# alipbcs/ZetaRay

Hardware: NVIDIA H100
Metric: Mpaths/s (1spp ReSTIR PT, 1080p) (higher is better)
Workload: dtype f32

## Files before the change

include/zr_abi.h:

```cpp
#ifndef ZR_ABI_H
#define ZR_ABI_H

#include <stdint.h>
#include <stddef.h>

#ifdef __cplusplus
extern "C" {
#endif

#if defined(_WIN32)
#define ZR_API __declspec(dllexport)
#else
#define ZR_API __attribute__((visibility("default")))
#endif

typedef int32_t zr_status;
enum
{
    ZR_OK = 0,
    ZR_ERR_INVALID_ARG = 1,
    ZR_ERR_CUDA = 2,
    ZR_ERR_NOT_INITIALIZED = 3,
    ZR_ERR_UNSUPPORTED = 4,
    ZR_ERR_OUT_OF_MEMORY = 5
// ... 176 lines not shown
    uint32_t le_b_meta;
    uint32_t lightIdx;
    float w_sum;
    float W;
    uint32_t pad[2];
} zr_rdi_reservoir;

typedef struct zr_image2d
{
    void* d_ptr;
    uint32_t width;
    uint32_t height;
    uint32_t pitch_bytes;
    uint32_t texel_bytes;
} zr_image2d;

typedef void (*zr_halo_exchange_fn)(void* user, const zr_image2d* planes, int n_planes, void* stream);

typedef struct zr_scene zr_scene;

typedef struct zr_scene_desc
{
    const zr_vertex* h_vertices;            uint32_t num_vertices;
    const uint32_t* h_indices;              uint32_t num_indices;
    const zr_mesh_instance* h_instances;    uint32_t num_instances;
    const uint32_t* h_instance_num_tris;
    const zr_material* h_materials;         uint32_t num_materials;
    const zr_emissive_tri* h_emissives;     uint32_t num_emissives;
} zr_scene_desc;

ZR_API zr_status zr_scene_create(const zr_scene_desc* desc, zr_scene** out);
ZR_API void zr_scene_destroy(zr_scene* scene);
ZR_API zr_status zr_scene_bvh_stats(const zr_scene* scene, uint32_t out[4]);

ZR_API zr_status zr_bvh_build_host(const float* h_world_tris, uint32_t num_tris, void* h_nodes, uint32_t node_capacity,
    uint32_t* h_leaf_order, uint32_t out_info[4]);

ZR_API zr_status zr_scene_trace_closest(const zr_scene* scene, const float* d_rays, uint32_t n,
    float* d_hits, void* stream);
ZR_API zr_status zr_scene_trace_any(const zr_scene* scene, const float* d_rays, uint32_t n,
    uint32_t* d_hit_flags, void* stream);


ZR_API zr_status zr_alias_table_build(float* d_weights, uint32_t n, zr_alias_entry* d_table,
    uint32_t* d_scratch, void* stream);
ZR_API zr_status zr_alias_table_sample(const zr_alias_entry* d_table, uint32_t n, uint32_t seed,
    uint32_t num_draws, uint32_t* d_out_idx, float* d_out_pdf, void* stream);
ZR_API zr_status zr_estimate_emissive_power(const zr_scene* scene, float* d_power, void* stream);
ZR_API zr_status zr_prelighting_render(zr_scene* scene, void* stream);

typedef struct zr_presampled_tri
{
    float pos[3];
    uint32_t normal;
    float pdf;
    uint32_t ID;
    uint32_t idx;
    uint32_t bary;
    uint16_t le[3];
    uint16_t twoSided;
} zr_presampled_tri;
#define ZR_PRESAMPLING_MIN_EMISSIVES 13107u
#define ZR_PRESAMPLING_NUM_SETS 128u
#define ZR_PRESAMPLING_SET_SIZE 512u
ZR_API zr_status zr_scene_set_presampling(zr_scene* scene, uint32_t num_sets, uint32_t set_size);
ZR_API zr_status zr_presample_emissives(zr_scene* scene, uint32_t frame_num, void* stream);
// ... 221 lines not shown
```

zetaray_b200/csrc/rdi.cu:

```cuda
#include "zr_pixel.cuh"
#include "zr_planes.h"
#include "zr_schedule.h"

#include "zr_rdi.cuh"

namespace zr
{
namespace
{
#ifndef ZR_RDI_THREADS
#define ZR_RDI_THREADS 512
#endif
    __global__ void ZR_LB(ZR_RDI_THREADS) k_di_temporal(SceneDev sc, FrameView f, DIParams prm, zr_rdi_reservoir* __restrict__ resCurr,
        const zr_rdi_reservoir* __restrict__ resPrev, uint2* __restrict__ target, float4* __restrict__ finalImg, uint32_t dispX, uint32_t dispY,
        const uint32_t* __restrict__ order)
    {
        const zr_frame_constants& fc = f.fc;
        uint2 sg = make_uint2(0, 0);
        const uint32_t groupFlat = order[blockIdx.x] * (ZR_RDI_THREADS / 64) + (threadIdx.x >> 6);
        const uint32_t tInGroup = threadIdx.x & 63;
        uint2 px = make_uint2(0xffffffffu, 0xffffffffu);
        if (groupFlat < dispX * dispY)
            px = SwizzleThreadGroup(groupFlat, 0, tInGroup & 7, tInGroup >> 3, 8, 8, dispX, 16, 4, 16 * dispY, sg);
        const long long t0 = clock64();
        bool act = !(px.x >= f.W || px.y >= f.H || px.y < prm.rowBegin || px.y >= prm.rowEnd);
        const uint32_t x = px.x, y = px.y;
        const size_t idx = act ? (size_t)y * f.W + x : 0;
        if (act)
        {
            const GFlags flags = FlagsAt(f.core, f.W, x, y);
            if (flags.invalid)
            {
                finalImg[idx] = f4(0, 0, 0, 0);
                act = false;
            }
            else if (flags.emissive && !prm.spatial)
            {
                WriteEmissive(fc, f, finalImg, idx);
                act = false;
            }
        }
        Pixel p;
        p.surface = BSDF::ShadingData::InitEmpty();
        p.pos = f3(0); p.normal = f3(0); p.roughness = 0;
        RNG rng_thread; rng_thread.State = 0;
        int numBsdfSamples = 0;
        if (act)
        {
            p = LoadPixel(f, sc, f.core, f.coat, x, y, false, x, y);
            rng_thread = RNG::Init(x, y, fc.FrameNum);
            numBsdfSamples = (!p.surface.GlossSpecular() && p.roughness < 0.3f) ? 2 : 1;
        }
        RNG rng_group = RNG::Init(groupFlat % dispX, groupFlat / dispX, fc.FrameNum);
        const uint32_t sampleSetIdx = rng_group.UniformUintBounded_Faster(sc.numSampleSets);
        Reservoir r = RIS_InitialCandidates_Sync(act, sc, p.pos, p.normal, p.roughness, p.surface, sampleSetIdx, numBsdfSamples, rng_thread);
        if (prm.temporal)
        {
            float2 motionVec = f2(0, 0);
            TemporalCandidate tc; tc.valid = false; tc.px = tc.py = 0; tc.pos = tc.normal = f3(0);
            tc.surface = BSDF::ShadingData::InitEmpty();
            ZR_PHASE();
            if (act)
            {
                motionVec = unpack_snorm16x2(__ldg(&f.me[idx].x));
                const float2 currUV = f2((float)x + 0.5f, (float)y + 0.5f) / f2((float)f.W, (float)f.H);
                const float2 prevUV = currUV - motionVec;
                tc = FindTemporalCandidate(f, sc, p.pos, p.normal, p.roughness, p.surface, prevUV);
            }
            TemporalResample1_Sync(act && tc.valid, sc, p.pos, p.normal, p.surface, tc, resPrev, f.W, r, rng_thread);
            if (act && prm.spatial)
            {
                const bool disoccluded = !tc.valid && (dot(motionVec, motionVec) > 0);
                r.target = disoccluded ? -r.target : r.target;
                WriteTarget(target, idx, r.target);
                r.target = Math::Sanitize(r.target);
            }
        }
        AccountCost(prm.costMap, f.W, f.H, px.x, px.y, t0);
        if (!act)
            return;
        if (prm.temporal || prm.reset)
        {
            zr_rdi_reservoir rec;
            r.Write(rec, prm.M_max);
            StoreRdi(&resCurr[idx], rec);
        }
        if (!prm.spatial || !prm.temporal)
            WriteFinal(fc, finalImg, idx, r.target * r.W);
    }

    __global__ void ZR_LB(ZR_RDI_THREADS) k_di_spatial(SceneDev sc, FrameView f, DIParams prm, const zr_rdi_reservoir* __restrict__ resCurr,
        const uint2* __restrict__ target, float4* __restrict__ finalImg, uint32_t dispX, uint32_t dispY,
        const uint32_t* __restrict__ order)
    {
        const zr_frame_constants& fc = f.fc;
        uint2 sg = make_uint2(0, 0);
        const uint32_t groupFlat = order[blockIdx.x] * (ZR_RDI_THREADS / 64) + (threadIdx.x >> 6);
        const uint32_t tInGroup = threadIdx.x & 63;
        uint2 px = make_uint2(0xffffffffu, 0xffffffffu);
        if (groupFlat < dispX * dispY)
            px = SwizzleThreadGroup(groupFlat, 0, tInGroup & 7, tInGroup >> 3, 8, 8, dispX, 16, 4, 16 * dispY, sg);
        const long long t0 = clock64();
        bool active = px.x < f.W && px.y < f.H && px.y >= prm.rowBegin && px.y < prm.rowEnd;
        const int x = (int)px.x, y = (int)px.y;
        const size_t idx = active ? (size_t)y * f.W + x : 0;
        if (active)
        {
            const GFlags flags = FlagsAt(f.core, f.W, x, y);
            if (flags.invalid) active = false;
            else if (flags.emissive)
            {
                WriteEmissive(fc, f, finalImg, idx);
                active = false;
            }
        }
        Pixel p;
        p.surface = BSDF::ShadingData::InitEmpty();
        p.pos = f3(0); p.normal = f3(0); p.roughness = 0; p.z = 0;
        Reservoir r = Reservoir::Init();
        bool disoccluded = false;
        if (active)
        {
            p = LoadPixel(f, sc, f.core, f.coat, x, y, false, x, y);
            zr_rdi_reservoir rec;
            LoadRdi(&resCurr[idx], rec);
            r = Reservoir::Load(rec);
            if (r.lightIdx != UINT32_MAX_)
            {
                const zr_emissive_tri& tri = sc.emissives[r.lightIdx];
                r.lightID = tri.ID;
                const float3 vtx0 = Light::Vtx0(tri);
                const float3 vtx1 = Light::DecodeEmissiveTriV1(tri);
                const float3 vtx2 = Light::DecodeEmissiveTriV2(tri);
                r.lightPos = (1.0f - r.bary.x - r.bary.y) * vtx0 + r.bary.x * vtx1 + r.bary.y * vtx2;
                r.lightNormal = cross(vtx1 - vtx0, vtx2 - vtx0);
                r.lightNormal = dot(r.lightNormal, r.lightNormal) == 0 ? r.lightNormal : normalize(r.lightNormal);
                r.doubleSided = Light::IsDoubleSided(tri);
                r.target = LoadTarget(target, idx);
                disoccluded = r.target.x < 0 || r.target.y < 0 || r.target.z < 0;
                r.target = abs3(r.target);
            }
        }
        const uint32_t waveDisoccluded = __popc(__ballot_sync(0xffffffffu, active && disoccluded));
        RNG rng_group = RNG::Init(groupFlat % dispX, groupFlat / dispX, fc.FrameNum);
        rng_group.UniformUintBounded_Faster(sc.numSampleSets);
        const bool extra = !prm.stochasticSpatial || (rng_group.Uniform() < 0.6f);
        if (prm.extraDisocclusion)
            disoccluded = disoccluded && (waveDisoccluded > 3);
        int numSamples = extra ? 2 : 1;
        numSamples = !disoccluded ? numSamples : 4;
        RNG rng = RNG::Init((uint32_t)x, (uint32_t)y, fc.FrameNum);
        const float u0 = rng.Uniform();
        const int offset = (int)rng.UniformUintBounded_Faster(8);
        const float theta = u0 * TWO_PI;
        float sinTheta, cosTheta;
        zr_sincosf(theta, &sinTheta, &cosTheta);
        PairwiseMIS pairwiseMIS = PairwiseMIS::Init((uint32_t)numSamples, r);
        float3 samplePos[4]; int spx[4], spy[4]; uint32_t k = 0;
        ZR_PHASE();
        for (int i = 0; i < 4; i++)
        {
            if (!(active && i < numSamples)) continue;
            const float2 sampleUV = f2(c_disk32[((offset + i) & 31) * 2], c_disk32[((offset + i) & 31) * 2 + 1]);
            float2 rotated;
            rotated.x = dot(sampleUV, f2(cosTheta, -sinTheta));
            rotated.y = dot(sampleUV, f2(sinTheta, cosTheta));
            rotated = rotated * 16.0f;
            const float fx = fmaxf(rintf((float)x + rotated.x), 0.0f), fy = fmaxf(rintf((float)y + rotated.y), 0.0f);
            if (fx >= (float)f.W || fy >= (float)f.H) continue;
            const int qx = (int)fx, qy = (int)fy;
            float rough_i;
            const GFlags flags_i = FlagsAt(f.core, f.W, qx, qy, &rough_i);
            if (flags_i.invalid || flags_i.emissive) continue;
            const Pixel pi = LoadPixel(f, sc, f.core, f.coat, qx, qy, false, qx, qy);
            bool valid = PlaneHeuristicDI(pi.pos, p.normal, p.pos, p.z);
            valid = valid && (fabsf(rough_i - p.roughness) < 0.15f);
            if (!valid) continue;
            samplePos[k] = pi.pos; spx[k] = qx; spy[k] = qy;
            k++;
        }
        pairwiseMIS.k = k;
        for (uint32_t i = 0; i < 4; i++)
        {
            const bool go = active && (i < k);
            if (!__syncthreads_or(go))
                break;
            Pixel pi;
            pi.normal = f3(0);
            BSDF::ShadingData surface_i = BSDF::ShadingData::InitEmpty();
            Reservoir r_spatial = Reservoir::Init();
            float3 pos_i = f3(0);
            if (go)
            {
                pi = LoadPixel(f, sc, f.core, f.coat, spx[i], spy[i], false, spx[i], spy[i]);
                const uint4 c = ld128(&f.core[(size_t)spy[i] * f.W + spx[i]]);
                const float3 bc = f3((float)(c.z & 0xff) / 255.0f, (float)((c.z >> 8) & 0xff) / 255.0f, (float)((c.z >> 16) & 0xff) / 255.0f);
                const float bw = pi.flags.subsurface ? (float)(c.z >> 24) / 255.0f : 0.0f;
                pos_i = samplePos[i];
                const float3 wo_i = normalize(pi.origin - pos_i);
                surface_i = BSDF::ShadingData::Init(pi.normal, wo_i, pi.flags.metallic, pi.roughness, bc, BSDF::ETA_AIR,
                    pi.eta_next, pi.flags.transmissive, 0.0f, to_half(bw), pi.surface.coat_weight, pi.surface.coat_color,
                    pi.coatRoughness, pi.coatIor, sc.rho);
                zr_rdi_reservoir recN;
                LoadRdi(&resCurr[(size_t)spy[i] * f.W + spx[i]], recN);
                r_spatial = Reservoir::Load(recN);
            }
            pairwiseMIS.Stream_Sync(go, sc, r, p.pos, p.normal, p.surface, r_spatial, pos_i, pi.normal, surface_i, rng);
        }
        AccountCost(prm.costMap, f.W, f.H, px.x, px.y, t0);
        if (!active)
            return;
        pairwiseMIS.End(r, rng);
        const Reservoir rs = pairwiseMIS.r_s;
        WriteFinal(fc, finalImg, idx, rs.target * rs.W);
    }
}
}

struct zr_direct_pass
{
    uint32_t width = 0, height = 0;
    struct Sized
    {
        zr::Planes planes{ "zr_direct_pass" };
        zr_rdi_reservoir* d_res[2] = { nullptr, nullptr };
        uint2* d_target = nullptr;
        float4* d_final = nullptr;
    } sz;
    int currTemporalIdx = 0;
    bool isTemporalReservoirValid = false;
    bool resetTemporalTextures = true;
    bool patternLoaded = false;
    zr_direct_params params = Defaults();
// ... 30 lines not shown
    }
    zr_status LoadPattern()
    {
        if (patternLoaded) return ZR_OK;
        float pat[64];
        zr_status st = zr::read_asset("zr_direct_pass", "disk32.bin", pat, sizeof(pat));
        if (st != ZR_OK) return st;
        ZR_CUDA(cudaMemcpyToSymbol(zr::c_disk32, pat, 256));
        patternLoaded = true;
        return ZR_OK;
    }
    zr_status Render(const zr_frame_inputs* in, cudaStream_t stream)
    {
        using namespace zr;
        FrameView f;
        zr_status st = LightingFrame("zr_direct_pass", in, width, height, f);
        if (st != ZR_OK) return st;
        st = LoadPattern();
        if (st != ZR_OK) return st;
        const bool doTemporal = isTemporalReservoirValid && params.temporal_resample;
        const bool doSpatial = doTemporal && params.spatial_resample;
        if (doTemporal && (!in->prev.d_core || !in->prev.d_coat))
        {
            set_error("zr_direct_pass_render: temporal reuse needs the previous G-buffer");
            return ZR_ERR_INVALID_ARG;
        }
        DIParams prm{ doTemporal, doSpatial, params.stochastic_spatial, params.extra_disocclusion_sampling, params.M_max,
            params.alpha_min, resetTemporalTextures, strip.rowBegin, strip.ClampedRowEnd(height), strip.d_costMap };
        const uint32_t dispX = (width + 7) / 8, dispY = (height + 7) / 8;
        const int cur = currTemporalIdx;
        st = strip.Schedule(width, height, 8, 8, ZR_RDI_THREADS / 64);
        if (st != ZR_OK) return st;
        const BlockSchedule& sched = strip.sched;
        ZR_PROF("k_di_temporal", stream);
        k_di_temporal<<<sched.count, ZR_RDI_THREADS, 0, stream>>>(in->scene->dev, f, prm, sz.d_res[cur], sz.d_res[1 - cur], sz.d_target, sz.d_final, dispX, dispY, sched.d_order);
        ZR_LAUNCH_CHECK();
        strip.Exchange(sz.d_res[cur], width, height, 32u, stream);
        if (doSpatial)
        {
            ZR_PROF("k_di_spatial", stream);
            k_di_spatial<<<sched.count, ZR_RDI_THREADS, 0, stream>>>(in->scene->dev, f, prm, sz.d_res[cur], sz.d_target, sz.d_final, dispX, dispY, sched.d_order);
            ZR_LAUNCH_CHECK();
        }
        isTemporalReservoirValid = true;
        currTemporalIdx = 1 - cur;
        resetTemporalTextures = false;
        return ZR_OK;
    }
};

extern "C"
{
    zr_status zr_direct_pass_create(uint32_t width, uint32_t height, zr_direct_pass** out) { return zr::CreatePass("zr_direct_pass", width, height, out); }
    zr_status zr_direct_pass_resize(zr_direct_pass* p, uint32_t width, uint32_t height) { return zr::ResizePass("zr_direct_pass", p, width, height); }
    zr_status zr_direct_pass_reset_temporal(zr_direct_pass* p) { return zr::ResetPass(p); }
    zr_status zr_direct_pass_default_params(zr_direct_params* out) { return zr::DefaultParams<zr_direct_pass>(out); }
    zr_status zr_direct_pass_set_params(zr_direct_pass* p, const zr_direct_params* params)
    {
        if (!p || !params) return ZR_ERR_INVALID_ARG;
        if (params->M_max == 0 || params->M_max > 31) { zr::set_error("zr_direct_pass_set_params: M_max must be in 1..31 (5-bit field)"); return ZR_ERR_INVALID_ARG; }
        p->params = *params;
        return ZR_OK;
    }
    zr_status zr_direct_pass_render(zr_direct_pass* p, const zr_frame_inputs* in, void* stream)
    {
        if (!p) return ZR_ERR_INVALID_ARG;
        return p->Render(in, (cudaStream_t)stream);
    }
    zr_status zr_direct_pass_set_rows(zr_direct_pass* p, uint32_t y0, uint32_t y1) { return p ? p->strip.SetRows(y0, y1, p->height) : ZR_ERR_INVALID_ARG; }
    zr_status zr_direct_pass_set_halo_exchange(zr_direct_pass* p, zr_halo_exchange_fn fn, void* user) { return p ? p->strip.SetHaloExchange(fn, user) : ZR_ERR_INVALID_ARG; }
    zr_status zr_direct_pass_set_schedule_costs(zr_direct_pass* p, const double* h_tile_cost, uint32_t tiles_x, uint32_t tiles_y)
    {
        return p ? p->strip.SetScheduleCosts(h_tile_cost, tiles_x, tiles_y, p->width, p->height) : ZR_ERR_INVALID_ARG;
    }
// ... 28 lines not shown
```

zetaray_b200/csrc/rpt.cu:

```cuda
#include "zr_rpt_io.cuh"
#include "zr_rpt_spatial.h"
#include "zr_schedule.h"

namespace zr
{
namespace
{
    using namespace RPT;

    __device__ __align__(8) float c_disk512[1024];

#ifndef ZR_PT_THREADS
#define ZR_PT_THREADS 768
#endif
    struct PtParked
    {
        Reservoir r;
        Reconnection rc;
        uint32_t pad;
    };
    static_assert(sizeof(PtParked) % 4 == 0 && (sizeof(PtParked) / 4) % 2 == 1, "PtParked must be an odd number of words");
    constexpr size_t PT_SMEM_BYTES = (size_t)ZR_PT_THREADS * sizeof(PtParked);

    __global__ void ZR_LB(ZR_PT_THREADS) k_pathtrace(SceneDev sc, FrameView f, RptParams prm, zr_rpt_reservoir* __restrict__ res,
        float4* __restrict__ target, float4* __restrict__ finalImg, uint32_t dispX, uint32_t dispY, const uint32_t* __restrict__ order)
    {
        extern __shared__ PtParked s_ptParked[];
        const zr_frame_constants& fc = f.fc;
        const long long t0 = clock64();
        uint2 sg = make_uint2(0, 0);
        const uint32_t groupFlat = order[blockIdx.x] * (ZR_PT_THREADS / 128) + (threadIdx.x >> 7);
        const uint32_t tInGroup = threadIdx.x & 127;
        uint2 px = make_uint2(0xffffffffu, 0xffffffffu);
        if (groupFlat < dispX * dispY)
            px = SwizzleThreadGroup(groupFlat, 0, tInGroup & 15, tInGroup >> 4, 16, 8, dispX, 16, 4, 16 * dispY, sg);
        bool inBounds = px.x < f.W && px.y < f.H && px.y >= prm.rowBegin && px.y < prm.rowEnd;
        const size_t idx = (size_t)px.y * f.W + px.x;
        bool alive = false;
        if (inBounds)
        {
            const GFlags flags = FlagsAt(f.core, f.W, px.x, px.y);
            if (flags.invalid || flags.emissive)
            {
                if (!fc.Accumulate || !fc.CameraStatic)
                    finalImg[idx] = f4(0, 0, 0, 0);
                inBounds = false;
            }
        }
        float3 pos = f3(0), normal = f3(0), li = f3(0), throughput = f3(0), throughput_k = f3(1), tr = f3(1);
        BSDF::ShadingData surface;
        BSDF::BSDFSample bsdfSample = BSDF::BSDFSample::Init();
        HitEmissive nextHit;
        nextHit.hit = false;
        Reconnection& rc = s_ptParked[threadIdx.x].rc;
        Reservoir& r = s_ptParked[threadIdx.x].r;
        rc = Reconnection::Init();
        r = Reservoir::Init();
        PrevHit prevHit;
        prevHit.alpha_lobe = 0; prevHit.wi = f3(0); prevHit.pdf = 0; prevHit.lobe = BSDF::DIFFUSE_R;
        float eta_curr = BSDF::ETA_AIR, eta_next = BSDF::DEFAULT_ETA_MAT;
        bool inTranslucentMedium = false;
        int bounce = 0, maxNumBounces = 0;
        RNG rngReplay, rngThread, rngGroup;
        rngReplay.State = rngThread.State = rngGroup.State = 0;
        uint32_t sampleSetIdx = 0;
        uint32_t seedReplay0 = 0;

        if (inBounds)
        {
            const Pixel p = LoadPixel(f, sc, f.core, f.coat, px.x, px.y, false, px.x, px.y);
            rngGroup = RNG::Init4(sg.x, sg.y, fc.FrameNum, 1);
            const uint3 state = RNG::PCG3d(make_uint3(px.x, px.y, fc.FrameNum));
            rngReplay = RNG::InitSeed(state.x);
            rngThread = RNG::InitSeed(state.y);
            seedReplay0 = state.x;
            maxNumBounces = (int)(p.surface.specTr ? prm.maxGlossyTrBounces : prm.maxNonTrBounces);
            bsdfSample = BSDF::SampleBSDF(p.normal, p.surface, rngReplay);
            if (dot(bsdfSample.bsdfOverPdf, bsdfSample.bsdfOverPdf) != 0)
            {
                sampleSetIdx = rngGroup.UniformUintBounded_Faster(sc.numSampleSets);
                pos = p.pos; normal = p.normal; surface = p.surface;
                throughput = bsdfSample.bsdfOverPdf;
                prevHit.alpha_lobe = BSDF::LobeAlpha(p.surface, bsdfSample.lobe);
                prevHit.lobe = bsdfSample.lobe; prevHit.wi = bsdfSample.wi; prevHit.pdf = bsdfSample.pdf;
                eta_curr = dot(p.normal, bsdfSample.wi) < 0 ? p.eta_next : BSDF::ETA_AIR;
                inTranslucentMedium = eta_curr != BSDF::ETA_AIR;
                alive = true;
            }
        }
        ZR_PHASE();
        if (alive)
            nextHit = FindClosestEmissive(sc, pos, normal, bsdfSample.wi, surface.Transmissive());

        while (__syncthreads_or(alive))
        {
            bool atRR = false;
            Hit hitInfo;
            float prevBsdfSamplePdf = 0; BSDF::LOBE prevBsdfSampleLobe = BSDF::DIFFUSE_R;
            const int pathVertex = bounce + 2;
            if (alive && !nextHit.hit)
                alive = false;
            if (alive)
            {
                hitInfo = HitAttributes(sc, nextHit.geoIdx, nextHit.primIdx, nextHit.bary, nextHit.t);
                const float3 newPos = mad(hitInfo.t, bsdfSample.wi, pos);
                if (!GetMaterialData(sc, -bsdfSample.wi, eta_curr, hitInfo, surface, eta_next))
                    alive = false;
                else
                {
                    pos = newPos;
                    normal = hitInfo.normal;
                    prevBsdfSamplePdf = bsdfSample.pdf;
                    prevBsdfSampleLobe = bsdfSample.lobe;
                    tr = f3(1);
                    if (inTranslucentMedium && (surface.trDepth > 0))
                    {
                        const float3 c = surface.baseColor_Fr0_TrCol;
                        const float3 extCoeff = f3(-zr_logf(c.x), -zr_logf(c.y), -zr_logf(c.z)) / surface.trDepth;
                        tr = f3(zr_expf(-hitInfo.t * extCoeff.x), zr_expf(-hitInfo.t * extCoeff.y), zr_expf(-hitInfo.t * extCoeff.z));
                        throughput *= tr;
                    }
                }
            }
            ZR_PHASE();
            BSDF::BSDFSample nextBsdfSample = bsdfSample;
            const int nextBounce = pathVertex - 1;
            if (alive && nextBounce <= maxNumBounces)
                nextBsdfSample = BSDF::SampleBSDF(hitInfo.normal, surface, rngReplay);
            ZR_PHASE();
            RaySetup rs; rs.go = false;
            RayHit rh; rh.hit = false;
            if (alive)
            {
                rs = SetupClosestEmissive(pos, hitInfo.normal, nextBsdfSample.wi, surface.Transmissive());
                if (rs.go)
                    rh = TraceClosest(sc, rs.o, nextBsdfSample.wi, rs.tmin, FLT_MAX_);
            }
            ZR_PHASE();
            NeeLightState nee;
            nee.facing = false; nee.ld = f3(0);
            bool lightSample = false;
            uint32_t seed_nee = 0;
            if (alive)
            {
                nextHit = FinishClosestEmissive(sc, rs, rh, nextBsdfSample.wi);
                const DirectLightingEstimate ls_b = NEE_Bsdf_Finish(sc, pos, surface, nextBounce, maxNumBounces, nextBsdfSample, nextHit);
                if (nextHit.HitWasEmissive())
                {
                    const float3 fOverPdf = throughput * ls_b.ld;
                    li += fOverPdf;
                    rc.L = Reconnection::half3(ls_b.ld * throughput_k);
                    MaybeSetCase2OrCase3(pathVertex, pos, hitInfo.normal, hitInfo.t, hitInfo.ID, hitInfo.meshIdx, surface,
                        prevHit, ls_b, 0, rc, prm.alpha_min);
                    r.Update(Math::Luminance(fOverPdf), fOverPdf, rc, rngThread);
                }
                lightSample = !IsSpecularSurface(surface);
                if (lightSample)
                {
                    seed_nee = rngThread.State;
                    BSDF::ShadingData surfNee = surface;
                    nee = NEE_Emissive_Begin(sc, pos, hitInfo.normal, surfNee, sampleSetIdx, rngThread);
                }
            }
            ZR_PHASE();
            if (lightSample && nee.facing && dot(nee.ld, nee.ld) > 0)
            {
                const RaySetup seg = SetupSegment(pos, nee.ret.wi, nee.t, hitInfo.normal, nee.ret.ID, surface.Transmissive());
                const bool visible = seg.go ? !TraceAnyExcept(sc, seg.o, nee.ret.wi, seg.tmin, seg.tmax, nee.ret.ID) : false;
                nee.ld *= visible ? 1.0f : 0.0f;
            }
            ZR_PHASE();
            if (lightSample)
            {
                float bsdfPdf = 0;
                if (nee.facing && dot(nee.ld, nee.ld) > 0)
                {
                    BSDF::ShadingData surfNee = surface;
                    surfNee.SetWi(nee.ret.wi, hitInfo.normal);
                    bsdfPdf = BSDF::BSDFSamplerPdf(hitInfo.normal, surfNee, nee.ret.wi, rngThread);
                    bsdfPdf *= nee.dwdA;
                }
                const DirectLightingEstimate ls = NEE_Emissive_Finish(nee, bsdfPdf);
                const float3 fOverPdf = throughput * ls.ld;
                li += fOverPdf;
                if (rc.IsCase2() || rc.IsCase3())
                    rc.Clear();
                rc.L = Reconnection::half3(ls.ld * throughput_k);
                MaybeSetCase2OrCase3(pathVertex, pos, hitInfo.normal, hitInfo.t, hitInfo.ID, hitInfo.meshIdx, surface,
                    prevHit, ls, seed_nee, rc, prm.alpha_min);
                r.Update(Math::Luminance(fOverPdf), fOverPdf, rc, rngThread);
            }
            if (alive)
            {
                bsdfSample = nextBsdfSample;
                if (bounce >= (maxNumBounces - 1))
                    alive = false;
                else
                {
                    if (rc.IsCase2() || rc.IsCase3())
                        rc.Clear();
                    bounce++;
                    atRR = true;
                }
            }
            const uint32_t rrMask = __ballot_sync(0xffffffffu, atRR);
            if (rrMask == 0)
                continue;
            const int rrBounce = __shfl_sync(0xffffffffu, bounce, __ffs(rrMask) - 1);
            const bool doRR = prm.russianRoulette && (rrBounce >= 3);
            float waveThroughput = 0.0f;
// ... 251 lines not shown

struct zr_indirect_pass
{
    uint32_t width = 0, height = 0;
    struct Sized
    {
        zr::Planes planes{ "zr_indirect_pass" };
        zr_rpt_reservoir* d_res[2] = { nullptr, nullptr };
        float4* d_target = nullptr;
        float4* d_final = nullptr;
        uint16_t* d_neighbor = nullptr;
        uint16_t* d_threadMap = nullptr;
        zr::SpatialQueued queued;
    } sz;
    zr::ShiftStreams shiftStreams;
    int currTemporalIdx = 0;
    bool isTemporalReservoirValid = false;
    bool resetTemporalTextures = true;
    bool patternLoaded = false;
    zr::LightingStrip strip{ "zr_indirect_pass" };
    zr_indirect_params params = Defaults();

    static zr_indirect_params Defaults()
    {
        zr_indirect_params p{};
        p.max_non_tr_bounces = 3; p.max_glossy_tr_bounces = 4; p.russian_roulette = 1; p.temporal_resample = 1;
        p.num_spatial_passes = 1; p.M_max_temporal = 10; p.M_max_spatial = 8; p.boiling_suppression = 1;
        p.sort_temporal = 1; p.sort_spatial = 1; p.alpha_min = 0.175f * 0.175f;
        return p;
    }

    zr_status Setup()
    {
        ZR_CUDA(cudaFuncSetAttribute(zr::k_pathtrace, cudaFuncAttributeMaxDynamicSharedMemorySize, (int)zr::PT_SMEM_BYTES));
        int ptBlocks = 0;
        ZR_CUDA(cudaOccupancyMaxActiveBlocksPerMultiprocessor(&ptBlocks, zr::k_pathtrace, ZR_PT_THREADS, zr::PT_SMEM_BYTES));
        if (ptBlocks < 1)
        {
            zr::set_error("zr_indirect_pass: k_pathtrace (%d threads, %zu B shared) cannot be resident", ZR_PT_THREADS, zr::PT_SMEM_BYTES);
            return ZR_ERR_UNSUPPORTED;
        }
        const size_t ptSmem = (size_t)ptBlocks * (zr::PT_SMEM_BYTES + 1024);
        ZR_CUDA(cudaFuncSetAttribute(zr::k_pathtrace, cudaFuncAttributePreferredSharedMemoryCarveout,
            (int)((ptSmem * 100 + 228 * 1024 - 1) / (228 * 1024))));
        return shiftStreams.Init();
    }

    zr_status OnWindowResized(uint32_t w, uint32_t h)
    {
        const size_t n = (size_t)w * h;
        Sized next;
        for (int i = 0; i < 2; i++) ZR_TRY(next.planes.Alloc(next.d_res[i], n));
        ZR_TRY(next.planes.Alloc(next.d_threadMap, n));
        ZR_TRY(next.planes.Alloc(next.d_target, n));
        ZR_TRY(next.planes.Alloc(next.d_final, n));
        ZR_TRY(next.planes.Alloc(next.d_neighbor, n));
        ZR_TRY(next.queued.Build(w, h, next.d_res[0], next.d_res[1]));
        ZR_TRY(next.planes.Clear());
        sz = std::move(next);
        width = w; height = h;
        strip.ForgetSize();
        ResetFlags();
        return ZR_OK;
    }

    void ResetFlags() { currTemporalIdx = 0; isTemporalReservoirValid = false; resetTemporalTextures = true; }
    zr_status ResetTemporal()
    {
        ZR_TRY(sz.planes.Clear());
        ResetFlags();
        return ZR_OK;
    }

    zr_status LoadPattern()
    {
        if (patternLoaded) return ZR_OK;
        float pat[1024];
// ... 3 lines not shown
        patternLoaded = true;
        return ZR_OK;
    }

    zr_status Render(const zr_frame_inputs* in, cudaStream_t stream)
    {
        using namespace zr;
        FrameView f;
        zr_status st = LightingFrame("zr_indirect_pass", in, width, height, f);
        if (st != ZR_OK) return st;
        st = LoadPattern();
        if (st != ZR_OK) return st;

        const bool doTemporal = params.temporal_resample && isTemporalReservoirValid;
        const bool doSpatial = (params.num_spatial_passes > 0) && doTemporal;
        if (doTemporal && (!in->prev.d_core || !in->prev.d_coat))
        {
            set_error("zr_indirect_pass_render: temporal reuse needs the previous G-buffer");
            return ZR_ERR_INVALID_ARG;
        }
        RptParams prm;
        prm.maxNonTrBounces = params.max_non_tr_bounces; prm.maxGlossyTrBounces = params.max_glossy_tr_bounces;
        prm.russianRoulette = params.russian_roulette; prm.M_max_temporal = params.M_max_temporal; prm.M_max_spatial = params.M_max_spatial;
        prm.boilingSuppression = params.boiling_suppression; prm.sortSpatial = params.sort_spatial; prm.alpha_min = params.alpha_min;
        prm.temporalResample = doTemporal; prm.resetTemporal = resetTemporalTextures; prm.spatialFlag = doSpatial;
        prm.rowBegin = strip.rowBegin; prm.rowEnd = strip.ClampedRowEnd(height);
        prm.costMap = strip.d_costMap;
        st = strip.Schedule(width, height, 16, 8, ZR_PT_THREADS / 128);
        if (st != ZR_OK) return st;
        const uint32_t rows = prm.rowEnd - prm.rowBegin;

        int cur = currTemporalIdx;
        const uint32_t dispX = (width + 15) / 16, dispY = (height + 7) / 8;
        ZR_PROF("k_pathtrace", stream);
        k_pathtrace<<<strip.sched.count, ZR_PT_THREADS, PT_SMEM_BYTES, stream>>>(in->scene->dev, f, prm, sz.d_res[cur], sz.d_target, sz.d_final, dispX, dispY,
            strip.sched.d_order);
        ZR_LAUNCH_CHECK();
        if (doTemporal)
        {
            st = sz.queued.RunTemporal(shiftStreams, in->scene->dev, f, prm, sz.d_res[cur], sz.d_res[1 - cur], sz.d_target, sz.d_final, stream);
            if (st != ZR_OK) return st;
        }
        strip.Exchange(sz.d_res[cur], width, height, 64u, stream);
        if (doSpatial)
        {
            for (uint32_t pass = 0; pass < params.num_spatial_passes; pass++)
            {
                ZR_PROF("k_spatial_search", stream);
                k_spatial_search<<<dim3((width + 31) / 32, (rows + 7) / 8), 256, 0, stream>>>(f, prm, sz.d_neighbor);
                ZR_LAUNCH_CHECK();
                zr_rpt_reservoir* rin = sz.d_res[cur];
                zr_rpt_reservoir* rout = sz.d_res[1 - cur];
                cur = 1 - cur;
                if (params.sort_spatial)
                {
                    const uint32_t sx = (width + 31) / 32, sy = (height + 31) / 32;
                    ZR_PROF("k_sort", stream);
                    const uint32_t ty0 = prm.rowBegin / 32, ty1 = (prm.rowEnd + 31) / 32;
                    k_sort<<<dim3(sx, ty1 - ty0), 256, 0, stream>>>(f, 3, 1u, rin, nullptr, sz.d_neighbor, sz.d_threadMap, sx, sy, ty0);
                    ZR_LAUNCH_CHECK();
                }
                st = sz.queued.Run(shiftStreams, in->scene->dev, f, prm, rin, rout, sz.d_target, sz.d_final, sz.d_neighbor, sz.d_threadMap, stream);
                if (st != ZR_OK) return st;
                strip.Exchange(rout, width, height, 64u, stream);
            }
        }
        isTemporalReservoirValid = true;
        currTemporalIdx = 1 - cur;
        resetTemporalTextures = false;
        return ZR_OK;
    }
};

extern "C"
{
    zr_status zr_indirect_pass_create(uint32_t width, uint32_t height, zr_indirect_pass** out) { return zr::CreatePass("zr_indirect_pass", width, height, out); }
    zr_status zr_indirect_pass_resize(zr_indirect_pass* p, uint32_t width, uint32_t height) { return zr::ResizePass("zr_indirect_pass", p, width, height); }
    zr_status zr_indirect_pass_reset_temporal(zr_indirect_pass* p) { return zr::ResetPass(p); }
    zr_status zr_indirect_pass_default_params(zr_indirect_params* out) { return zr::DefaultParams<zr_indirect_pass>(out); }
    zr_status zr_indirect_pass_set_params(zr_indirect_pass* p, const zr_indirect_params* params)
    {
        if (!p || !params) return ZR_ERR_INVALID_ARG;
        if (params->max_non_tr_bounces < 1 || params->max_non_tr_bounces > 8 || params->max_glossy_tr_bounces < 1 ||
            params->max_glossy_tr_bounces > 8 || params->M_max_temporal > 15 || params->M_max_spatial > 15 || params->num_spatial_passes > 2)
        {
            zr::set_error("zr_indirect_pass_set_params: value out of range (bounces 1..8, M_max <= 15, spatial passes <= 2)");
            return ZR_ERR_INVALID_ARG;
        }
        p->params = *params;
        return ZR_OK;
    }
    zr_status zr_indirect_pass_render(zr_indirect_pass* p, const zr_frame_inputs* in, void* stream)
    {
        if (!p) return ZR_ERR_INVALID_ARG;
        return p->Render(in, (cudaStream_t)stream);
// ... 38 lines not shown
```

zetaray_b200/csrc/rpt_spatial.cu:

```cuda
#include "zr_rpt_spatial.h"
#include "zr_rpt_shift.cuh"
#include "zr_tma.cuh"

namespace zr
{
namespace
{
    using namespace RPT;

    __global__ void __launch_bounds__(256) k_spatial_classify(FrameView f, RptParams prm, const zr_rpt_reservoir* __restrict__ resIn,
        const uint16_t* __restrict__ neighbor, uint32_t* __restrict__ queue, uint32_t* __restrict__ counters, uint32_t capacity)
    {
        __shared__ uint32_t s_count[SpatialQueued::NUM_CLASSES], s_base[SpatialQueued::NUM_CLASSES];
        const uint32_t x = blockIdx.x * 32 + (threadIdx.x & 31);
        const uint32_t y = prm.rowBegin + blockIdx.y * 8 + (threadIdx.x >> 5);
        if (threadIdx.x < SpatialQueued::NUM_CLASSES) s_count[threadIdx.x] = 0;
        __syncthreads();
        uint32_t cls[2] = { NO_ITEM, NO_ITEM };
        if (x < f.W && y < f.H && y < prm.rowEnd)
        {
            const GFlags flags = FlagsAt(f.core, f.W, (int)x, (int)y);
            int nx = 0, ny = 0;
            if (!(flags.invalid || flags.emissive) && NeighborOf(f, neighbor, (int)x, (int)y, nx, ny))
            {
// ... 290 lines not shown
    capacity = 2 * n;
    ZR_TRY(planes.Alloc(d_queue, NUM_CLASSES * capacity, false));
    ZR_TRY(planes.Alloc(d_counters, 16, false));
    ZR_TRY(planes.Alloc(d_shift, n));
    ZR_TRY(planes.Alloc(d_flags, n));
    ZR_TRY(planes.Alloc(d_maps, 2, false));
    const zr_rpt_reservoir* res[2] = { res0, res1 };
    CUtensorMap maps[2];
    swizzled = (w % 2) == 0;
    for (int i = 0; i < 2; i++)
    {
        mapBase[i] = res[i];
        bool ok;
        if (swizzled)
        {
            const uint64_t dims[3] = { 16, w / 2, h };
            const uint64_t strides[2] = { 128, (uint64_t)w * 64 };
            const uint32_t box[3] = { 16, 16, 32 };
            ok = tma::EncodeWords(&maps[i], res[i], 3, dims, strides, box, true);
        }
        else
            ok = tma::EncodePlane2D(&maps[i], res[i], w, h, 64, (uint64_t)w * 64, 32, 32);
        if (!ok)
        {
            set_error("zr_indirect_pass: cuTensorMapEncodeTiled failed for the %ux%u reservoir plane", w, h);
            return ZR_ERR_CUDA;
        }
    }
    ZR_CUDA(cudaMemcpy(d_maps, maps, sizeof(maps), cudaMemcpyHostToDevice));
    return planes.Clear();
}

zr_status SpatialQueued::Run(const ShiftStreams& ss, const SceneDev& sc, const FrameView& f, const RptParams& prm, const zr_rpt_reservoir* resIn,
    zr_rpt_reservoir* resOut, const float4* target, float4* finalImg, const uint16_t* neighbor, const uint16_t* threadMap, cudaStream_t stream)
{
    const int plane = resIn == mapBase[0] ? 0 : (resIn == mapBase[1] ? 1 : -1);
    if (plane < 0) { set_error("zr_indirect_pass: spatial input is not one of the pass's reservoir planes"); return ZR_ERR_INVALID_ARG; }
    const uint32_t rows = prm.rowEnd - prm.rowBegin;
    ZR_CUDA(cudaMemsetAsync(d_counters, 0, 16 * sizeof(uint32_t), stream));
    {
        ZR_PROF("k_spatial_classify", stream);
        k_spatial_classify<<<dim3((width + 31) / 32, (rows + 7) / 8), 256, 0, stream>>>(f, prm, resIn, neighbor, d_queue, d_counters, (uint32_t)capacity);
        ZR_LAUNCH_CHECK();
    }
    {
        ZR_PROF("k_shift", stream);
        const zr_status ls = LaunchShifts<false>(*this, ss, sc, f, prm, resIn, nullptr, neighbor, stream);
        zr::prof_after();
        if (ls != ZR_OK) return ls;
        cudaError_t e = cudaGetLastError();
        if (e != cudaSuccess) return zr::cuda_fail(e, "k_shift launch");
    }
    {
        const uint32_t tilesX = (width + 31) / 32;
        const uint32_t tileRow0 = prm.rowBegin / 32, tileRow1 = (prm.rowEnd + 31) / 32;
        const uint32_t numTiles = tilesX * (tileRow1 - tileRow0);
        const uint32_t grid = numTiles < (uint32_t)ss.numSMs ? numTiles : (uint32_t)ss.numSMs;
        ZR_PROF("k_spatial_merge", stream);
        k_spatial_merge<<<grid, 1024, sizeof(MergeSmem), stream>>>(d_maps + plane, f, prm, resIn, resOut, target, finalImg, neighbor, threadMap,
            d_shift, tilesX, tileRow0, numTiles, swizzled ? 1u : 0u);
        ZR_LAUNCH_CHECK();
    }
    return ZR_OK;
}
}
```

zetaray_b200/csrc/rpt_temporal.cu:

```cuda
#include "zr_rpt_spatial.h"
#include "zr_rpt_shift.cuh"

namespace zr
{
namespace
{
    using namespace RPT;
    enum : uint8_t { TF_OK = 1, TF_REPLAY_OK = 2 };

    __global__ void __launch_bounds__(256) k_temporal_classify(SceneDev sc, FrameView f, RptParams prm, const zr_rpt_reservoir* __restrict__ resCurr,
        const zr_rpt_reservoir* __restrict__ resPrev, uint8_t* __restrict__ tflags, uint32_t* __restrict__ queue, uint32_t* __restrict__ counters,
        uint32_t capacity)
    {
        __shared__ uint32_t s_count[SpatialQueued::NUM_CLASSES], s_base[SpatialQueued::NUM_CLASSES];
        const int x = (int)(blockIdx.x * 32 + (threadIdx.x & 31));
        const int y = (int)(prm.rowBegin + blockIdx.y * 8 + (threadIdx.x >> 5));
        if (threadIdx.x < SpatialQueued::NUM_CLASSES) s_count[threadIdx.x] = 0;
        __syncthreads();
        uint32_t cls[2] = { NO_ITEM, NO_ITEM };
        uint32_t flagBits = 0;
        if (x < (int)f.W && y < (int)f.H && y < (int)prm.rowEnd)
        {
            const size_t idx = (size_t)y * f.W + x;
            const GFlags flags = DecodeFlags(ld128(&f.core[idx]).w & 0xff);
// ... 115 lines not shown
            const float m_prev = denom > 0 ? numerator / denom : 0;
            const float w_prev = m_prev * r_prev.W * targetLum_curr;
            if (r_curr.Update(w_prev, shTarget, r_prev.rc, rng))
            {
                r_curr.rc.partialJacobian = shJ;
                changed = true;
            }
        }
        const float targetLum = Math::Luminance(r_curr.target);
        r_curr.W = targetLum > 0 ? r_curr.w_sum / targetLum : 0;
        r_curr.M = M_new;
        if (changed)
        {
            zr_rpt_reservoir out;
            r_curr.Write(out, M_max);
            StoreRecord(&resCurr[idx], out);
            if (prm.spatialFlag)
            {
                r_curr.target = Math::Sanitize(r_curr.target);
                target[idx] = f4(r_curr.target.x, r_curr.target.y, r_curr.target.z, 0.0f);
            }
        }
        else
        {
            r_curr.WriteReservoirData(rec, M_max);
            st128(&resCurr[idx], make_uint4(rec.meta, asuint(rec.w_sum), asuint(rec.W), rec.L_b));
        }
        if (!prm.spatialFlag)
            WriteOutputColor(fc, finalImg, idx, r_curr.target * r_curr.W);
    }
}

zr_status SpatialQueued::RunTemporal(const ShiftStreams& ss, const SceneDev& sc, const FrameView& f, const RptParams& prm, zr_rpt_reservoir* resCurr,
    const zr_rpt_reservoir* resPrev, float4* target, float4* finalImg, cudaStream_t stream)
{
    const uint32_t rows = prm.rowEnd - prm.rowBegin;
    const dim3 grid((width + 31) / 32, (rows + 7) / 8);
    ZR_CUDA(cudaMemsetAsync(d_counters, 0, 16 * sizeof(uint32_t), stream));
    {
        ZR_PROF("k_temporal_classify", stream);
        k_temporal_classify<<<grid, 256, 0, stream>>>(sc, f, prm, resCurr, resPrev, d_flags, d_queue, d_counters, (uint32_t)capacity);
        ZR_LAUNCH_CHECK();
    }
    {
        ZR_PROF("k_shift_temporal", stream);
        const zr_status ls = LaunchShifts<true>(*this, ss, sc, f, prm, resCurr, resPrev, nullptr, stream);
        zr::prof_after();
        if (ls != ZR_OK) return ls;
        cudaError_t e = cudaGetLastError();
        if (e != cudaSuccess) return zr::cuda_fail(e, "k_shift (temporal) launch");
    }
    {
        ZR_PROF("k_temporal_merge", stream);
        k_temporal_merge<<<grid, 256, 0, stream>>>(sc, f, prm, resCurr, resPrev, target, finalImg, d_flags, d_shift);
        ZR_LAUNCH_CHECK();
    }
    return ZR_OK;
}
}
```

zetaray_b200/csrc/scene.cu:

```cuda
#include "zr_scene.cuh"
#include <vector>
#include <algorithm>
#include <cmath>
#include <cstring>

namespace zr
{
namespace
{
    __global__ void k_world_tris(SceneDev sc, const uint32_t* __restrict__ triMesh, const uint32_t* __restrict__ meshFirstTri,
        uint32_t numTris, float* __restrict__ out )
    {
        const uint32_t g = blockIdx.x * blockDim.x + threadIdx.x;
        if (g >= numTris) return;
        const uint32_t m = triMesh[g];
        const uint32_t p = g - meshFirstTri[m];
        const zr_mesh_instance md = LoadInstance(sc, m);
        const float4 q = normalize(Math::DecodeNormalized4(md.Rotation));
        const float3 s = h3(md.Scale);
        const float3 t = f3(md.Translation[0], md.Translation[1], md.Translation[2]);
        const uint32_t tri = p * 3 + md.BaseIdxOffset;
        float3 pw[3];
        for (int k = 0; k < 3; k++)
        {
// ... 59 lines not shown
            if (mi.MatIdx >= desc->num_materials)
            {
                set_error("zr_scene_create: instance %u uses material %u of %u", m, (unsigned)mi.MatIdx, desc->num_materials);
                return ZR_ERR_INVALID_ARG;
            }
            for (uint64_t i = 0; i < 3 * nt; i++)
                if ((uint64_t)mi.BaseVtxOffset + desc->h_indices[mi.BaseIdxOffset + i] >= desc->num_vertices)
                {
                    set_error("zr_scene_create: instance %u, index %llu points past the vertex buffer", m, (unsigned long long)i);
                    return ZR_ERR_INVALID_ARG;
                }
            if (mi.BaseEmissiveTriOffset != 0xffffffffu && (uint64_t)mi.BaseEmissiveTriOffset + nt > desc->num_emissives)
            {
                set_error("zr_scene_create: instance %u's emissive triangles [%u, %llu) lie past the %u emissive triangles", m,
                    mi.BaseEmissiveTriOffset, (unsigned long long)(mi.BaseEmissiveTriOffset + nt), desc->num_emissives);
                return ZR_ERR_INVALID_ARG;
            }
            totalTris += nt;
        }
        if (totalTris == 0) { set_error("zr_scene_create: scene has no triangles"); return ZR_ERR_INVALID_ARG; }
        if (totalTris > 0x7fffffffull) { set_error("zr_scene_create: more than 2^31 triangles"); return ZR_ERR_INVALID_ARG; }
        if (desc->num_emissives && !desc->h_emissives) { set_error("zr_scene_create: null emissive buffer"); return ZR_ERR_INVALID_ARG; }
    }
    zr_scene* sc = new zr_scene();
    zr_status st;
#define UP(field, ptr, n) if ((st = upload(sc, ptr, n, &sc->dev.field)) != ZR_OK) { zr_scene_destroy(sc); return st; }
    UP(vertices, desc->h_vertices, desc->num_vertices);
    UP(indices, desc->h_indices, desc->num_indices);
    UP(instances, desc->h_instances, desc->num_instances);
    UP(materials, desc->h_materials, desc->num_materials);
    UP(emissives, desc->h_emissives, desc->num_emissives);
    sc->dev.numInstances = desc->num_instances;
    sc->dev.numEmissives = desc->num_emissives;

    std::vector<uint32_t> triMesh, meshFirst(desc->num_instances);
    uint32_t total = 0;
    for (uint32_t m = 0; m < desc->num_instances; m++)
    {
        meshFirst[m] = total;
        if (desc->h_instances[m].BaseIdxOffset + 3 * desc->h_instance_num_tris[m] > desc->num_indices)
        {
            set_error("zr_scene_create: instance %u indexes past the index buffer", m);
            zr_scene_destroy(sc);
            return ZR_ERR_INVALID_ARG;
        }
        for (uint32_t p = 0; p < desc->h_instance_num_tris[m]; p++) triMesh.push_back(m);
        total += desc->h_instance_num_tris[m];
    }
    if (total == 0) { set_error("zr_scene_create: scene has no triangles"); zr_scene_destroy(sc); return ZR_ERR_INVALID_ARG; }
    sc->dev.numTris = total;
    UP(triMesh, triMesh.data(), triMesh.size());
    UP(meshFirstTri, meshFirst.data(), meshFirst.size());

    {
        std::vector<uint16_t> rho(64 * 32 * 16);
        if ((st = read_asset("zr_scene_create", "rho_lut.bin", rho.data(), rho.size() * sizeof(uint16_t))) != ZR_OK) { zr_scene_destroy(sc); return st; }
        UP(rho, rho.data(), rho.size());
    }

    float* d_wt = nullptr;
    cudaError_t e = cudaMalloc(&d_wt, (size_t)total * 9 * sizeof(float));
    if (e != cudaSuccess) { zr_scene_destroy(sc); return cuda_fail(e, "world triangles (alloc)"); }
    k_world_tris<<<(total + 127) / 128, 128>>>(sc->dev, sc->dev.triMesh, sc->dev.meshFirstTri, total, d_wt);
    count_launch();
    e = cudaGetLastError();
    std::vector<float> wt((size_t)total * 9);
// ... 51 lines not shown
    zr_status zr_scene_create(const zr_scene_desc* desc, zr_scene** out) { return zr::scene_create(desc, out); }
    void zr_scene_destroy(zr_scene* sc)
    {
        if (!sc) return;
        for (int i = 0; i < sc->numAllocs; i++) cudaFree(sc->allocs[i]);
        if (sc->d_alias) cudaFree(sc->d_alias);
        if (sc->d_power) cudaFree(sc->d_power);
        if (sc->d_aliasScratch) cudaFree(sc->d_aliasScratch);
        if (sc->d_sampleSets) cudaFree(sc->d_sampleSets);
        if (sc->d_lvg) cudaFree(sc->d_lvg);
        delete sc;
    }
    zr_status zr_bvh_build_host(const float* h_world_tris, uint32_t num_tris, void* h_nodes, uint32_t node_capacity,
        uint32_t* h_leaf_order, uint32_t out_info[4])
    {
        if (!h_world_tris || !out_info || num_tris == 0) { zr::set_error("zr_bvh_build_host: null argument"); return ZR_ERR_INVALID_ARG; }
        zr::BvhBuild w;
        zr::build_bvh8(h_world_tris, num_tris, w);
        out_info[0] = (uint32_t)w.nodes.size(); out_info[1] = num_tris; out_info[2] = w.maxDepth; out_info[3] = w.maxStack;
        if (h_nodes)
        {
            if (node_capacity < w.nodes.size()) { zr::set_error("zr_bvh_build_host: %zu nodes, capacity %u", w.nodes.size(), node_capacity); return ZR_ERR_INVALID_ARG; }
            memcpy(h_nodes, w.nodes.data(), w.nodes.size() * sizeof(zr::BVH8Node));
        }
        if (h_leaf_order) memcpy(h_leaf_order, w.leafOrder.data(), (size_t)num_tris * sizeof(uint32_t));
        return ZR_OK;
    }
    zr_status zr_scene_bvh_stats(const zr_scene* sc, uint32_t out[4])
    {
        if (!sc || !out) return ZR_ERR_INVALID_ARG;
        out[0] = sc->info.numNodes; out[1] = sc->info.numTris; out[2] = sc->info.maxDepth; out[3] = sc->info.bytes;
        return ZR_OK;
    }
    zr_status zr_scene_trace_closest(const zr_scene* sc, const float* d_rays, uint32_t n, float* d_hits, void* stream)
    {
        if (!sc || !d_rays || !d_hits) { zr::set_error("zr_scene_trace_closest: null argument"); return ZR_ERR_INVALID_ARG; }
        if (n == 0) return ZR_OK;
        ZR_PROF("k_trace_closest", (cudaStream_t)stream);
        zr::k_trace_closest<<<(n + 127) / 128, 128, 0, (cudaStream_t)stream>>>(sc->dev, d_rays, n, d_hits);
        ZR_LAUNCH_CHECK();
        return ZR_OK;
    }
    zr_status zr_scene_trace_any(const zr_scene* sc, const float* d_rays, uint32_t n, uint32_t* d_flags, void* stream)
    {
        if (!sc || !d_rays || !d_flags) { zr::set_error("zr_scene_trace_any: null argument"); return ZR_ERR_INVALID_ARG; }
        if (n == 0) return ZR_OK;
        ZR_PROF("k_trace_any", (cudaStream_t)stream);
        zr::k_trace_any<<<(n + 127) / 128, 128, 0, (cudaStream_t)stream>>>(sc->dev, d_rays, n, d_flags);
        ZR_LAUNCH_CHECK();
        return ZR_OK;
    }
    zr_status zr_scene_get_alias_table(const zr_scene* sc, const zr_alias_entry** d_table, uint32_t* n)
    {
        if (!sc || !d_table || !n) return ZR_ERR_INVALID_ARG;
        *d_table = sc->d_alias; *n = sc->dev.numEmissives;
        return ZR_OK;
    }
}
```

zetaray_b200/csrc/zr_bsdf.cuh:

```cuda
#pragma once
#include "zr_common.cuh"

namespace zr
{
namespace RT
{
    ZR_D float BalanceHeuristic(float p_1, float p_2, float f, float n_1 = 1, float n_2 = 1)
    {
        float denom = n_1 * p_1 + n_2 * p_2;
        if (denom == 0) return 0;
        return (n_1 * f) / denom;
    }
    ZR_D float BalanceHeuristic3(float p_1, float p_2, float p_3, float f, float n_1 = 1, float n_2 = 1, float n_3 = 1)
    {
        float denom = n_1 * p_1 + n_2 * p_2 + n_3 * p_3;
        if (denom == 0) return 0;
        return (n_1 * f) / denom;
    }
    ZR_D float3 PowerHeuristic(float p_1, float p_2, float3 f, float n_1 = 1, float n_2 = 1)
    {
        float a = n_1 * p_1;
        float b = n_2 * p_2;
        float denom = a * a + b * b;
        if (denom == 0) return f3(0);
// ... 149 lines not shown
        f *= dwh_dwi;
        f *= ndotwi;
        return f * (1 - fr);
    }
    ZR_D float3 SampleGGXVNDF(float3 wo, float alpha_x, float alpha_y, float2 u)
    {
        float3 Vh = normalize(f3(alpha_x * wo.x, alpha_y * wo.y, wo.z));
        float phi = TWO_PI * u.x;
        float z = mad((1.0f - u.y), (1.0f + Vh.z), -Vh.z);
        float sinTheta = sqrtf(saturate(1.0f - z * z));
        float s, c;
        zr_sincosf(phi, &s, &c);
        float x = sinTheta * c;
        float y = sinTheta * s;
        float3 cc = f3(x, y, z);
        float3 Nh = cc + Vh;
        return normalize(f3(alpha_x * Nh.x, alpha_y * Nh.y, fmaxf(0.0f, Nh.z)));
    }
    ZR_D float3 SampleGGXMicrofacet(float3 wo, float alpha, float3 shadingNormal, float2 u)
    {
        Math::CoordinateSystem onb = Math::CoordinateSystem::Build(shadingNormal);
        float3 woLocal = f3(dot(onb.b1, wo), dot(onb.b2, wo), dot(shadingNormal, wo));
        float3 whLocal = SampleGGXVNDF(woLocal, alpha, alpha, u);
        return mad(whLocal.x, onb.b1, mad(whLocal.y, onb.b2, whLocal.z * shadingNormal));
    }
    ZR_D float GGXMicrofacetPdf(float alpha, float ndotwh, float ndotwo)
    {
        float alphaSq = alpha * alpha;
        float NDF = GGX(ndotwh, alphaSq);
        float G1 = SmithG1(alphaSq, ndotwo);
        return (NDF * G1) / ndotwo;
    }

    struct ShadingData
    {
        float alpha;
        float3 wo;
        float ndotwi, ndotwo, ndotwh, whdotwi, whdotwo, wodotwi, g_wo;
        float3 baseColor_Fr0_TrCol;
        float eta;
        bool specTr, metallic, backfacing_wo, invalid, reflection;
        float trDepth;
        float subsurface;
        float coat_weight;
        float3 coat_color;
        float coat_alpha;
        float coat_eta;
        const uint16_t* rho;

        static ZR_D ShadingData InitEmpty()
        {
            ShadingData ret;
            memset(&ret, 0, sizeof(ret));
            ret.eta = DEFAULT_ETA_MAT / ETA_AIR;
            ret.coat_eta = DEFAULT_ETA_COAT;
            return ret;
        }
        static ZR_D ShadingData Init(float3 shadingNormal, float3 wo, bool metallic, float roughness, float3 baseColor,
            float eta_curr = ETA_AIR, float eta_next = DEFAULT_ETA_MAT, bool specTr = false,
            float transmissionDepth = 0, float subsurface = 0, float coat_weight = 0, float3 coat_color = f3(0.0f),
            float coat_roughness = 0, float eta_coat = DEFAULT_ETA_COAT, const uint16_t* rhoTable = nullptr)
        {
            float2 roughness4 = f2(roughness, coat_roughness);
            if (coat_weight > 0 && coat_roughness > 0)
            {
                roughness4 = roughness4 * roughness4;
                roughness4 = roughness4 * roughness4;
                float roughness_coated = fminf(roughness4.x + 2 * roughness4.y, 1);
                roughness_coated = rsqrt_(rsqrt_(roughness_coated));
                roughness = Math::Lerp(roughness, roughness_coated, coat_weight);
            }
            ShadingData si;
            memset(&si, 0, sizeof(si));
            si.wo = wo;
            float ndotwo = dot(shadingNormal, wo);
            si.backfacing_wo = ndotwo <= 0;
            si.ndotwo = fmaxf(ndotwo, 1e-5f);
            si.metallic = metallic;
            si.alpha = roughness * roughness;
            si.baseColor_Fr0_TrCol = baseColor;
            si.specTr = specTr;
            si.trDepth = to_half(transmissionDepth);
            si.subsurface = to_half(subsurface);
            float eta_base = eta_curr == ETA_AIR ? eta_next : eta_curr;
            float eta_no_coat = eta_next / eta_curr;
            float eta_coated = eta_base >= eta_coat ? eta_base / eta_coat : eta_coat / eta_base;
            si.eta = Math::Lerp(eta_no_coat, eta_coated, coat_weight);
            si.g_wo = !metallic && !specTr ? E_FON_approx(fmaxf(ndotwo, 1e-4f), roughness) : 0;
            si.coat_weight = coat_weight;
            si.coat_color = coat_color;
            si.coat_alpha = coat_roughness * coat_roughness;
            si.coat_eta = eta_curr == ETA_AIR ? eta_coat / ETA_AIR : ETA_AIR / eta_coat;
            si.rho = rhoTable;
            return si;
        }

        ZR_D bool ThinWalled() const { return subsurface > 0; }
        ZR_D bool Transmissive() const { return specTr || ThinWalled(); }
        ZR_D bool Coated() const { return coat_weight != 0; }
        ZR_D bool GlossSpecular() const { return alpha <= MAX_ALPHA_SPECULAR; }
        ZR_D bool CoatSpecular() const { return coat_alpha <= MAX_ALPHA_SPECULAR; }
        ZR_D float3 TransmissionTint() const { return trDepth > 0 ? f3(1) : baseColor_Fr0_TrCol; }

        ZR_D void SetWi_Refl(float3 wi, float3 shadingNormal, float3 wh)
        {
            reflection = true;
            float ndotwi_n = dot(shadingNormal, wi);
            ndotwh = saturate(dot(shadingNormal, wh));
            whdotwo = saturate(dot(wh, wo));
            whdotwi = whdotwo;
            bool isInvalid = backfacing_wo || ndotwh == 0 || whdotwo == 0;
            invalid = isInvalid || ndotwi_n <= 0;
            ndotwi = fmaxf(ndotwi_n, 1e-5f);
            wodotwi = dot(wo, wi);
        }
        ZR_D void SetWi_Refl(float3 wi, float3 shadingNormal)
        {
            float3 wh = normalize(wi + wo);
            SetWi_Refl(wi, shadingNormal, wh);
        }
        ZR_D void SetWi_Tr(float3 wi, float3 shadingNormal, float3 wh)
        {
            reflection = false;
            float ndotwi_n = dot(shadingNormal, wi);
            ndotwh = saturate(dot(shadingNormal, wh));
            whdotwo = saturate(dot(wh, wo));
            whdotwi = fabsf(dot(wh, wi));
            bool isInvalid = backfacing_wo || (specTr && (ndotwh == 0 || whdotwo == 0));
            invalid = isInvalid || ndotwi_n >= 0 || !Transmissive() || metallic;
            ndotwi = fmaxf(fabsf(ndotwi_n), 1e-5f);
            wodotwi = dot(wo, wi);
        }
// ... 27 lines not shown
            tir = false;
            if (metallic)
                return FresnelSchlick(fr0, cosTheta_i);
            float eta_relative = 1.0f / eta;
            float sinTheta_iSq = saturate(mad(-cosTheta_i, cosTheta_i, 1.0f));
            float cosTheta_tSq = mad(-eta_relative * eta_relative, sinTheta_iSq, 1.0f);
            tir = cosTheta_tSq <= 0;
            if (tir)
                return f3(1);
            float cosTheta_t = sqrtf(cosTheta_tSq);
            return f3(Fresnel_Dielectric(cosTheta_i, eta_relative, cosTheta_t));
        }
        ZR_D float3 Fresnel() const
        {
            float3 fr0 = metallic ? baseColor_Fr0_TrCol : f3(DielectricF0(eta));
            bool unused;
            return Fresnel(fr0, unused);
        }
        ZR_D float Fresnel_Coat(float& cosTheta_t) const
        {
            cosTheta_t = 0;
            float cosTheta_i = whdotwo;
            float eta_relative = 1.0f / coat_eta;
            float sinTheta_iSq = saturate(mad(-cosTheta_i, cosTheta_i, 1.0f));
            float cosTheta_tSq = mad(-eta_relative * eta_relative, sinTheta_iSq, 1.0f);
            if (cosTheta_tSq <= 0)
                return 1;
            cosTheta_t = sqrtf(cosTheta_tSq);
            float Fr0 = DielectricF0(coat_eta);
            float cosTheta = coat_eta > 1 ? cosTheta_i : cosTheta_t;
            return FresnelSchlick_Dielectric(Fr0, cosTheta);
        }
    };

    ZR_D bool IsLobeValid(const ShadingData& surface, LOBE lt)
    {
        if (lt == ALL) return true;
        if (surface.metallic && (lt != GLOSSY_R) && (lt != COAT)) return false;
        if (!surface.specTr && (lt == GLOSSY_T)) return false;
        if (surface.specTr && (lt == DIFFUSE_R)) return false;
        if (!surface.ThinWalled() && (lt == DIFFUSE_T)) return false;
        if (!surface.Coated() && (lt == COAT)) return false;
        return true;
    }
    ZR_D float LobeAlpha(const ShadingData& surface, LOBE lt)
    {
        if (lt == GLOSSY_R || lt == GLOSSY_T) return surface.alpha;
        if (lt == COAT) return surface.coat_alpha;
        return 1.0f;
    }

    ZR_D float3 EvalDiffuse(bool EON, const ShadingData& surface)
    {
        float s = surface.subsurface == 0 ? 1 : surface.subsurface * 0.5f;
        float diffuseRoughness = sqrtf(surface.alpha);
        float3 diffuse = OrenNayar(EON, surface.baseColor_Fr0_TrCol, diffuseRoughness, surface.ndotwo, surface.ndotwi,
            surface.wodotwi, surface.g_wo);
        return s * diffuse;
    }
    ZR_D float3 SampleDiffuse(float3 normal, float2 u, float& pdf)
    {
        float3 wiLocal = Sampling::SampleCosineWeightedHemisphere(u, pdf);
        Math::CoordinateSystem onb = Math::CoordinateSystem::Build(normal);
        return mad(wiLocal.x, onb.b1, mad(wiLocal.y, onb.b2, wiLocal.z * normal));
    }
    ZR_D float DiffusePdf(const ShadingData& surface) { return surface.ndotwi * ONE_OVER_PI; }
    ZR_D float3 EvalGloss(const ShadingData& surface, float3 fr)
    {
        return GGXMicrofacetBRDF(surface.alpha, surface.ndotwh, surface.ndotwo, surface.ndotwi, fr, surface.GlossSpecular());
    }
    ZR_D float3 SampleGloss(const ShadingData& surface, float3 shadingNormal, float2 u)
    {
        if (surface.GlossSpecular())
            return reflect(-surface.wo, shadingNormal);
        float3 wh = SampleGGXMicrofacet(surface.wo, surface.alpha, shadingNormal, u);
        return reflect(-surface.wo, wh);
    }
    ZR_D float GlossPdf(const ShadingData& surface)
    {
        if (surface.GlossSpecular())
            return surface.ndotwh >= MIN_N_DOT_H_SPECULAR ? 1.0f : 0.0f;
        float pdf = GGXMicrofacetPdf(surface.alpha, surface.ndotwh, surface.ndotwo);
        return pdf / 4.0f;
    }
    ZR_D float EvalTranslucentTr(const ShadingData& surface, float fr)
    {
        return GGXMicrofacetBTDF(surface.alpha, surface.ndotwh, surface.ndotwo, surface.ndotwi, surface.whdotwo,
            surface.whdotwi, surface.eta, fr, surface.GlossSpecular());
    }
    ZR_D float EvalCoat(const ShadingData& surface, float Fr)
    {
        return surface.coat_weight * GGXMicrofacetBRDF(surface.coat_alpha, surface.ndotwh, surface.ndotwo, surface.ndotwi,
            f3(Fr), surface.CoatSpecular()).x;
    }
    ZR_D float3 SampleCoat(const ShadingData& surface, float3 shadingNormal, float2 u)
    {
        float3 wh = surface.CoatSpecular() ? shadingNormal :
            SampleGGXMicrofacet(surface.wo, surface.coat_alpha, shadingNormal, u);
        return reflect(-surface.wo, wh);
    }
    ZR_D float CoatPdf(const ShadingData& surface)
    {
        if (surface.CoatSpecular())
            return surface.ndotwh >= MIN_N_DOT_H_SPECULAR ? 1.0f : 0.0f;
        float pdf = GGXMicrofacetPdf(surface.coat_alpha, surface.ndotwh, surface.ndotwo);
        return pdf / 4.0f;
    }
    ZR_D float3 TranslucentTrOverPdf(const ShadingData& surface, float fr)
    {
        if (surface.GlossSpecular())
            return (1 - fr) * surface.TransmissionTint();
        float alphaSq = surface.alpha * surface.alpha;
        return SmithHeightCorrelatedG2OverG1(alphaSq, surface.ndotwi, surface.ndotwo) * (1 - fr) * surface.TransmissionTint();
    }
    ZR_D float3 coat_tr_pow(float3 coat_color, float c)
    {
        return f3(zr_expf(c * zr_logf(coat_color.x)), zr_expf(c * zr_logf(coat_color.y)), zr_expf(c * zr_logf(coat_color.z)));
    }
    ZR_D float3 BaseWeight(const ShadingData& surface)
    {
        float3 base_weight = f3(1);
        if (surface.Coated())
        {
            float cosTheta_t;
            float Fr_coat = surface.Fresnel_Coat(cosTheta_t);
            bool tir_c = cosTheta_t <= 0;
            if (tir_c)
                return f3(0);
            float reflectance_c = surface.CoatSpecular() ? Fr_coat :
                GGXReflectance_Dielectric(surface.rho, surface.coat_alpha, surface.ndotwo, surface.coat_eta);
            float c = 0.5f / cosTheta_t + 0.5f / surface.whdotwo;
            float3 coat_tr = coat_tr_pow(surface.coat_color, c);
            base_weight = Math::Lerp(f3(1.0f), (1 - reflectance_c) * coat_tr, surface.coat_weight);
        }
        return base_weight;
    }
    ZR_D float3 TransmittanceToDielectricBaseTr(const ShadingData& surface)
    {
        float3 base_weight = BaseWeight(surface);
        float reflectance_g = surface.GlossSpecular() ? 0 :
            GGXReflectance_Dielectric(surface.rho, surface.alpha, surface.ndotwo, surface.eta);
        return (1 - reflectance_g) * base_weight;
    }
    ZR_D float3 DielectricBaseSpecularTr(const ShadingData& surface, float Fr_g)
    {
        if (surface.invalid || !surface.specTr)
            return f3(0);
        float3 transmittance = TransmittanceToDielectricBaseTr(surface);
        float glossyTr = EvalTranslucentTr(surface, Fr_g);
        return glossyTr * surface.TransmissionTint() * transmittance;
    }
    ZR_D float3 DielectricBaseDiffuseTr(const ShadingData& surface, float Fr_g)
    {
        if (surface.invalid)
            return f3(0);
        float3 base_weight = BaseWeight(surface);
        float reflectance_g = surface.GlossSpecular() ? Fr_g :
            GGXReflectance_Dielectric(surface.rho, surface.alpha, surface.ndotwo, surface.eta);
        return (1 - reflectance_g) * EvalDiffuse(false, surface) * base_weight;
    }

    struct BSDFEval { float3 f; float3 Fr_g; bool tir; };

    ZR_D BSDFEval Unified(const ShadingData& surface)
    {
        BSDFEval ret;
        ret.f = f3(0); ret.Fr_g = f3(0); ret.tir = false;
        if (surface.invalid)
            return ret;
        float3 base_weight = f3(1);
        if (surface.Coated())
        {
            float cosThetaT_o;
            float Fr_coat = surface.Fresnel_Coat(cosThetaT_o);
            bool tir_c = cosThetaT_o <= 0;
            if (!surface.reflection && tir_c)
                return ret;
            if (surface.reflection)
            {
                ret.f = f3(EvalCoat(surface, Fr_coat));
                if (tir_c)
                    return ret;
            }
            float reflectance_c = surface.CoatSpecular() ? Fr_coat :
                GGXReflectance_Dielectric(surface.rho, surface.coat_alpha, surface.ndotwo, surface.coat_eta);
            float c = 1.0f / cosThetaT_o;
            float3 coat_tr = coat_tr_pow(surface.coat_color, c);
            base_weight = Math::Lerp(f3(1.0f), (1 - reflectance_c) * coat_tr, surface.coat_weight);
        }
        float3 fr0 = surface.metallic ? surface.baseColor_Fr0_TrCol : f3(DielectricF0(surface.eta));
        ret.Fr_g = surface.Fresnel(fr0, ret.tir);
        float3 glossyRefl = EvalGloss(surface, ret.Fr_g);
        if (surface.metallic || ret.tir)
        {
            ret.f += base_weight * glossyRefl;
            return ret;
        }
        float reflectance_g = surface.GlossSpecular() ? ret.Fr_g.x :
            GGXReflectance_Dielectric(surface.rho, surface.alpha, surface.ndotwo, surface.eta);
        if (!surface.specTr)
        {
            float3 diffuse = EvalDiffuse(true, surface);
            ret.f += base_weight * ((1 - reflectance_g) * diffuse + glossyRefl * (surface.reflection ? 1.0f : 0.0f));
            return ret;
        }
        if (surface.reflection)
        {
            ret.f += glossyRefl * base_weight;
            return ret;
        }
        reflectance_g = surface.GlossSpecular() ? 0 : reflectance_g;
        float glossyTr = EvalTranslucentTr(surface, ret.Fr_g.x);
        ret.f = ((1 - reflectance_g) * glossyTr * surface.TransmissionTint()) * base_weight;
        return ret;
    }

    struct BSDFSample
    {
        float3 wi; LOBE lobe; float pdf; float3 bsdfOverPdf; float3 f;
        static ZR_D BSDFSample Init() { BSDFSample r; r.wi = f3(0); r.lobe = DIFFUSE_R; r.pdf = 0; r.bsdfOverPdf = f3(0); r.f = f3(0); return r; }
    };
    struct BSDFSamplerEval { float pdf; float3 bsdfOverPdf; float3 f; };

    ZR_D BSDFSample SampleBSDF_NoDiffuse(float3 normal, ShadingData surface, float2 u_c, float2 u_g,
        float u_wrs_0, float u_wrs_1)
    {
        BSDFSample ret = BSDFSample::Init();
        float pdf_base = 1;
        if (surface.Coated())
        {
            float reflectance_c = GGXReflectance_Dielectric(surface.rho, surface.coat_alpha, surface.ndotwo, surface.coat_eta);
            float pdf_coat = reflectance_c * surface.coat_weight;
            pdf_base = 1 - pdf_coat;
            if (u_wrs_0 < pdf_coat)
            {
                float3 wi_c = SampleCoat(surface, normal, u_c);
                surface.SetWi_Refl(wi_c, normal);
                BSDFEval eval = Unified(surface);
                ret.wi = wi_c;
                ret.lobe = COAT;
                ret.f = eval.f;
                ret.pdf = CoatPdf(surface) * pdf_coat;
                ret.bsdfOverPdf = ret.f / ret.pdf;
                return ret;
            }
        }
        float3 wh = surface.GlossSpecular() ? normal : SampleGGXMicrofacet(surface.wo, surface.alpha, normal, u_g);
        float3 wi_r = reflect(-surface.wo, wh);
        surface.SetWi_Refl(wi_r, normal, wh);
        float wh_pdf = GGXMicrofacetPdf(surface.alpha, surface.ndotwh, surface.ndotwo);
        ret.wi = wi_r;
        ret.lobe = GLOSSY_R;
        ret.pdf = surface.GlossSpecular() ? 1 : wh_pdf / 4.0f;
        ret.pdf *= pdf_base;
        BSDFEval eval = Unified(surface);
        ret.f = eval.f;
        ret.bsdfOverPdf = ret.f / ret.pdf;
        if (surface.metallic || !surface.specTr || eval.tir)
            return ret;
        float3 wi_t = refract(-surface.wo, wh, 1 / surface.eta);
        float p_r = eval.Fr_g.x * Math::Luminance(f3(1.0f));
        p_r = p_r / (p_r + (1 - eval.Fr_g.x) * Math::Luminance(f3(1.0f)));
        if (u_wrs_1 < p_r)
        {
            ret.bsdfOverPdf /= p_r;
            ret.pdf *= p_r;
        }
        else
        {
            surface.SetWi_Tr(wi_t, normal, wh);
            ret.pdf = (1 - p_r) * pdf_base;
            if (!surface.GlossSpecular())
            {
                ret.pdf *= wh_pdf * surface.whdotwo;
                float dwh_dwi = JacobianHalfVecToIncident_Tr(surface.eta, surface.whdotwo, surface.whdotwi);
                ret.pdf *= dwh_dwi;
            }
            ret.f = DielectricBaseSpecularTr(surface, eval.Fr_g.x);
            ret.bsdfOverPdf = ret.pdf > 0 ? ret.f / ret.pdf : f3(0);
            ret.wi = wi_t;
            ret.lobe = GLOSSY_T;
        }
        return ret;
    }

    ZR_D BSDFSample SampleBSDF_NoDiffuse(float3 normal, const ShadingData& surface, RNG& rng)
    {
        float2 u_c = rng.Uniform2D();
        float2 u_g = rng.Uniform2D();
        float u_wrs_0 = rng.Uniform();
        float u_wrs_1 = rng.Uniform();
        return SampleBSDF_NoDiffuse(normal, surface, u_c, u_g, u_wrs_0, u_wrs_1);
    }

    ZR_D BSDFSample SampleBSDF_NoSpecTr(float3 normal, ShadingData surface, float2 u_coat, float2 u_g, float2 u_d,
        float u_wrs_g, float u_wrs_dr, float u_wrs_dt)
    {
        BSDFSample ret = BSDFSample::Init();
        float w_sum = 0;
        float3 target = f3(0);
        if (surface.Coated())
        {
            float3 wi_c = SampleCoat(surface, normal, u_coat);
            surface.SetWi_Refl(wi_c, normal);
            BSDFEval eval = Unified(surface);
            target = eval.f;
            ret.wi = wi_c;
            ret.lobe = COAT;
            ret.f = target;
            float pdf_c = CoatPdf(surface);
            float pdf_g = GlossPdf(surface);
            float pdf_d = !surface.metallic ? DiffusePdf(surface) : 0;
            float targetLum_c = Math::Luminance(target);
            w_sum = RT::BalanceHeuristic3(pdf_c, pdf_g, pdf_d, targetLum_c);
        }
        {
            float3 wi_g = SampleGloss(surface, normal, u_g);
            surface.SetWi_Refl(wi_g, normal);
            BSDFEval eval = Unified(surface);
            float3 target_g = eval.f;
            float pdf_g = GlossPdf(surface);
            float pdf_d = !surface.metallic && !eval.tir ? DiffusePdf(surface) : 0;
            float pdf_c = surface.Coated() ? CoatPdf(surface) : 0;
            float w_g = RT::BalanceHeuristic3(pdf_g, pdf_d, pdf_c, Math::Luminance(target_g));
            w_sum += w_g;
            if ((w_sum > 0) && (u_wrs_g < (w_g / w_sum)))
            {
                target = target_g;
// ... 15 lines not shown
                float pdf_g = GlossPdf(surface);
                float pdf_c = surface.Coated() ? CoatPdf(surface) : 0;
                float w_dr = RT::BalanceHeuristic3(pdf_d, pdf_g, pdf_c, Math::Luminance(target_dr));
                w_sum += w_dr;
                if ((w_sum > 0) && (u_wrs_dr < (w_dr / w_sum)))
                {
                    target = target_dr;
                    ret.wi = wi_d;
                    ret.lobe = DIFFUSE_R;
                    ret.f = target_dr;
                }
            }
            if (surface.ThinWalled())
            {
                float3 wi_dt = -wi_d;
                float3 target_dt = DielectricBaseDiffuseTr(surface, Fr_g);
                float w_dt = Math::Luminance(target_dt) / pdf_d;
                w_sum += w_dt;
                if ((w_sum > 0) && (u_wrs_dt < (w_dt / w_sum)))
                {
                    target = target_dt;
                    ret.wi = wi_dt;
                    ret.lobe = DIFFUSE_T;
                    ret.f = target_dt;
                }
            }
        }
        float targetLum = Math::Luminance(target);
        ret.bsdfOverPdf = targetLum > 0 ? target * w_sum / targetLum : f3(0);
        ret.pdf = w_sum > 0 ? targetLum / w_sum : 0;
        return ret;
    }

    ZR_D BSDFSample SampleBSDF(float3 normal, const ShadingData& surface, RNG& rng)
    {
        float2 u_c = rng.Uniform2D();
        float2 u_g = rng.Uniform2D();
        float2 u_d = rng.Uniform2D();
        float u_wrs_0 = rng.Uniform();
        float u_wrs_1 = rng.Uniform();
        float u_wrs_2 = rng.Uniform();
        if (!surface.specTr)
            return SampleBSDF_NoSpecTr(normal, surface, u_c, u_g, u_d, u_wrs_0, u_wrs_1, u_wrs_2);
        return SampleBSDF_NoDiffuse(normal, surface, u_c, u_g, u_wrs_0, u_wrs_1);
    }

    ZR_D BSDFSamplerEval EvalBSDFSampler_NoSpecTr(float3 normal, ShadingData surface, float3 wi, LOBE lobe,
        float2 u_c, float2 u_g, float2 u_d)
    {
        BSDFSamplerEval ret;
        float w_sum = 0;
        float3 target = f3(0);
        if (surface.Coated())
        {
            const bool isZ_c = lobe == COAT;
            const float3 wi_c = isZ_c ? wi : SampleCoat(surface, normal, u_c);
            surface.SetWi_Refl(wi_c, normal);
            target = Unified(surface).f;
            const float targetLum_c = Math::Luminance(target);
            const float pdf_c = CoatPdf(surface);
            const float pdf_g = GlossPdf(surface);
            const float pdf_d = !surface.metallic ? DiffusePdf(surface) : 0;
            w_sum = RT::BalanceHeuristic3(pdf_c, pdf_g, pdf_d, targetLum_c);
        }
        {
            const bool isZ_g = lobe == GLOSSY_R;
            const float3 wi_g = isZ_g ? wi : SampleGloss(surface, normal, u_g);
            surface.SetWi_Refl(wi_g, normal);
            const float3 target_g = Unified(surface).f;
            const float targetLum_g = Math::Luminance(target_g);
            const float pdf_g = GlossPdf(surface);
            const float pdf_d = !surface.metallic ? DiffusePdf(surface) : 0;
            const float pdf_c = surface.Coated() ? CoatPdf(surface) : 0;
            w_sum += RT::BalanceHeuristic3(pdf_g, pdf_d, pdf_c, targetLum_g);
            target = isZ_g ? target_g : target;
        }
        if (!surface.metallic)
        {
            float pdfUnused;
            float3 w_d = SampleDiffuse(normal, u_d, pdfUnused);
            float Fr_g;
            {
                const bool isZ_dr = lobe == DIFFUSE_R;
                const float3 wi_d = isZ_dr ? wi : w_d;
                surface.SetWi_Refl(wi_d, normal);
                BSDFEval eval = Unified(surface);
                const float3 target_dr = eval.f;
                Fr_g = eval.Fr_g.x;
                const float targetLum_dr = Math::Luminance(target_dr);
                const float pdf_d = DiffusePdf(surface);
                const float pdf_g = GlossPdf(surface);
                const float pdf_c = surface.Coated() ? CoatPdf(surface) : 0;
                w_sum += RT::BalanceHeuristic3(pdf_d, pdf_g, pdf_c, targetLum_dr);
                target = isZ_dr ? target_dr : target;
            }
            if (surface.ThinWalled())
            {
                const bool isZ_dt = lobe == DIFFUSE_T;
                const float3 target_dt = DielectricBaseDiffuseTr(surface, Fr_g);
                const float targetLum_dt = Math::Luminance(target_dt);
                const float pdf_d = DiffusePdf(surface);
                w_sum += targetLum_dt / pdf_d;
                target = isZ_dt ? target_dt : target;
            }
        }
        float targetLum = Math::Luminance(target);
        ret.bsdfOverPdf = targetLum > 0 ? target * w_sum / targetLum : f3(0);
        ret.pdf = w_sum > 0 ? targetLum / w_sum : 0;
        ret.f = target;
        return ret;
    }

    ZR_D BSDFSamplerEval EvalBSDFSampler_NoDiffuse(float3 normal, ShadingData surface, float3 wi, LOBE lobe)
    {
        float3 wh = surface.SetWi(wi, normal);
        BSDFEval eval = Unified(surface);
        float pdf_base = 1;
        BSDFSamplerEval ret;
        ret.f = eval.f;
        if (surface.Coated())
        {
            float reflectance_c = GGXReflectance_Dielectric(surface.rho, surface.coat_alpha, surface.ndotwo, surface.coat_eta);
            float pdf_coat = reflectance_c * surface.coat_weight;
            pdf_base = 1 - pdf_coat;
            if (lobe == COAT)
            {
                ret.pdf = CoatPdf(surface) * pdf_coat;
                ret.bsdfOverPdf = ret.f / ret.pdf;
                return ret;
            }
        }
        const float wh_pdf = GGXMicrofacetPdf(surface.alpha, surface.ndotwh, surface.ndotwo);
        ret.pdf = !surface.GlossSpecular() ? wh_pdf / 4.0f : (surface.ndotwh >= MIN_N_DOT_H_SPECULAR ? 1.0f : 0.0f);
        ret.pdf *= pdf_base;
        ret.bsdfOverPdf = ret.f / ret.pdf;
        if (surface.metallic || !surface.specTr || eval.tir)
            return ret;
        float targetScaleLum = Math::Luminance(f3(1.0f));
        float targetScaleOtherLum = Math::Luminance(f3(1.0f));
        float p_r = eval.Fr_g.x * (lobe == GLOSSY_R ? targetScaleLum : targetScaleOtherLum);
        p_r = p_r / (p_r + (1 - eval.Fr_g.x) * (lobe == GLOSSY_R ? targetScaleOtherLum : targetScaleLum));
        if (lobe == GLOSSY_R)
        {
            ret.bsdfOverPdf /= p_r;
            ret.pdf *= p_r;
            return ret;
        }
        ret.bsdfOverPdf = ((!surface.invalid ? 1.0f : 0.0f) * (!surface.reflection ? 1.0f : 0.0f)) *
            TranslucentTrOverPdf(surface, eval.Fr_g.x);
        ret.bsdfOverPdf *= TransmittanceToDielectricBaseTr(surface);
        ret.bsdfOverPdf *= f3(1.0f);
        ret.bsdfOverPdf /= pdf_base;
        ret.bsdfOverPdf /= (1 - p_r);
        ret.pdf = 1 - p_r;
        ret.pdf *= surface.GlossSpecular() ? (surface.ndotwh >= MIN_N_DOT_H_SPECULAR ? 1.0f : 0.0f) : wh_pdf * surface.whdotwo;
        ret.pdf *= pdf_base;
        if (!surface.GlossSpecular())
        {
            float dwh_dwi = JacobianHalfVecToIncident_Tr(surface.eta, surface.whdotwo, surface.whdotwi);
            ret.pdf *= dwh_dwi;
        }
        return ret;
    }

    ZR_D BSDFSamplerEval EvalBSDFSampler(float3 normal, const ShadingData& surface, float3 wi, LOBE lobe, RNG& rng)
    {
        float2 u_c = rng.Uniform2D();
        float2 u_g = rng.Uniform2D();
        float2 u_d = rng.Uniform2D();
        rng.Uniform(); rng.Uniform(); rng.Uniform();
        if (!surface.specTr)
            return EvalBSDFSampler_NoSpecTr(normal, surface, wi, lobe, u_c, u_g, u_d);
        return EvalBSDFSampler_NoDiffuse(normal, surface, wi, lobe);
    }

    ZR_D float BSDFSamplerPdf_NoDiffuse(float3 normal, ShadingData surface, float3 wi)
    {
        float3 wh = surface.SetWi(wi, normal);
        float pdf_base = 1;
        float pdf_c = 0;
        if (surface.Coated())
        {
            float reflectance_c = GGXReflectance_Dielectric(surface.rho, surface.coat_alpha, surface.ndotwo, surface.coat_eta);
            float pdf_coat = reflectance_c * surface.coat_weight;
            pdf_base = 1 - pdf_coat;
            if (surface.reflection)
                pdf_c = CoatPdf(surface) * pdf_coat;
        }
        const float wh_pdf = GGXMicrofacetPdf(surface.alpha, surface.ndotwh, surface.ndotwo);
        if (surface.metallic || !surface.specTr)
        {
            float pdf_gr = surface.GlossSpecular() ? (surface.ndotwh >= MIN_N_DOT_H_SPECULAR ? 1.0f : 0.0f) : wh_pdf / 4.0f;
            pdf_gr *= pdf_base;
            return surface.reflection ? pdf_c + pdf_gr : 0;
        }
        float pdf_g = surface.GlossSpecular() ? (surface.ndotwh >= MIN_N_DOT_H_SPECULAR ? 1.0f : 0.0f) : 1;
        pdf_g *= pdf_base;
        float targetScaleLum = Math::Luminance(f3(1.0f));
        float targetScaleOtherLum = Math::Luminance(f3(1.0f));
        float Fr_g = surface.Fresnel().x;
        float pdf_r = Fr_g * (surface.reflection ? targetScaleLum : targetScaleOtherLum);
        pdf_r = pdf_r / (pdf_r + (1 - Fr_g) * (surface.reflection ? targetScaleOtherLum : targetScaleLum));
        if (surface.reflection)
        {
            pdf_g *= surface.GlossSpecular() ? 1 : (wh_pdf / 4.0f);
            pdf_g *= pdf_r;
            return pdf_g + pdf_c;
        }
        pdf_g *= 1 - pdf_r;
        if (!surface.GlossSpecular())
        {
            pdf_g *= wh_pdf * surface.whdotwo;
            float dwh_dwi = JacobianHalfVecToIncident_Tr(surface.eta, surface.whdotwo, surface.whdotwi);
            pdf_g *= dwh_dwi;
        }
        return pdf_g;
    }

    ZR_D float BSDFSamplerPdf(float3 normal, ShadingData surface, float3 wi_z, RNG& rng)
    {
        if (surface.specTr)
            return BSDFSamplerPdf_NoDiffuse(normal, surface, wi_z);
        surface.SetWi(wi_z, normal);
        if (!surface.reflection && !surface.ThinWalled())
            return 0;
        BSDFEval eval_z = Unified(surface);
        float targetLum = Math::Luminance(eval_z.f);
        if (targetLum == 0)
            return 0;
        float w_sum_c, w_sum_g, w_sum_dr, w_sum_dt;
        {
            float pdf_g = GlossPdf(surface);
            float pdf_d = !surface.metallic ? DiffusePdf(surface) : 0;
            float pdf_c = surface.Coated() ? CoatPdf(surface) : 0;
            float w = surface.reflection ? RT::BalanceHeuristic3(pdf_g, pdf_d, pdf_c, targetLum) :
                (targetLum / pdf_d) * (!surface.metallic ? 1.0f : 0.0f);
            w_sum_g = w; w_sum_dr = w; w_sum_dt = w; w_sum_c = w;
        }
        if (w_sum_g == 0)
            return 0;
        float pdf_d;
        float3 wi_d = SampleDiffuse(normal, rng.Uniform2D(), pdf_d);
        float Fr_g = 0;
        if (!surface.metallic)
        {
            surface.SetWi_Refl(wi_d, normal);
            BSDFEval eval = Unified(surface);
            Fr_g = eval.Fr_g.x;
            float targetLum_dr = Math::Luminance(eval.f);
            float pdf_g = GlossPdf(surface);
            float pdf_c = surface.Coated() ? CoatPdf(surface) : 0;
            float w = RT::BalanceHeuristic3(pdf_d, pdf_g, pdf_c, targetLum_dr);
// ... 39 lines not shown
```

zetaray_b200/csrc/zr_pixel.cuh:

```cuda
#pragma once
#include "zr_rt.cuh"

namespace zr
{
struct GFlags { bool metallic, transmissive, emissive, invalid, trDepthGt0, subsurface, coated; };

ZR_D GFlags DecodeFlags(uint32_t v)
{
    GFlags r;
    r.transmissive = (v & 0x1) != 0;
    r.emissive = (v & (1 << 1)) != 0;
    r.invalid = (v & (1 << 2)) != 0;
    r.trDepthGt0 = (v & (1 << 3)) != 0;
    r.subsurface = (v & (1 << 4)) != 0;
    r.coated = (v & (1 << 5)) != 0;
    r.metallic = (v & (1 << 7)) != 0;
    return r;
}

ZR_D float DecodeIOR(float e) { return mad(e, 2.5f - 1.0f, 1.0f); }

struct FrameView
{
    zr_frame_constants fc;
// ... 5 lines not shown
inline zr_status LightingFrame(const char* pass, const zr_frame_inputs* in, uint32_t width, uint32_t height, FrameView& f)
{
    if (!in || !in->scene || !in->curr.d_core || !in->curr.d_motion_emissive || !in->curr.d_coat)
    {
        set_error("%s_render: missing scene or G-buffer", pass);
        return ZR_ERR_INVALID_ARG;
    }
    const zr_status st = check_frame_size(pass, in->frame, width, height);
    if (st != ZR_OK) return st;
    if (in->scene->dev.numEmissives == 0 || !in->scene->aliasBuilt)
    {
        set_error("%s_render: needs emissive triangles and zr_prelighting_render first (the sun/sky variants are not part of this build)", pass);
        return ZR_ERR_UNSUPPORTED;
    }
    if (in->scene->dev.sampleSetSize && !in->scene->samplesValid)
    {
        set_error("%s_render: presampling is enabled but zr_presample_emissives has not run", pass);
        return ZR_ERR_NOT_INITIALIZED;
    }
    f.fc = in->frame;
    f.core = (const uint4*)in->curr.d_core; f.depth = (const float*)in->curr.d_depth;
    f.me = (const uint2*)in->curr.d_motion_emissive; f.coat = (const uint2*)in->curr.d_coat;
    f.pcore = (const uint4*)in->prev.d_core; f.pcoat = (const uint2*)in->prev.d_coat;
    f.W = width; f.H = height;
    return ZR_OK;
}

ZR_D void AccountCost(unsigned long long* costMap, uint32_t W, uint32_t H, uint32_t x, uint32_t y, long long t0)
{
    if (costMap && threadIdx.x == 0 && x < W && y < H)
        atomicAdd(&costMap[(size_t)(y >> 5) * ((W + 31) >> 5) + (x >> 5)], (unsigned long long)(clock64() - t0));
}

struct Pixel
{
    GFlags flags; float roughness; float z; float3 pos, normal, origin; float2 lensSample;
    BSDF::ShadingData surface; float eta_next;
    float coatRoughness, coatIor;
};

ZR_D float3 row3(const float m[3][4], int r) { return f3(m[r][0], m[r][1], m[r][2]); }

ZR_D GFlags FlagsAt(const uint4* __restrict__ core, uint32_t W, int x, int y, float* roughness = nullptr)
{
    const uint32_t w = __ldg(&core[(size_t)y * W + x].w);
    if (roughness) *roughness = (float)((w >> 8) & 0xff) / 255.0f;
    return DecodeFlags(w & 0xff);
}

ZR_D Pixel LoadPixel(const FrameView& f, const SceneDev& sc, const uint4* __restrict__ core, const uint2* __restrict__ coat,
    int px, int py, bool prev, int coatX, int coatY)
{
    const zr_frame_constants& fc = f.fc;
    Pixel p;
    const uint4 c = ld128(&core[(size_t)py * f.W + px]);
    p.flags = DecodeFlags(c.w & 0xff);
    p.roughness = (float)((c.w >> 8) & 0xff) / 255.0f;
    p.z = asfloat(c.x);
    p.lensSample = f2(0, 0);
    p.origin = prev ? f3(fc.PrevViewInv[0][3], fc.PrevViewInv[1][3], fc.PrevViewInv[2][3]) : f3(fc.CameraPos[0], fc.CameraPos[1], fc.CameraPos[2]);
    if (fc.DoF)
    {
        const uint3 h = RNG::PCG3d(make_uint3((uint32_t)px, (uint32_t)py, (uint32_t)px));
        RNG rngDoF = RNG::Init(h.z, h.y, prev ? fc.FrameNum - 1 : fc.FrameNum);
        p.lensSample = Sampling::UniformSampleDiskConcentric(rngDoF.Uniform2D());
        p.lensSample = p.lensSample * fc.LensRadius;
    }
    const float2 renderDim = f2((float)f.W, (float)f.H);
    const float2 jitter = prev ? f2(fc.PrevCameraJitter[0], fc.PrevCameraJitter[1]) : f2(fc.CurrCameraJitter[0], fc.CurrCameraJitter[1]);
    const float3 bx = prev ? row3(fc.PrevView, 0) : row3(fc.CurrView, 0);
    const float3 by = prev ? row3(fc.PrevView, 1) : row3(fc.CurrView, 1);
    const float3 bz = prev ? row3(fc.PrevView, 2) : row3(fc.CurrView, 2);
    p.pos = Math::WorldPosFromScreenSpace2(f2((float)px, (float)py), renderDim, p.z, fc.TanHalfFOV, fc.AspectRatio, jitter,
        bx, by, bz, fc.DoF != 0, p.lensSample, fc.FocusDepth, p.origin);
    p.normal = Math::DecodeUnitVector(Math::DecodeUNorm2(c.y));
    const float3 baseColor = f3((float)(c.z & 0xff) / 255.0f, (float)((c.z >> 8) & 0xff) / 255.0f, (float)((c.z >> 16) & 0xff) / 255.0f);
    const float baseW = p.flags.subsurface ? (float)(c.z >> 24) / 255.0f : 0.0f;
    p.eta_next = BSDF::DEFAULT_ETA_MAT;
    if (p.flags.transmissive)
        p.eta_next = DecodeIOR((float)((c.w >> 16) & 0xff) / 255.0f);
    float coat_weight = 0; float3 coat_color = f3(0.0f); float coat_roughness = 0; float coat_ior = BSDF::DEFAULT_ETA_COAT;
    if (p.flags.coated)
    {
        const uint2 cc = __ldg(&coat[(size_t)coatY * f.W + coatX]);
        const uint32_t px_ = cc.x & 0xffff, py_ = cc.x >> 16, pz_ = cc.y & 0xffff;
        coat_weight = Math::UNorm8ToFloat((py_ >> 8) & 0xff);
        coat_roughness = Math::UNorm8ToFloat(pz_ & 0xff);
        coat_color = Math::UnpackRGB8(px_ | ((py_ & 0xff) << 16));
        coat_ior = DecodeIOR(Math::UNorm8ToFloat(pz_ >> 8));
    }
    p.coatRoughness = coat_roughness; p.coatIor = coat_ior;
    const float3 wo = normalize(p.origin - p.pos);
    p.surface = BSDF::ShadingData::Init(p.normal, wo, p.flags.metallic, p.roughness, baseColor, BSDF::ETA_AIR, p.eta_next,
        p.flags.transmissive, p.flags.trDepthGt0 ? 1.0f : 0.0f, to_half(baseW), coat_weight, coat_color, coat_roughness,
        coat_ior, sc.rho);
    return p;
}

ZR_D void WriteOutputColor(const zr_frame_constants& fc, float4* __restrict__ finalImg, size_t idx, float3 li)
{
    li = isnan3(li) ? f3(0) : li;
    if (fc.Accumulate && fc.CameraStatic && fc.NumFramesCameraStatic > 1)
    {
        const float4 prev = finalImg[idx];
        finalImg[idx] = f4(prev.x + li.x, prev.y + li.y, prev.z + li.z, prev.w);
    }
    else
        finalImg[idx] = f4(li.x, li.y, li.z, 0.0f);
}
}
```

zetaray_b200/csrc/zr_rdi.cuh:

```cuda
#pragma once
#include "zr_pixel.cuh"

namespace zr
{
namespace
{
    struct DIParams
    {
        uint32_t temporal, spatial, stochasticSpatial, extraDisocclusion, M_max; float alpha_min; uint32_t reset;
        uint32_t rowBegin, rowEnd;
        unsigned long long* costMap;
    };

    __constant__ float c_disk32[64];

struct Reservoir
{
    float w_sum, W; float3 le; uint32_t lightIdx; float2 bary; uint32_t M;
    float3 target; uint32_t lightID; float3 lightPos, lightNormal; bool doubleSided;

    static ZR_D Reservoir Init()
    {
        Reservoir r;
        r.le = f3(0); r.M = 0; r.w_sum = 0; r.W = 0; r.lightIdx = UINT32_MAX_; r.bary = f2(0, 0);
// ... 80 lines not shown
struct EmissiveData
{
    float3 wi; float t; uint32_t ID; float3 lightPos, lightNormal; bool doubleSided;
    static ZR_D EmissiveData Init(const SceneDev& sc, uint32_t lightIdx, float2 bary)
    {
        EmissiveData ret;
        const zr_emissive_tri& tri = sc.emissives[lightIdx];
        ret.ID = tri.ID;
        const float3 vtx0 = Light::Vtx0(tri);
        const float3 vtx1 = Light::DecodeEmissiveTriV1(tri);
        const float3 vtx2 = Light::DecodeEmissiveTriV2(tri);
        ret.lightPos = (1.0f - bary.x - bary.y) * vtx0 + bary.x * vtx1 + bary.y * vtx2;
        ret.lightNormal = cross(vtx1 - vtx0, vtx2 - vtx0);
        ret.lightNormal = dot(ret.lightNormal, ret.lightNormal) == 0 ? ret.lightNormal : normalize(ret.lightNormal);
        ret.doubleSided = Light::IsDoubleSided(tri);
        ret.wi = f3(0); ret.t = 0;
        return ret;
    }
    ZR_D void SetSurfacePos(float3 pos)
    {
        wi = lightPos - pos;
        t = dot(wi, wi) == 0 ? 0 : length(wi);
        wi = t == 0 ? f3(0) : wi / t;
        lightNormal = doubleSided && dot(-wi, lightNormal) < 0 ? -lightNormal : lightNormal;
    }
    ZR_D float dWdA() const
    {
        float cosThetaPrime = saturate(dot(lightNormal, -wi));
        return t == 0 ? 0 : cosThetaPrime / (t * t);
    }
};

#define ZR_PHASE() __syncthreads()
ZR_D Reservoir RIS_InitialCandidates_Sync(bool act, const SceneDev& sc, float3 pos, float3 normal, float roughness, BSDF::ShadingData surface,
    uint32_t sampleSetIdx, int numBsdfSamples, RNG& rng)
{
    Reservoir r = Reservoir::Init();
    const bool specular = surface.GlossSpecular() && (surface.metallic || surface.specTr) && (!surface.Coated() || surface.CoatSpecular());
    const int numLightSamples = !specular ? 3 : 0;
    for (int s_b = 0; s_b < 2; s_b++)
    {
        const bool go = act && (s_b < numBsdfSamples);
        BSDF::BSDFSample bsdfSample = BSDF::BSDFSample::Init();
        ZR_PHASE();
        if (go)
            bsdfSample = BSDF::SampleBSDF_NoDiffuse(normal, surface, rng);
        ZR_PHASE();
        BSDFHitInfo hitInfo;
        hitInfo.hit = false;
        if (go)
            hitInfo = FindClosestHitDI(sc, pos, normal, bsdfSample.wi, surface.Transmissive());
        ZR_PHASE();
        if (go)
        {
            float3 wi = bsdfSample.wi;
            float pdf_w = bsdfSample.pdf;
            float w_b = 0;
            float3 le = f3(0), lightNormal = f3(0), target = f3(0);
            uint32_t emissiveID = UINT32_MAX_;
            bool doubleSided = false;
            if (hitInfo.hit)
            {
                const zr_emissive_tri& emissive = sc.emissives[hitInfo.emissiveTriIdx];
                le = Light::Le_EmissiveTriangle(emissive);
                const float3 vtx0 = Light::Vtx0(emissive);
                const float3 vtx1 = Light::DecodeEmissiveTriV1(emissive);
                const float3 vtx2 = Light::DecodeEmissiveTriV2(emissive);
// ... 46 lines not shown
            wi = isZero ? wi : wi / t;
            dwdA = isZero ? 0 : saturate(dot(lightSample.normal, -wi)) / (t * t);
            surface.SetWi(wi, normal);
            facing = dot(lightSample.normal, -wi) > 0;
            if (facing)
                target = le * BSDF::Unified(surface).f * dwdA;
        }
        ZR_PHASE();
        if (go && facing && (dot(target, target) > 0))
            target *= Visibility_Segment(sc, pos, wi, t, normal, lightID, surface.Transmissive()) ? 1.0f : 0.0f;
        ZR_PHASE();
        if (go)
        {
            const float denom = (float)numLightSamples * pdf_light + (float)numBsdfSamples * BSDF::BSDFSamplerPdf_NoDiffuse(normal, surface, wi) * dwdA;
            const float m_l = denom > 0 ? 1.0f / denom : 0;
            const float w_l = m_l * Math::Luminance(target);
            if (r.Update(w_l, le, emissiveIdx, lightSample.bary, rng))
            {
                r.target = target; r.lightID = lightID; r.lightNormal = lightSample.normal; r.lightPos = lightSample.pos; r.doubleSided = doubleSided;
            }
        }
    }
    float targetLum = Math::Luminance(r.target);
    r.W = targetLum > 0.0f ? r.w_sum / targetLum : 0.0f;
    return r;
}

ZR_D bool PlaneHeuristicDI(float3 samplePos, float3 currNormal, float3 currPos, float linearDepth, float tolerance = 1e-1f)
{
    float planeDist = dot(currNormal, samplePos - currPos);
    return fabsf(planeDist) <= tolerance * linearDepth;
}

struct TemporalCandidate { BSDF::ShadingData surface; float3 pos, normal; int px, py; bool valid; };

ZR_D TemporalCandidate FindTemporalCandidate(const FrameView& f, const SceneDev& sc, float3 pos, float3 normal, float roughness, const BSDF::ShadingData& surface, float2 prevUV)
{
    TemporalCandidate c; c.valid = false; c.px = c.py = 0; c.pos = c.normal = f3(0);
    if (prevUV.x < 0.0f || prevUV.y < 0.0f || prevUV.x > 1.0f || prevUV.y > 1.0f) return c;
    const float2 renderDim = f2((float)f.W, (float)f.H);
    float2 pp = prevUV * renderDim;
    int ppx = (int)pp.x, ppy = (int)pp.y;
    float prevRoughness;
    GFlags prevFlags = FlagsAt(f.pcore, f.W, ppx, ppy, &prevRoughness);
    if (prevFlags.invalid || prevFlags.emissive || (fabsf(prevRoughness - roughness) > 0.15f) ||
        (prevFlags.metallic != surface.metallic) || (prevFlags.transmissive != surface.specTr))
        return c;
    Pixel p = LoadPixel(f, sc, f.pcore, f.pcoat, ppx, ppy, true, ppx, ppy);
    if (!PlaneHeuristicDI(p.pos, normal, pos, p.z))
        return c;
    c.surface = p.surface; c.px = ppx; c.py = ppy; c.pos = p.pos; c.normal = p.normal; c.valid = true;
    return c;
}

ZR_D void TemporalResample1_Sync(bool act, const SceneDev& sc, float3 pos, float3 normal, const BSDF::ShadingData& surface, TemporalCandidate candidate,
    const zr_rdi_reservoir* prevRes, uint32_t W, Reservoir& r_curr, RNG& rng)
{
    Reservoir r_prev = Reservoir::Init();
    if (act)
        r_prev = Reservoir::Load(prevRes[(size_t)candidate.py * W + candidate.px]);
    const uint32_t newM = r_curr.M + r_prev.M;
    const bool doCtT = act && (r_curr.w_sum != 0);
    float3 wi_offset = f3(0);
    float t_offset = 0, targetLum_offset = 0;
    float3 target_offset = f3(0);
    if (doCtT)
    {
        wi_offset = r_curr.lightPos - candidate.pos;
        const bool isZero = dot(wi_offset, wi_offset) == 0;
        t_offset = isZero ? 0 : length(wi_offset);
        wi_offset = isZero ? wi_offset : wi_offset / t_offset;
        candidate.surface.SetWi(wi_offset, candidate.normal);
        float3 lightNormal = r_curr.lightNormal;
        if (r_curr.doubleSided && dot(-wi_offset, lightNormal) < 0)
            lightNormal = -lightNormal;
        float cosThetaPrime = saturate(dot(lightNormal, -wi_offset));
        const float dwdA = isZero ? 0 : cosThetaPrime / (t_offset * t_offset);
        target_offset = r_curr.le * dwdA;
    }
    ZR_PHASE();
    if (doCtT)
    {
        target_offset *= BSDF::Unified(candidate.surface).f;
        targetLum_offset = Math::Luminance(target_offset);
    }
    ZR_PHASE();
    if (doCtT)
    {
        if (targetLum_offset > 0)
            targetLum_offset *= Visibility_Segment(sc, candidate.pos, wi_offset, t_offset, candidate.normal, r_curr.lightID,
                candidate.surface.Transmissive()) ? 1.0f : 0.0f;
        const float numerator = (float)r_curr.M * Math::Luminance(r_curr.target);
        const float denom = numerator + (float)r_prev.M * targetLum_offset * 1.0f;
        const float m_curr = denom > 0 ? numerator / denom : 0;
        r_curr.w_sum *= m_curr;
    }
    const bool doTtC = act && (r_prev.lightIdx != UINT32_MAX_);
    EmissiveData prevEmissive;
    BSDF::ShadingData surfaceWi = surface;
    float3 target_curr = f3(0);
    if (doTtC)
    {
        prevEmissive = EmissiveData::Init(sc, r_prev.lightIdx, r_prev.bary);
        prevEmissive.SetSurfacePos(pos);
        const float dwdA = prevEmissive.dWdA();
        surfaceWi.SetWi(prevEmissive.wi, normal);
        target_curr = r_prev.le * dwdA;
    }
    ZR_PHASE();
    if (doTtC)
        target_curr *= BSDF::Unified(surfaceWi).f;
    ZR_PHASE();
    if (doTtC)
    {
        if (dot(target_curr, target_curr) > 0)
            target_curr *= Visibility_Segment(sc, pos, prevEmissive.wi, prevEmissive.t, normal, prevEmissive.ID, surfaceWi.Transmissive()) ? 1.0f : 0.0f;
        const float targetLum_curr = Math::Luminance(target_curr);
        if (targetLum_curr > 0)
        {
            const float targetLum_prev = r_prev.W > 0 ? r_prev.w_sum / r_prev.W : 0;
            const float numerator = (float)r_prev.M * targetLum_prev;
            const float denom = numerator / 1.0f + (float)r_curr.M * targetLum_curr;
            const float m_prev = denom > 0 ? numerator / denom : 0;
            const float w_prev = m_prev * targetLum_curr * r_prev.W;
            if (r_curr.Update(w_prev, r_prev.le, r_prev.lightIdx, r_prev.bary, rng))
                r_curr.target = target_curr;
        }
    }
    if (act)
    {
        float targetLum = Math::Luminance(r_curr.target);
        r_curr.W = targetLum > 0.0f ? r_curr.w_sum / targetLum : 0.0f;
        r_curr.M = newM;
    }
}

struct PairwiseMIS
{
    Reservoir r_s; float m_c; float M_s; uint32_t k;
    static ZR_D PairwiseMIS Init(uint32_t numStrategies, const Reservoir& r_c)
    {
        PairwiseMIS ret;
        ret.r_s = Reservoir::Init(); ret.m_c = 1.0f; ret.M_s = to_half((float)r_c.M); ret.k = numStrategies;
        return ret;
    }
    ZR_D float Compute_m_i(const Reservoir& r_c, const Reservoir& r_i, float targetLum, float jacobian) const
    {
        const float p_i_y_i = r_i.W > 0 ? r_i.w_sum / r_i.W : 0;
        const float p_c_y_i = targetLum;
        float numerator = (float)r_i.M * p_i_y_i;
        float denom = (numerator / jacobian) + ((float)r_c.M / (float)k) * p_c_y_i;
        return denom > 0 ? numerator / denom : 0;
    }
    ZR_D void Update_m_c(const Reservoir& r_c, const Reservoir& r_i, float targetLum, float jacobian)
    {
        const float p_i_y_c = targetLum;
        const float p_c_y_c = Math::Luminance(r_c.target);
        const float numerator = (float)r_i.M * p_i_y_c * jacobian;
        const float denom = numerator + ((float)r_c.M / (float)k) * p_c_y_c;
        m_c += 1 - (numerator / denom);
    }
    ZR_D void Stream_Sync(bool act, const SceneDev& sc, const Reservoir& r_c, float3 pos_c, float3 normal_c, BSDF::ShadingData surface_c, const Reservoir& r_i,
        float3 pos_i, float3 normal_i, BSDF::ShadingData surface_i, RNG& rng)
    {
        float3 target_c_y_i = f3(0), target_i_y_c = f3(0.0f);
        float m_i = 0;
        const bool has_i = act && (r_i.lightIdx != UINT32_MAX_);
        const float jacobian_i_to_c = 1;
        EmissiveData emissive_i;
        if (has_i)
        {
            emissive_i = EmissiveData::Init(sc, r_i.lightIdx, r_i.bary);
            emissive_i.SetSurfacePos(pos_c);
            float dwdA = emissive_i.dWdA();
            surface_c.SetWi(emissive_i.wi, normal_c);
            target_c_y_i = r_i.le * dwdA;
        }
        ZR_PHASE();
        if (has_i && (dot(target_c_y_i, target_c_y_i) > 0))
            target_c_y_i *= Visibility_Segment(sc, pos_c, emissive_i.wi, emissive_i.t, normal_c, emissive_i.ID, surface_c.Transmissive()) ? 1.0f : 0.0f;
        ZR_PHASE();
        if (has_i)
        {
            target_c_y_i *= BSDF::Unified(surface_c).f;
            const float targetLum = Math::Luminance(target_c_y_i);
            m_i = Compute_m_i(r_c, r_i, targetLum, jacobian_i_to_c);
        }
        float jacobian_c_to_i = 0;
        const bool has_c = act && (r_c.lightIdx != UINT32_MAX_);
        float3 wi_i = f3(0);
        float t_i = 0;
        if (has_c)
        {
            jacobian_c_to_i = 1;
            wi_i = r_c.lightPos - pos_i;
            const bool isZero = dot(wi_i, wi_i) == 0;
// ... 79 lines not shown
```

zetaray_b200/csrc/zr_rpt.cuh:

```cuda
#pragma once
#include "zr_rt.cuh"

namespace zr
{
namespace RPT
{
    using BSDF::LOBE;
    using BSDF::ShadingData;
    using Light::TYPE;

    struct Reconnection
    {
        static constexpr uint32_t EMPTY = 0xf;
        float3 x_k;
        uint32_t ID;
        uint32_t meshIdx;
        float partialJacobian;
        float3 w_k_lightNormal_w_sky;
        float lightPdf;
        uint32_t seed_replay;
        uint32_t seed_nee;
        float dwdA;
        float3 L;
        uint32_t k;
// ... 199 lines not shown
                s.lightPdf = rc.lightPdf;
            }
        }
        ZR_D void WriteReservoirData(zr_rpt_reservoir& s, uint32_t M_max) const
        {
            uint32_t k = rc.Empty() ? rc.k : (rc.k > 2 ? rc.k : 2) - 2;
            uint32_t m = M < M_max ? M : M_max;
            s.meta = (s.meta & 0xffffff00u) | ((k | (m << 4)) & 0xff);
            s.w_sum = w_sum; s.W = W;
        }
    };

    ZR_D bool CanReconnect(float alpha_lobe_k_min_1, float alpha_lobe_k, LOBE lobe_k_min_1, LOBE lobe_k, float alpha_min)
    {
        if ((alpha_lobe_k_min_1 < alpha_min) || (alpha_lobe_k < alpha_min)) return false;
        if ((lobe_k_min_1 == BSDF::GLOSSY_T) && (lobe_k == BSDF::GLOSSY_T)) return false;
        return true;
    }

    struct DirectLightingEstimate
    {
        float3 ld, le, wi, pos, normal;
        float pdf_solidAngle, dwdA;
        TYPE lt; LOBE lobe; uint32_t ID; float pdf_light; bool twoSided;
        static ZR_D DirectLightingEstimate Init()
        {
            DirectLightingEstimate r;
            r.ld = f3(0); r.le = f3(0); r.wi = f3(0); r.pdf_solidAngle = 0; r.dwdA = 1; r.lt = Light::NONE;
            r.ID = UINT32_MAX_; r.pos = f3(0); r.pdf_light = 0; r.twoSided = true; r.normal = f3(0); r.lobe = BSDF::DIFFUSE_R;
            return r;
        }
    };

    ZR_D bool IsSpecularSurface(const ShadingData& surface)
    {
        return surface.GlossSpecular() && (surface.metallic || surface.specTr) && (!surface.Coated() || surface.CoatSpecular());
    }

#define ZR_PHASE() __syncthreads()

    struct RaySetup { float3 o; float tmin, tmax; bool go; };

    ZR_D RaySetup SetupClosestEmissive(float3 pos, float3 normal, float3 wi, bool transmissive)
    {
        RaySetup rs; rs.o = f3(0); rs.tmin = 0; rs.tmax = FLT_MAX_; rs.go = true;
        const bool wiBackface = dot(normal, wi) <= 0;
        if (wiBackface)
        {
            if (transmissive) normal = -normal;
            else { rs.go = false; return rs; }
        }
        rs.o = RTU::OffsetRayRTG(pos, normal);
        rs.tmin = wiBackface ? T_MIN_TR_RAY : T_MIN_REFL_RAY;
        return rs;
    }
    ZR_D HitEmissive FinishClosestEmissive(const SceneDev& sc, const RaySetup& rs, const RayHit& h, float3 wi)
    {
        HitEmissive ret;
        ret.hit = false;
        ret.emissiveTriIdx = UINT32_MAX_;
        ret.t = 0; ret.geoIdx = 0; ret.primIdx = 0; ret.bary = f2(0, 0); ret.lightPos = f3(0);
        if (rs.go && h.hit)
        {
            ret.hit = true;
            ret.bary = h.bary;
            ret.t = h.t;
            ret.geoIdx = __ldg(&sc.triMesh[h.tri]);
// ... 26 lines not shown
        Hit ret;
        ret.hit = false;
        ret.ID = UINT32_MAX_;
        ret.t = 0; ret.uv = f2(0, 0); ret.normal = f3(0); ret.meshIdx = 0; ret.matIdx = 0;
        return ret;
    }
    ZR_D Hit FinishClosest(const SceneDev& sc, const RaySetup& rs, const RayHit& h)
    {
        if (!(rs.go && h.hit))
            return MissHit();
        const uint32_t mesh = __ldg(&sc.triMesh[h.tri]);
        return HitAttributes(sc, mesh, h.tri - __ldg(&sc.meshFirstTri[mesh]), h.bary, h.t);
    }
    ZR_D RaySetup SetupSegment(float3 origin, float3 wi, float rayT, float3 normal, uint32_t triID, bool transmissive)
    {
        RaySetup rs; rs.o = f3(0); rs.tmin = 0; rs.tmax = 0; rs.go = false;
        if (triID == UINT32_MAX_) return rs;
        if (rayT < 1e-6f) return rs;
        const float ndotwi = dot(normal, wi);
        if (ndotwi == 0) return rs;
        const bool wiBackface = ndotwi < 0;
        if (wiBackface)
        {
            if (transmissive) normal = -normal;
            else return rs;
        }
        rs.o = RTU::OffsetRayRTG(origin, normal);
        rs.tmin = 3e-6f;
        rs.tmax = Math::PrevFloat32(rayT * 0.999f - Math::NextFloat32(rs.tmin));
        rs.go = true;
        return rs;
    }

    ZR_D DirectLightingEstimate NEE_Bsdf_Finish(const SceneDev& sc, float3 pos, const ShadingData& surface, int nextBounce,
        int maxNumBounces, BSDF::BSDFSample& bsdfSample, const HitEmissive& hitInfo)
    {
        DirectLightingEstimate ret = DirectLightingEstimate::Init();
        const bool specular = IsSpecularSurface(surface);
        const int numLightSamples = specular ? 0 : 1;
        const float wiPdf = bsdfSample.pdf;
        const float3 wi = bsdfSample.wi;
        const float3 f = bsdfSample.f;
        if (hitInfo.HitWasEmissive())
        {
            const zr_emissive_tri& emissive = sc.emissives[hitInfo.emissiveTriIdx];
            const float3 le = Light::Le_EmissiveTriangle(emissive);
            const float3 vtx0 = Light::Vtx0(emissive);
            const float3 vtx1 = Light::DecodeEmissiveTriV1(emissive);
            const float3 vtx2 = Light::DecodeEmissiveTriV2(emissive);
            float3 lightNormal = cross(vtx1 - vtx0, vtx2 - vtx0);
            float twoArea = length(lightNormal);
            lightNormal = dot(lightNormal, lightNormal) == 0 ? f3(0.0f) : lightNormal / twoArea;
            lightNormal = Light::IsDoubleSided(emissive) && (dot(-wi, lightNormal) < 0) ? -lightNormal : lightNormal;
            float lightPdf = 0;
            if (!specular)
            {
                const float lightSourcePdf = numLightSamples > 0 ? sc.aliasTable[hitInfo.emissiveTriIdx].CachedP_Orig : 0;
                lightPdf = twoArea > 0 ? lightSourcePdf * (2.0f / twoArea) : 0;
            }
            float dwdA = saturate(dot(lightNormal, -wi)) / (hitInfo.t * hitInfo.t);
            float wiPdf_area = wiPdf * dwdA;
            float3 ld = le * f * dwdA;
            ret.ld = specular ? (wiPdf_area > 0 ? ld / wiPdf_area : f3(0)) : RT::PowerHeuristic(wiPdf_area, lightPdf, ld);
            ret.le = le; ret.wi = wi; ret.pdf_solidAngle = wiPdf; ret.dwdA = dwdA; ret.ID = emissive.ID;
            ret.pos = mad(hitInfo.t, wi, pos);
            ret.normal = lightNormal; ret.pdf_light = lightPdf; ret.lobe = bsdfSample.lobe; ret.lt = Light::EMISSIVE;
            ret.twoSided = Light::IsDoubleSided(emissive);
        }
        if (nextBounce >= maxNumBounces)
            bsdfSample.bsdfOverPdf = f3(0);
        return ret;
    }

    struct NeeLightState { DirectLightingEstimate ret; float3 ld; float t, lightPdf, dwdA; bool facing; };

    ZR_D NeeLightState NEE_Emissive_Begin(const SceneDev& sc, float3 pos, float3 normal, ShadingData& surface, uint32_t sampleSetIdx, RNG& rng)
    {
        NeeLightState st;
        st.ret = DirectLightingEstimate::Init();
        st.ret.lt = Light::EMISSIVE;
        st.ret.lobe = BSDF::ALL;
        const Light::LightSample lightSample = Light::SampleLight(sc, pos, sampleSetIdx, rng, true);
        const float3 le = lightSample.le;
        st.lightPdf = lightSample.pdf;
        st.t = length(lightSample.pos - pos);
        const float3 wi = (lightSample.pos - pos) / st.t;
        st.facing = (dot(lightSample.normal, -wi) > 0) && (st.t > 0);
        st.ld = f3(0); st.dwdA = 0;
        if (st.facing)
        {
            st.dwdA = saturate(dot(lightSample.normal, -wi)) / (st.t * st.t);
            surface.SetWi(wi, normal);
            st.ld = le * BSDF::Unified(surface).f * st.dwdA;
            st.ret.le = le; st.ret.wi = wi; st.ret.ID = lightSample.ID;
            st.ret.pos = lightSample.pos; st.ret.normal = lightSample.normal; st.ret.twoSided = lightSample.twoSided;
        }
        return st;
    }
    ZR_D DirectLightingEstimate NEE_Emissive_Finish(const NeeLightState& st, float bsdfPdf)
    {
        DirectLightingEstimate ret = st.ret;
        if (st.facing)
        {
            ret.ld = RT::PowerHeuristic(st.lightPdf, bsdfPdf, st.ld);
            ret.pdf_solidAngle = st.lightPdf / st.dwdA; ret.dwdA = st.dwdA; ret.pdf_light = st.lightPdf;
        }
        return ret;
    }

    struct OffsetPath { float3 target; float partialJacobian; bool surfKMin1Tramsmissive; };

    struct OffsetPathContext
    {
        float3 throughput, pos, normal;
        ShadingData surface;
        float eta_curr, eta_next;
        RNG rngReplay;

        static ZR_D OffsetPathContext Init()
        {
            OffsetPathContext c;
            c.throughput = f3(0); c.pos = f3(0); c.normal = f3(0);
            c.surface = ShadingData::InitEmpty();
            c.eta_curr = BSDF::ETA_AIR; c.eta_next = BSDF::DEFAULT_ETA_MAT; c.rngReplay.State = 0;
            return c;
        }
        ZR_D OffsetPathContext Quantize() const
        {
            OffsetPathContext ctx = Init();
            ctx.throughput = f3(to_half(throughput.x), to_half(throughput.y), to_half(throughput.z));
            if (dot(ctx.throughput, ctx.throughput) == 0)
                return ctx;
            ctx.pos = pos;
            ctx.normal = Math::DecodeOct32(Math::EncodeOct32u(normal));
            ctx.eta_curr = mad(Math::UNorm8ToFloat(Math::FloatToUNorm8((eta_curr - 1.0f) / 1.5f)), 1.5f, 1.0f);
            ctx.eta_next = mad(Math::UNorm8ToFloat(Math::FloatToUNorm8((eta_next - 1.0f) / 1.5f)), 1.5f, 1.0f);
            float3 wo = Math::DecodeOct32(Math::EncodeOct32u(surface.wo));
            float roughness = Math::UNorm8ToFloat(Math::FloatToUNorm8(!surface.GlossSpecular() ? sqrtf(surface.alpha) : 0));
            float3 baseColor = Math::UnpackRGB8(Math::Float3ToRGB8(surface.baseColor_Fr0_TrCol));
            bool metallic = surface.metallic;
            bool specTr = surface.specTr;
            float trDepth = surface.trDepth > 0 ? 1.0f : 0.0f;
            bool coated = surface.Coated();
            float subsurface = Math::UNorm8ToFloat(Math::FloatToUNorm8(surface.subsurface));
            float eta_next_ = ctx.eta_curr == BSDF::ETA_AIR ? ctx.eta_next : BSDF::ETA_AIR;
            float coat_weight = 0; float3 coat_color = f3(0.0f); float coat_roughness = 0; float coat_ior = BSDF::DEFAULT_ETA_COAT;
            if (coated)
            {
                coat_weight = Math::UNorm8ToFloat(Math::FloatToUNorm8(surface.coat_weight));
                coat_color = Math::UnpackRGB8(Math::Float3ToRGB8(surface.coat_color));
                coat_roughness = Math::UNorm8ToFloat(Math::FloatToUNorm8(!surface.CoatSpecular() ? sqrtf(surface.coat_alpha) : 0));
                float coat_eta = surface.coat_eta >= 1.0f ? surface.coat_eta : 1.0f / surface.coat_eta;
                coat_ior = mad(Math::UNorm8ToFloat(Math::FloatToUNorm8((coat_eta - 1.0f) / 1.5f)), 1.5f, 1.0f);
            }
            ctx.surface = ShadingData::Init(ctx.normal, wo, metallic, roughness, baseColor, ctx.eta_curr, eta_next_, specTr,
                trDepth, to_half(subsurface), coat_weight, coat_color, coat_roughness, coat_ior, surface.rho);
            return ctx;
        }
    };

    ZR_D OffsetPathContext Replay_kGt2_Sync(bool act, const SceneDev& sc, float3 pos, float3 normal, float ior, const ShadingData& surface,
        const Reconnection& rc, float alpha_min)
    {
        OffsetPathContext ctx = OffsetPathContext::Init();
        BSDF::BSDFSample bsdfSample = BSDF::BSDFSample::Init();
        const int numBounces = (int)rc.k - 2;
        int bounce = 0;
        bool go = act, inTranslucentMedium = false;
        float alpha_lobe_prev = 0;
        LOBE lobe_prev = BSDF::DIFFUSE_R;
        if (go)
        {
            ctx.pos = pos; ctx.normal = normal; ctx.surface = surface;
            ctx.rngReplay = RNG::InitSeed(rc.seed_replay);
            ctx.eta_curr = BSDF::ETA_AIR; ctx.eta_next = ior;
            ctx.throughput = f3(1);
            bsdfSample = BSDF::SampleBSDF(ctx.normal, ctx.surface, ctx.rngReplay);
            if (dot(bsdfSample.bsdfOverPdf, bsdfSample.bsdfOverPdf) == 0) { ctx.throughput = f3(0); go = false; }
            else
            {
                ctx.throughput = bsdfSample.bsdfOverPdf;
                ctx.eta_curr = dot(ctx.normal, bsdfSample.wi) < 0 ? ctx.eta_next : BSDF::ETA_AIR;
                inTranslucentMedium = ctx.eta_curr != BSDF::ETA_AIR;
                alpha_lobe_prev = BSDF::LobeAlpha(ctx.surface, bsdfSample.lobe);
                lobe_prev = bsdfSample.lobe;
            }
        }
        while (__syncthreads_or(go))
        {
            RaySetup rs; rs.go = false;
            RayHit h; h.hit = false;
            if (go)
            {
                rs = SetupClosest(ctx.pos, ctx.normal, bsdfSample.wi, ctx.surface.Transmissive());
                if (rs.go)
                    h = TraceClosest(sc, rs.o, bsdfSample.wi, rs.tmin, FLT_MAX_);
            }
            ZR_PHASE();
            if (go)
            {
                Hit hitInfo = FinishClosest(sc, rs, h);
                if (!hitInfo.hit) { ctx.throughput = f3(0); go = false; }
                else if (!GetMaterialData(sc, -bsdfSample.wi, ctx.eta_curr, hitInfo, ctx.surface, ctx.eta_next)) { ctx.throughput = f3(0); go = false; }
                else
                {
                    ctx.pos = mad(hitInfo.t, bsdfSample.wi, ctx.pos);
                    ctx.normal = hitInfo.normal;
                    bounce++;
                    if (inTranslucentMedium && (ctx.surface.trDepth > 0))
                    {
                        float3 c = ctx.surface.baseColor_Fr0_TrCol;
                        float3 extCoeff = f3(-zr_logf(c.x), -zr_logf(c.y), -zr_logf(c.z)) / ctx.surface.trDepth;
                        ctx.throughput *= f3(zr_expf(-hitInfo.t * extCoeff.x), zr_expf(-hitInfo.t * extCoeff.y), zr_expf(-hitInfo.t * extCoeff.z));
                    }
                    if (bounce >= numBounces)
                        go = false;
                }
            }
            ZR_PHASE();
            if (go)
            {
                bsdfSample = BSDF::SampleBSDF(ctx.normal, ctx.surface, ctx.rngReplay);
                if (dot(bsdfSample.bsdfOverPdf, bsdfSample.bsdfOverPdf) == 0) { ctx.throughput = f3(0); go = false; }
                else
                {
                    const float alpha_lobe = BSDF::LobeAlpha(ctx.surface, bsdfSample.lobe);
                    if (CanReconnect(alpha_lobe_prev, alpha_lobe, lobe_prev, bsdfSample.lobe, alpha_min)) { ctx.throughput = f3(0); go = false; }
                    else
                    {
                        const bool transmitted = dot(ctx.normal, bsdfSample.wi) < 0;
                        ctx.eta_curr = transmitted ? (ctx.eta_curr == BSDF::ETA_AIR ? ctx.eta_next : BSDF::ETA_AIR) : ctx.eta_curr;
                        ctx.throughput *= bsdfSample.bsdfOverPdf;
                        inTranslucentMedium = ctx.eta_curr != BSDF::ETA_AIR;
                        alpha_lobe_prev = alpha_lobe;
                        lobe_prev = bsdfSample.lobe;
                    }
                }
            }
        }
        return ctx;
    }

    template<int CASE = 0>
    ZR_D OffsetPath Shift2_Sync(bool act, const SceneDev& sc, float3 pos, float3 normal, float ior, const ShadingData& surface,
        const Reconnection& rc, const OffsetPathContext* replayed, float alpha_min)
    {
        OffsetPath ret; ret.target = f3(0); ret.partialJacobian = 0; ret.surfKMin1Tramsmissive = false;
        OffsetPathContext ctx = OffsetPathContext::Init();
        const bool case1 = CASE == 0 ? rc.IsCase1() : CASE == 1, case2 = CASE == 0 ? rc.IsCase2() : CASE == 2,
            case3 = CASE == 0 ? rc.IsCase3() : CASE == 3;
        bool go = act;
        if (go)
        {
            ctx.pos = pos; ctx.normal = normal; ctx.surface = surface;
            ctx.rngReplay = RNG::InitSeed(rc.seed_replay);
            ctx.eta_curr = BSDF::ETA_AIR; ctx.eta_next = ior;
            ctx.throughput = f3(1);
            const int numBounces = (int)rc.k - 2;
            if (numBounces != 0)
            {
                ctx = *replayed;
                if (dot(ctx.throughput, ctx.throughput) == 0)
                    go = false;
                else
                {
                    ctx.rngReplay.State = 0;
                    for (int bounce = 0; bounce < numBounces; bounce++)
                    {
                        ctx.rngReplay.Uniform4D();
                        ctx.rngReplay.Uniform4D();
                        ctx.rngReplay.Uniform();
                    }
                }
            }
            if (go)
                ret.surfKMin1Tramsmissive = ctx.surface.specTr;
        }
        bool step = go && !case3;
        float3 w_k_min_1 = f3(0);
        if (step)
        {
// ... 15 lines not shown
            else if (BSDF::LobeAlpha(ctx.surface, rc.lobe_k_min_1) < alpha_min)
                go = false;
        }
        ZR_PHASE();
        BSDF::BSDFSamplerEval eval; eval.pdf = 0; eval.bsdfOverPdf = f3(0); eval.f = f3(0);
        if (step)
        {
            eval = BSDF::EvalBSDFSampler(ctx.normal, ctx.surface, w_k_min_1, rc.lobe_k_min_1, ctx.rngReplay);
            if (dot(eval.bsdfOverPdf, eval.bsdfOverPdf) == 0) { step = false; go = false; }
        }
        ZR_PHASE();
        RaySetup rs; rs.go = false;
        RayHit h; h.hit = false;
        if (step)
        {
            rs = SetupClosest(ctx.pos, ctx.normal, w_k_min_1, ctx.surface.Transmissive());
            if (rs.go)
                h = TraceClosest(sc, rs.o, w_k_min_1, rs.tmin, FLT_MAX_);
        }
        ZR_PHASE();
        if (step)
        {
            Hit hitInfo = FinishClosest(sc, rs, h);
            if (!hitInfo.hit || (hitInfo.ID != rc.ID)) { step = false; go = false; }
            else
            {
                const float3 y_k = mad(hitInfo.t, w_k_min_1, ctx.pos);
                const bool transmitted = dot(ctx.normal, w_k_min_1) < 0;
                ctx.eta_curr = transmitted ? (ctx.eta_curr == BSDF::ETA_AIR ? ctx.eta_next : BSDF::ETA_AIR) : ctx.eta_curr;
                const bool inTranslucentMedium = ctx.eta_curr != BSDF::ETA_AIR;
                if (!GetMaterialData(sc, -w_k_min_1, ctx.eta_curr, hitInfo, ctx.surface, ctx.eta_next)) { step = false; go = false; }
                else
                {
                    if (inTranslucentMedium && (ctx.surface.trDepth > 0))
                    {
                        float3 c = ctx.surface.baseColor_Fr0_TrCol;
                        float3 extCoeff = f3(-zr_logf(c.x), -zr_logf(c.y), -zr_logf(c.z)) / ctx.surface.trDepth;
                        ctx.throughput *= f3(zr_expf(-hitInfo.t * extCoeff.x), zr_expf(-hitInfo.t * extCoeff.y), zr_expf(-hitInfo.t * extCoeff.z));
                    }
                    float partialJacobian = eval.pdf;
                    partialJacobian *= fabsf(dot(-w_k_min_1, hitInfo.normal));
                    partialJacobian /= (hitInfo.t * hitInfo.t);
                    ctx.pos = y_k;
                    ctx.normal = hitInfo.normal;
                    ctx.throughput *= eval.bsdfOverPdf;
                    ret.partialJacobian = partialJacobian;
                    if (partialJacobian == 0) go = false;
                }
            }
        }
        const bool nee = go && !case1;
        ShadingData surfWi = ctx.surface;
        float3 wiE = rc.w_k_lightNormal_w_sky;
        float3 nrmE = ctx.normal;
        LOBE lobeE = rc.lobe_k;
        float dwdA = rc.dwdA, tE = 0, lightPdfE = rc.lightPdf;
        float3 ld = f3(0);
        RNG rngNEE = RNG::InitSeed(rc.seed_nee);
        bool needBsdf = nee;
        if (nee && case3)
        {
            wiE = rc.x_k - ctx.pos;
            tE = length(wiE);
            wiE /= tE;
            const float3 lightNormal = rc.w_k_lightNormal_w_sky;
            const bool twoSided = rc.lightPdf > 0;
            lightPdfE = fabsf(rc.lightPdf);
            nrmE = ctx.pos;
            lobeE = rc.lobe_k_min_1;
            const float wiDotLightNormal = dot(lightNormal, -wiE);
            dwdA = fabsf(wiDotLightNormal) / (tE * tE);
            needBsdf = (wiDotLightNormal > 0) || twoSided;
        }
        if (nee)
            surfWi.SetWi(wiE, nrmE);
        ZR_PHASE();
        if (nee && needBsdf)
            ld = rc.L * BSDF::Unified(surfWi).f * dwdA;
        ZR_PHASE();
        if (nee && case3 && (dot(ld, ld) > 0))
        {
            const RaySetup seg = SetupSegment(ctx.pos, wiE, tE, nrmE, rc.ID, surfWi.Transmissive());
            const bool visible = seg.go ? !TraceAnyExcept(sc, seg.o, wiE, seg.tmin, seg.tmax, rc.ID) : false;
            ld *= visible ? 1.0f : 0.0f;
        }
// ... 46 lines not shown
```

zetaray_b200/csrc/zr_rpt_io.cuh:

```cuda
#pragma once
#include "zr_rpt.cuh"
#include "zr_pixel.cuh"

namespace zr
{
struct RptParams
{
    uint32_t maxNonTrBounces, maxGlossyTrBounces, russianRoulette, M_max_temporal, M_max_spatial;
    uint32_t boilingSuppression, sortSpatial;
    float alpha_min;
    uint32_t temporalResample, resetTemporal, spatialFlag;
    uint32_t rowBegin, rowEnd;
    unsigned long long* costMap;
};

namespace
{
    using namespace RPT;

    ZR_D void LoadRecord(const zr_rpt_reservoir* __restrict__ p, zr_rpt_reservoir& r)
    {
        const uint4* q = reinterpret_cast<const uint4*>(p);
        uint4 v[4] = { q[0], q[1], q[2], q[3] };
        memcpy(&r, v, 64);
// ... 77 lines not shown
        return fabsf(dot(normal, prevPos - pos)) <= th * linearDepth;
    }

    ZR_D void XkToPrev(const SceneDev& sc, Reconnection& rc)
    {
        const zr_mesh_instance md = LoadInstance(sc, rc.meshIdx);
        const float4 q_curr = normalize(Math::DecodeNormalized4(md.Rotation));
        const float3 T = f3(md.Translation[0], md.Translation[1], md.Translation[2]);
        const float3 x_local = Math::InverseTransformTRS(rc.x_k, T, q_curr, h3(md.Scale));
        const float3 prevTranslation = T - h3(md.dTranslation);
        const float4 q_prev = normalize(Math::DecodeNormalized4(md.PrevRotation));
        rc.x_k = Math::TransformTRS(x_local, prevTranslation, q_prev, h3(md.PrevScale));
    }
    ZR_D void XkToCurr(const SceneDev& sc, Reconnection& rc)
    {
        const zr_mesh_instance md = LoadInstance(sc, rc.meshIdx);
        const float3 T = f3(md.Translation[0], md.Translation[1], md.Translation[2]);
        const float3 dT = h3(md.dTranslation);
        const float3 prevTranslation = T - dT;
        const float4 q_prev = normalize(Math::DecodeNormalized4(md.PrevRotation));
        const float3 prevScale = h3(md.PrevScale), scale = h3(md.Scale);
        const float3 x_local = Math::InverseTransformTRS(rc.x_k, prevTranslation, q_prev, prevScale);
        const float4 q_curr = normalize(Math::DecodeNormalized4(md.Rotation));
        rc.x_k = Math::TransformTRS(x_local, T, q_curr, scale);
        const float4 dRot = f4(q_prev.x - q_curr.x, q_prev.y - q_curr.y, q_prev.z - q_curr.z, q_prev.w - q_curr.w);
        const float3 dScale = prevScale - scale;
        rc.x_k_in_motion = dot(dT, dT) > 0;
        rc.x_k_in_motion = rc.x_k_in_motion || dot(dRot, dRot) > 0;
        rc.x_k_in_motion = rc.x_k_in_motion || dot(dScale, dScale) > 0;
    }

    struct PrevHit { float alpha_lobe; float3 wi; float pdf; BSDF::LOBE lobe; };

    ZR_D void MaybeSetCase2OrCase3(int pathVertex, float3 pos, float3 normal, float t, uint32_t ID, uint32_t meshIdx,
        const BSDF::ShadingData& surface, const PrevHit& prevHit, const DirectLightingEstimate& ls, uint32_t seed_nee,
        Reconnection& rc, float alpha_min)
    {
        const float alpha_lobe_direct = BSDF::LobeAlpha(surface, ls.lobe);
        if (rc.Empty() && CanReconnect(prevHit.alpha_lobe, alpha_lobe_direct, prevHit.lobe, ls.lobe, alpha_min))
        {
            rc.SetCase2(pathVertex, pos, t, normal, ID, meshIdx, prevHit.wi, prevHit.lobe, prevHit.pdf, ls.wi, ls.lobe,
                ls.pdf_solidAngle, ls.lt, ls.pdf_light, ls.le, seed_nee, ls.dwdA);
        }
        if (rc.Empty() && (alpha_lobe_direct >= alpha_min))
        {
            rc.SetCase3(pathVertex + 1, ls.pos, ls.lt, ls.lobe, ls.ID, ls.le, ls.normal, ls.pdf_solidAngle, ls.pdf_light,
                ls.dwdA, ls.wi, ls.twoSided, seed_nee);
        }
    }

}
}
```

zetaray_b200/csrc/zr_rpt_shift.cuh:

```cuda
#pragma once
#include "zr_rpt_spatial.h"

namespace zr
{
namespace
{
    using namespace RPT;
#ifndef ZR_SHIFT_THREADS
#define ZR_SHIFT_THREADS 512
#endif
#ifndef ZR_SHIFT_MINBLOCKS
#define ZR_SHIFT_MINBLOCKS 1
#endif
    constexpr int SHIFT_THREADS = ZR_SHIFT_THREADS, SHIFT_MINBLOCKS = ZR_SHIFT_MINBLOCKS;
    constexpr uint32_t NO_ITEM = 0xffffffffu;

    ZR_D uint32_t ShiftClass(uint32_t meta)
    {
        const uint32_t kMin2 = meta & 0xf;
        const uint32_t lt_k = (meta >> 14) & 3, lt_k1 = (meta >> 16) & 3;
        const uint32_t c = lt_k1 != 0 ? 1u : (lt_k != 0 ? 2u : 0u);
        return c * 2 + (kMin2 > 0 ? 1u : 0u);
    }


    template<int CASE, bool REPLAY, bool TEMPORAL>
    __global__ void __launch_bounds__(SHIFT_THREADS, SHIFT_MINBLOCKS) k_shift(SceneDev sc, FrameView f, RptParams prm,
        const zr_rpt_reservoir* __restrict__ resIn, const zr_rpt_reservoir* __restrict__ resPrev, const uint16_t* __restrict__ neighbor,
        const uint32_t* __restrict__ queue, uint32_t* __restrict__ counters, uint32_t cls, ShiftResult* __restrict__ out)
    {
        __shared__ uint32_t s_base;
        const uint32_t total = counters[cls];
        for (;;)
        {
            __syncthreads();
            if (threadIdx.x == 0) s_base = atomicAdd(&counters[8 + cls], (uint32_t)SHIFT_THREADS);
            __syncthreads();
            const uint32_t base = s_base;
            if (base >= total) break;
            const bool act = base + threadIdx.x < total;
            int x = 0, y = 0;
            uint32_t dir = 0;
            bool replayOk = act;
            Reservoir r = Reservoir::Init();
            Pixel p, pr;
            if (act)
            {
                const uint32_t item = __ldg(&queue[base + threadIdx.x]);
                x = (int)(item & 0xffff); y = (int)((item >> 16) & 0x3fff); dir = item >> 31;
                zr_rpt_reservoir rec;
                if (!TEMPORAL)
                {
                    int nx = 0, ny = 0;
                    NeighborOf(f, neighbor, x, y, nx, ny);
                    LoadRecord(dir == 0 ? &resIn[(size_t)y * f.W + x] : &resIn[(size_t)ny * f.W + nx], rec);
                    r = Reservoir::Load_NonReconnection(rec);
                    r.rc.x_k_in_motion = false;
                    r.Load_Reconnection(rec);
                    if (dir == 0) p = LoadPixel(f, sc, f.core, f.coat, nx, ny, false, x, y);
                    else p = LoadPixel(f, sc, f.core, f.coat, x, y, false, x, y);
                    if (REPLAY)
                    {
                        if (dir == 0) pr = LoadPixel(f, sc, f.core, f.coat, nx, ny, false, nx, ny);
                        else pr = p;
                    }
                }
                else
                {
                    replayOk = ((item >> 30) & 1) != 0;
                    int ppx = 0, ppy = 0;
                    PrevPixel(f, x, y, ppx, ppy);
                    LoadRecord(dir == 0 ? &resIn[(size_t)y * f.W + x] : &resPrev[(size_t)ppy * f.W + ppx], rec);
                    r = Reservoir::Load_NonReconnection(rec);
                    r.Load_Reconnection(rec);
                    if (r.rc.IsCase1() || r.rc.IsCase2())
                    {
                        if (dir == 0) XkToPrev(sc, r.rc);
                        else XkToCurr(sc, r.rc);
                    }
                    if (dir == 0) p = LoadPixel(f, sc, f.pcore, f.pcoat, ppx, ppy, true, x, y);
                    else p = LoadPixel(f, sc, f.core, f.coat, x, y, false, x, y);
                    if (REPLAY) pr = p;
                }
            }
            OffsetPathContext ctx = OffsetPathContext::Init();
            if (REPLAY)
            {
                ZR_PHASE();
                ctx = Replay_kGt2_Sync(act && replayOk, sc, pr.pos, pr.normal, pr.eta_next, pr.surface, r.rc, prm.alpha_min);
                if (act && replayOk)
                    ctx = ctx.Quantize();
            }
            const OffsetPath shift = Shift2_Sync<CASE>(act, sc, p.pos, p.normal, p.eta_next, p.surface, r.rc, &ctx, prm.alpha_min);
            if (act)
            {
                ShiftResult* o = &out[(size_t)y * f.W + x];
                if (dir == 0)
                    *reinterpret_cast<float2*>(&o->ctsTargetLum) = f2(Math::Luminance(shift.target), shift.partialJacobian);
                else if (TEMPORAL)
                    st128(o, make_uint4(asuint(shift.target.x), asuint(shift.target.y), asuint(shift.target.z), asuint(shift.partialJacobian)));
                else
                {
                    const float J = shift.partialJacobian;
                    const float Jenc = J > 0 ? (shift.surfKMin1Tramsmissive ? -J : J) : 0.0f;
                    st128(o, make_uint4(asuint(shift.target.x), asuint(shift.target.y), asuint(shift.target.z), asuint(Jenc)));
                }
            }
        }
    }

    template<bool TEMPORAL>
    zr_status LaunchShifts(const SpatialQueued& q, const ShiftStreams& ss, const SceneDev& sc, const FrameView& f, const RptParams& prm,
        const zr_rpt_reservoir* resIn, const zr_rpt_reservoir* resPrev, const uint16_t* neighbor, cudaStream_t stream)
    {
        const uint32_t grid = (uint32_t)ss.numSMs * SHIFT_MINBLOCKS;
        cudaStream_t s1 = ss.aux[0], s2 = ss.aux[1];
        ZR_CUDA(cudaEventRecord(ss.evFork, stream));
        ZR_CUDA(cudaStreamWaitEvent(s1, ss.evFork, 0));
        ZR_CUDA(cudaStreamWaitEvent(s2, ss.evFork, 0));
#define ZR_LAUNCH_SHIFT(CASE, REPLAY, CLS, STREAM) \
        k_shift<CASE, REPLAY, TEMPORAL><<<grid, SHIFT_THREADS, 0, STREAM>>>(sc, f, prm, resIn, resPrev, neighbor, q.d_queue + (size_t)(CLS) * q.capacity, \
            q.d_counters, CLS, q.d_shift); \
        zr::count_launch()
        ZR_LAUNCH_SHIFT(1, false, 0, stream);
        ZR_LAUNCH_SHIFT(2, false, 2, s1);
        ZR_LAUNCH_SHIFT(3, false, 4, s2);
        ZR_LAUNCH_SHIFT(1, true, 1, s1);
        ZR_LAUNCH_SHIFT(2, true, 3, s2);
        ZR_LAUNCH_SHIFT(3, true, 5, stream);
#undef ZR_LAUNCH_SHIFT
        ZR_CUDA(cudaEventRecord(ss.evJoin[0], s1));
        ZR_CUDA(cudaEventRecord(ss.evJoin[1], s2));
        ZR_CUDA(cudaStreamWaitEvent(stream, ss.evJoin[0], 0));
        ZR_CUDA(cudaStreamWaitEvent(stream, ss.evJoin[1], 0));
        return ZR_OK;
    }

    ZR_D void AppendItems(const uint32_t cls[2], const uint32_t item[2], uint32_t* __restrict__ queue, uint32_t* __restrict__ counters,
        uint32_t capacity, uint32_t* s_count, uint32_t* s_base)
    {
        const uint32_t lane = threadIdx.x & 31;
        uint32_t offs[2] = { 0, 0 };
        const uint32_t lt = (1u << lane) - 1;
#pragma unroll
        for (uint32_t c = 0; c < SpatialQueued::NUM_CLASSES; c++)
        {
            const uint32_t m0 = __ballot_sync(0xffffffffu, cls[0] == c), m1 = __ballot_sync(0xffffffffu, cls[1] == c);
            const uint32_t n0 = __popc(m0), n = n0 + __popc(m1);
            uint32_t base = 0;
            if (n && lane == 0) base = atomicAdd(&s_count[c], n);
            base = __shfl_sync(0xffffffffu, base, 0);
            if (cls[0] == c) offs[0] = base + __popc(m0 & lt);
            if (cls[1] == c) offs[1] = base + n0 + __popc(m1 & lt);
        }
// ... 12 lines not shown
```

zetaray_b200/csrc/zr_rpt_spatial.h:

```cpp
#pragma once
#include <cuda.h>
#include "zr_planes.h"
#include "zr_rpt_io.cuh"

namespace zr
{
struct ShiftResult
{
    float stcTarget[3];
    float stcJacobian;
    float ctsTargetLum;
    float ctsJacobian;
    uint32_t pad[2];
};
static_assert(sizeof(ShiftResult) == 32, "ShiftResult is two 128-bit words");

struct ShiftStreams
{
    int numSMs = 0;
    cudaStream_t aux[2] = { nullptr, nullptr };
    cudaEvent_t evFork = nullptr, evJoin[2] = { nullptr, nullptr };
    ShiftStreams() = default;
    ShiftStreams(const ShiftStreams&) = delete;
    ShiftStreams& operator=(const ShiftStreams&) = delete;
    ~ShiftStreams();
    zr_status Init();
};

struct SpatialQueued
{
    static constexpr int NUM_CLASSES = 6;
    Planes planes{ "zr_indirect_pass" };
    uint32_t width = 0, height = 0;
    uint32_t* d_queue = nullptr;
    uint32_t* d_counters = nullptr;
    ShiftResult* d_shift = nullptr;
    uint8_t* d_flags = nullptr;
    size_t capacity = 0;
    const void* mapBase[2] = { nullptr, nullptr };
    CUtensorMap* d_maps = nullptr;
    bool swizzled = false;

    zr_status Build(uint32_t w, uint32_t h, const zr_rpt_reservoir* res0, const zr_rpt_reservoir* res1);
    zr_status Run(const ShiftStreams& ss, const SceneDev& sc, const FrameView& f, const RptParams& prm, const zr_rpt_reservoir* resIn,
        zr_rpt_reservoir* resOut, const float4* target, float4* finalImg, const uint16_t* neighbor, const uint16_t* threadMap, cudaStream_t stream);
    zr_status RunTemporal(const ShiftStreams& ss, const SceneDev& sc, const FrameView& f, const RptParams& prm, zr_rpt_reservoir* resCurr,
        const zr_rpt_reservoir* resPrev, float4* target, float4* finalImg, cudaStream_t stream);
};
}
```

zetaray_b200/csrc/zr_rt.cuh:

```cuda
#pragma once
#include "zr_scene.cuh"
#include "zr_bsdf.cuh"

namespace zr
{
constexpr uint32_t UINT32_MAX_ = 0xffffffffu;

namespace RTU
{
    ZR_D float3 OffsetRayRTG(float3 pos, float3 geometricNormal)
    {
        const float origin = 1.0f / 32.0f;
        const float float_scale = 1.0f / 65536.0f;
        const float int_scale = 256.0f;
        int ofx = (int)(int_scale * geometricNormal.x), ofy = (int)(int_scale * geometricNormal.y), ofz = (int)(int_scale * geometricNormal.z);
        auto adj = [](float p, int of) { return asfloat((uint32_t)((int)asuint(p) + ((p < 0) ? -of : of))); };
        float3 p_i = f3(adj(pos.x, ofx), adj(pos.y, ofy), adj(pos.z, ofz));
        return f3(fabsf(pos.x) < origin ? pos.x + float_scale * geometricNormal.x : p_i.x,
                  fabsf(pos.y) < origin ? pos.y + float_scale * geometricNormal.y : p_i.y,
                  fabsf(pos.z) < origin ? pos.z + float_scale * geometricNormal.z : p_i.z);
    }
}

constexpr float T_MIN_REFL_RAY = 1e-6f;
// ... 106 lines not shown
    if (ndotwi == 0) return false;
    bool wiBackface = ndotwi < 0;
    if (wiBackface)
    {
        if (transmissive) normal = -normal;
        else return false;
    }
    const float3 adjustedOrigin = RTU::OffsetRayRTG(origin, normal);
    const float tMin = 3e-6f;
    const float tMax = Math::PrevFloat32(rayT * 0.999f - Math::NextFloat32(tMin));
    return !TraceAnyExcept(sc, adjustedOrigin, wi, tMin, tMax, triID);
}

ZR_D bool Visibility_Segment_Precise(const SceneDev& sc, float3 origin, float3 wi, float rayT, float3 normal, uint32_t triID,
    bool transmissive)
{
    if (triID == UINT32_MAX_) return false;
    if (rayT < 1e-6f) return false;
    float ndotwi = dot(normal, wi);
    if (ndotwi == 0) return false;
    bool wiBackface = ndotwi < 0;
    if (wiBackface)
    {
        if (transmissive) normal = -normal;
        else return false;
    }
    const float3 adjustedOrigin = RTU::OffsetRayRTG(origin, normal);
    const RayHit h = TraceClosest(sc, adjustedOrigin, wi, 3e-6f, rayT);
    if (h.hit)
        return triID == TriID(sc, h.tri);
    return true;
}

ZR_D bool GetMaterialData(const SceneDev& sc, float3 wo, float eta_curr, Hit& hitInfo, BSDF::ShadingData& surface, float& eta)
{
    const zr_material mat = LoadMaterial(sc, hitInfo.matIdx);
    const bool hitBackface = dot(wo, hitInfo.normal) < 0;
    eta = BSDF::DEFAULT_ETA_MAT;
    if (!Mat::DoubleSided(mat) && hitBackface)
        return false;
    if (Mat::DoubleSided(mat) && hitBackface)
        hitInfo.normal = -hitInfo.normal;
    float3 baseColor = Mat::GetBaseColorFactor(mat);
    float metallic = Mat::Metallic(mat) ? 1.0f : 0.0f;
    float roughness = Mat::GetSpecularRoughness(mat);
    bool tr = Mat::Transmissive(mat);
    eta = Mat::GetSpecularIOR(mat);
    float trDepth = tr ? Mat::GetTransmissionDepth(mat) : 0;
    float eta_next = eta_curr == BSDF::ETA_AIR ? eta : BSDF::ETA_AIR;
    float subsurface = Mat::ThinWalled(mat) ? to_half(Mat::GetSubsurface(mat)) : 0;
    float coat_weight = Mat::GetCoatWeight(mat);
    float3 coat_color = Mat::GetCoatColor(mat);
    float coat_roughness = Mat::GetCoatRoughness(mat);
    float coat_ior = Mat::GetCoatIOR(mat);
    surface = BSDF::ShadingData::Init(hitInfo.normal, wo, metallic >= 0.9f, roughness, baseColor, eta_curr, eta_next, tr,
        trDepth, subsurface, coat_weight, coat_color, coat_roughness, coat_ior, sc.rho);
    return true;
}

namespace Light
{
    enum TYPE : uint32_t { NONE = 0, SUN = 1, SKY = 2, EMISSIVE = 3 };
    ZR_D TYPE TypeFromValue(uint32_t x) { return x <= 2 ? (TYPE)x : EMISSIVE; }

    ZR_D float3 DecodeEmissiveTriV1(const zr_emissive_tri& tri)
    {
        float2 v = f2((float)tri.V0V1[0] / 65535.0f, (float)tri.V0V1[1] / 65535.0f);
        float3 decoded = Math::DecodeUnitVector(v);
        return mad(decoded, zr_f16_to_f32(tri.EdgeLengths[0]), f3(tri.Vtx0[0], tri.Vtx0[1], tri.Vtx0[2]));
    }
    ZR_D float3 DecodeEmissiveTriV2(const zr_emissive_tri& tri)
    {
        float2 v = f2((float)tri.V0V2[0] / 65535.0f, (float)tri.V0V2[1] / 65535.0f);
        float3 decoded = Math::DecodeUnitVector(v);
        return mad(decoded, zr_f16_to_f32(tri.EdgeLengths[1]), f3(tri.Vtx0[0], tri.Vtx0[1], tri.Vtx0[2]));
    }
    ZR_D bool IsDoubleSided(const zr_emissive_tri& tri) { return tri.PackedA & (1u << 25); }
    ZR_D float3 Vtx0(const zr_emissive_tri& tri) { return f3(tri.Vtx0[0], tri.Vtx0[1], tri.Vtx0[2]); }

    ZR_D float3 Le_EmissiveTriangle(const zr_emissive_tri& tri)
    {
        const float3 emissiveFactor = Math::UnpackRGB8(tri.PackedA);
        const float emissiveStrength = zr_f16_to_f32((uint16_t)(tri.PackedB >> 16));
        float3 le = emissiveFactor * emissiveStrength;
        if (Math::Luminance(le) == 0)
            return f3(0.0f);
        return le;
    }
// ... 126 lines not shown
```

zetaray_b200/csrc/zr_scene.cuh:

```cuda
#pragma once
#include "zr_common.cuh"
#include "zr_bvh.h"

namespace zr
{
struct SceneDev
{
    const zr_vertex* vertices;
    const uint32_t* indices;
    const zr_mesh_instance* instances;
    const zr_material* materials;
    const zr_emissive_tri* emissives;
    const zr_alias_entry* aliasTable;
    const uint4* nodes;
    const float4* tris;
    const uint32_t* triMesh;
    const uint32_t* meshFirstTri;
    const uint16_t* rho;
    uint32_t numInstances;
    uint32_t numEmissives;
    uint32_t numTris;
    const zr_presampled_tri* sampleSets;
    uint32_t numSampleSets, sampleSetSize;
    const zr_voxel_sample* lvg;
// ... 224 lines not shown
}

ZR_D float3 h3(const uint16_t h[3]) { return f3(zr_f16_to_f32(h[0]), zr_f16_to_f32(h[1]), zr_f16_to_f32(h[2])); }

struct VertexD { float3 pos; float2 uv; uint32_t normal; uint32_t tangent; };
ZR_D VertexD LoadVertex(const SceneDev& sc, uint32_t idx)
{
    const uint32_t* p = reinterpret_cast<const uint32_t*>(sc.vertices + idx);
    VertexD v;
    v.pos = f3(asfloat(__ldg(p)), asfloat(__ldg(p + 1)), asfloat(__ldg(p + 2)));
    v.uv = f2(asfloat(__ldg(p + 3)), asfloat(__ldg(p + 4)));
    v.normal = __ldg(p + 5);
    v.tangent = __ldg(p + 6);
    return v;
}

struct SceneHostInfo { uint32_t numNodes, numTris, maxDepth, bytes, maxStack; };
}

struct zr_scene
{
    zr::SceneDev dev{};
    zr::SceneHostInfo info{};
    void* allocs[16] = { 0 };
    int numAllocs = 0;
    zr_alias_entry* d_alias = nullptr;
    float* d_power = nullptr;
    uint32_t* d_aliasScratch = nullptr;
    bool aliasBuilt = false;
    zr_presampled_tri* d_sampleSets = nullptr;
    bool samplesValid = false;
    zr_voxel_sample* d_lvg = nullptr;
    bool lvgValid = false;
};
```

Measured before the change: 286.7.

## Specialize shading kernels on scene material features to drop unused BSDF paths

Scans the scene's materials at creation time for coat, transmission and thin-walled subsurface features. Makes ShadingData and the pixel, path-tracing, DI and shift kernels templates over a feature mask, and launches a MF_NONE instantiation when no such features exist. The aim is to let the compiler remove the coat, transmission and subsurface code paths, cutting registers and instructions. This doubles the number of kernel instantiations, and correctness relies on the host-side feature scan matching what the device would otherwise compute.

```diff
diff --git a/include/zr_abi.h b/include/zr_abi.h
--- a/include/zr_abi.h
+++ b/include/zr_abi.h
@@ -232,6 +232,10 @@
 ZR_API zr_status zr_scene_create(const zr_scene_desc* desc, zr_scene** out);
 ZR_API void zr_scene_destroy(zr_scene* scene);
 ZR_API zr_status zr_scene_bvh_stats(const zr_scene* scene, uint32_t out[4]);
+#define ZR_MATERIAL_COAT         0x1u
+#define ZR_MATERIAL_TRANSMISSION 0x2u
+#define ZR_MATERIAL_THIN_WALLED  0x4u
+ZR_API zr_status zr_scene_material_features(const zr_scene* scene, uint32_t* out);
 
 ZR_API zr_status zr_bvh_build_host(const float* h_world_tris, uint32_t num_tris, void* h_nodes, uint32_t node_capacity,
     uint32_t* h_leaf_order, uint32_t out_info[4]);
diff --git a/zetaray_b200/csrc/rdi.cu b/zetaray_b200/csrc/rdi.cu
--- a/zetaray_b200/csrc/rdi.cu
+++ b/zetaray_b200/csrc/rdi.cu
@@ -11,10 +11,12 @@
 #ifndef ZR_RDI_THREADS
 #define ZR_RDI_THREADS 512
 #endif
+    template<uint32_t MF>
     __global__ void ZR_LB(ZR_RDI_THREADS) k_di_temporal(SceneDev sc, FrameView f, DIParams prm, zr_rdi_reservoir* __restrict__ resCurr,
         const zr_rdi_reservoir* __restrict__ resPrev, uint2* __restrict__ target, float4* __restrict__ finalImg, uint32_t dispX, uint32_t dispY,
         const uint32_t* __restrict__ order)
     {
+        using SD = BSDF::ShadingDataT<MF>;
         const zr_frame_constants& fc = f.fc;
         uint2 sg = make_uint2(0, 0);
         const uint32_t groupFlat = order[blockIdx.x] * (ZR_RDI_THREADS / 64) + (threadIdx.x >> 6);
@@ -40,14 +42,14 @@
                 act = false;
             }
         }
-        Pixel p;
-        p.surface = BSDF::ShadingData::InitEmpty();
+        PixelT<SD> p;
+        p.surface = SD::InitEmpty();
         p.pos = f3(0); p.normal = f3(0); p.roughness = 0;
         RNG rng_thread; rng_thread.State = 0;
         int numBsdfSamples = 0;
         if (act)
         {
-            p = LoadPixel(f, sc, f.core, f.coat, x, y, false, x, y);
+            p = LoadPixel<SD>(f, sc, f.core, f.coat, x, y, false, x, y);
             rng_thread = RNG::Init(x, y, fc.FrameNum);
             numBsdfSamples = (!p.surface.GlossSpecular() && p.roughness < 0.3f) ? 2 : 1;
         }
@@ -57,8 +59,8 @@
         if (prm.temporal)
         {
             float2 motionVec = f2(0, 0);
-            TemporalCandidate tc; tc.valid = false; tc.px = tc.py = 0; tc.pos = tc.normal = f3(0);
-            tc.surface = BSDF::ShadingData::InitEmpty();
+            TemporalCandidateT<SD> tc; tc.valid = false; tc.px = tc.py = 0; tc.pos = tc.normal = f3(0);
+            tc.surface = SD::InitEmpty();
             ZR_PHASE();
             if (act)
             {
@@ -89,10 +91,12 @@
             WriteFinal(fc, finalImg, idx, r.target * r.W);
     }
 
+    template<uint32_t MF>
     __global__ void ZR_LB(ZR_RDI_THREADS) k_di_spatial(SceneDev sc, FrameView f, DIParams prm, const zr_rdi_reservoir* __restrict__ resCurr,
         const uint2* __restrict__ target, float4* __restrict__ finalImg, uint32_t dispX, uint32_t dispY,
         const uint32_t* __restrict__ order)
     {
+        using SD = BSDF::ShadingDataT<MF>;
         const zr_frame_constants& fc = f.fc;
         uint2 sg = make_uint2(0, 0);
         const uint32_t groupFlat = order[blockIdx.x] * (ZR_RDI_THREADS / 64) + (threadIdx.x >> 6);
@@ -114,14 +118,14 @@
                 active = false;
             }
         }
-        Pixel p;
-        p.surface = BSDF::ShadingData::InitEmpty();
+        PixelT<SD> p;
+        p.surface = SD::InitEmpty();
         p.pos = f3(0); p.normal = f3(0); p.roughness = 0; p.z = 0;
         Reservoir r = Reservoir::Init();
         bool disoccluded = false;
         if (active)
         {
-            p = LoadPixel(f, sc, f.core, f.coat, x, y, false, x, y);
+            p = LoadPixel<SD>(f, sc, f.core, f.coat, x, y, false, x, y);
             zr_rdi_reservoir rec;
             LoadRdi(&resCurr[idx], rec);
             r = Reservoir::Load(rec);
@@ -172,7 +176,7 @@
             float rough_i;
             const GFlags flags_i = FlagsAt(f.core, f.W, qx, qy, &rough_i);
             if (flags_i.invalid || flags_i.emissive) continue;
-            const Pixel pi = LoadPixel(f, sc, f.core, f.coat, qx, qy, false, qx, qy);
+            const PixelT<SD> pi = LoadPixel<SD>(f, sc, f.core, f.coat, qx, qy, false, qx, qy);
             bool valid = PlaneHeuristicDI(pi.pos, p.normal, p.pos, p.z);
             valid = valid && (fabsf(rough_i - p.roughness) < 0.15f);
             if (!valid) continue;
@@ -185,20 +189,20 @@
             const bool go = active && (i < k);
             if (!__syncthreads_or(go))
                 break;
-            Pixel pi;
+            PixelT<SD> pi;
             pi.normal = f3(0);
-            BSDF::ShadingData surface_i = BSDF::ShadingData::InitEmpty();
+            SD surface_i = SD::InitEmpty();
             Reservoir r_spatial = Reservoir::Init();
             float3 pos_i = f3(0);
             if (go)
             {
-                pi = LoadPixel(f, sc, f.core, f.coat, spx[i], spy[i], false, spx[i], spy[i]);
+                pi = LoadPixel<SD>(f, sc, f.core, f.coat, spx[i], spy[i], false, spx[i], spy[i]);
                 const uint4 c = ld128(&f.core[(size_t)spy[i] * f.W + spx[i]]);
                 const float3 bc = f3((float)(c.z & 0xff) / 255.0f, (float)((c.z >> 8) & 0xff) / 255.0f, (float)((c.z >> 16) & 0xff) / 255.0f);
                 const float bw = pi.flags.subsurface ? (float)(c.z >> 24) / 255.0f : 0.0f;
                 pos_i = samplePos[i];
                 const float3 wo_i = normalize(pi.origin - pos_i);
-                surface_i = BSDF::ShadingData::Init(pi.normal, wo_i, pi.flags.metallic, pi.roughness, bc, BSDF::ETA_AIR,
+                surface_i = SD::Init(pi.normal, wo_i, pi.flags.metallic, pi.roughness, bc, BSDF::ETA_AIR,
                     pi.eta_next, pi.flags.transmissive, 0.0f, to_half(bw), pi.surface.coat_weight, pi.surface.coat_color,
                     pi.coatRoughness, pi.coatIor, sc.rho);
                 zr_rdi_reservoir recN;
@@ -295,14 +299,15 @@
         st = strip.Schedule(width, height, 8, 8, ZR_RDI_THREADS / 64);
         if (st != ZR_OK) return st;
         const BlockSchedule& sched = strip.sched;
+        const bool plain = (in->scene->materialFeatures & BSDF::MF_ALL) == 0;
         ZR_PROF("k_di_temporal", stream);
-        k_di_temporal<<<sched.count, ZR_RDI_THREADS, 0, stream>>>(in->scene->dev, f, prm, sz.d_res[cur], sz.d_res[1 - cur], sz.d_target, sz.d_final, dispX, dispY, sched.d_order);
+        (plain ? k_di_temporal<BSDF::MF_NONE> : k_di_temporal<BSDF::MF_ALL>)<<<sched.count, ZR_RDI_THREADS, 0, stream>>>(in->scene->dev, f, prm, sz.d_res[cur], sz.d_res[1 - cur], sz.d_target, sz.d_final, dispX, dispY, sched.d_order);
         ZR_LAUNCH_CHECK();
         strip.Exchange(sz.d_res[cur], width, height, 32u, stream);
         if (doSpatial)
         {
             ZR_PROF("k_di_spatial", stream);
-            k_di_spatial<<<sched.count, ZR_RDI_THREADS, 0, stream>>>(in->scene->dev, f, prm, sz.d_res[cur], sz.d_target, sz.d_final, dispX, dispY, sched.d_order);
+            (plain ? k_di_spatial<BSDF::MF_NONE> : k_di_spatial<BSDF::MF_ALL>)<<<sched.count, ZR_RDI_THREADS, 0, stream>>>(in->scene->dev, f, prm, sz.d_res[cur], sz.d_target, sz.d_final, dispX, dispY, sched.d_order);
             ZR_LAUNCH_CHECK();
         }
         isTemporalReservoirValid = true;
diff --git a/zetaray_b200/csrc/rpt.cu b/zetaray_b200/csrc/rpt.cu
--- a/zetaray_b200/csrc/rpt.cu
+++ b/zetaray_b200/csrc/rpt.cu
@@ -22,9 +22,11 @@
     static_assert(sizeof(PtParked) % 4 == 0 && (sizeof(PtParked) / 4) % 2 == 1, "PtParked must be an odd number of words");
     constexpr size_t PT_SMEM_BYTES = (size_t)ZR_PT_THREADS * sizeof(PtParked);
 
+    template<uint32_t MF>
     __global__ void ZR_LB(ZR_PT_THREADS) k_pathtrace(SceneDev sc, FrameView f, RptParams prm, zr_rpt_reservoir* __restrict__ res,
         float4* __restrict__ target, float4* __restrict__ finalImg, uint32_t dispX, uint32_t dispY, const uint32_t* __restrict__ order)
     {
+        using SD = BSDF::ShadingDataT<MF>;
         extern __shared__ PtParked s_ptParked[];
         const zr_frame_constants& fc = f.fc;
         const long long t0 = clock64();
@@ -48,7 +50,7 @@
             }
         }
         float3 pos = f3(0), normal = f3(0), li = f3(0), throughput = f3(0), throughput_k = f3(1), tr = f3(1);
-        BSDF::ShadingData surface;
+        SD surface;
         BSDF::BSDFSample bsdfSample = BSDF::BSDFSample::Init();
         HitEmissive nextHit;
         nextHit.hit = false;
@@ -68,7 +70,7 @@
 
         if (inBounds)
         {
-            const Pixel p = LoadPixel(f, sc, f.core, f.coat, px.x, px.y, false, px.x, px.y);
+            const PixelT<SD> p = LoadPixel<SD>(f, sc, f.core, f.coat, px.x, px.y, false, px.x, px.y);
             rngGroup = RNG::Init4(sg.x, sg.y, fc.FrameNum, 1);
             const uint3 state = RNG::PCG3d(make_uint3(px.x, px.y, fc.FrameNum));
             rngReplay = RNG::InitSeed(state.x);
@@ -113,7 +115,7 @@
                     prevBsdfSamplePdf = bsdfSample.pdf;
                     prevBsdfSampleLobe = bsdfSample.lobe;
                     tr = f3(1);
-                    if (inTranslucentMedium && (surface.trDepth > 0))
+                    if (inTranslucentMedium && surface.TrDepthGt0())
                     {
                         const float3 c = surface.baseColor_Fr0_TrCol;
                         const float3 extCoeff = f3(-zr_logf(c.x), -zr_logf(c.y), -zr_logf(c.z)) / surface.trDepth;
@@ -158,7 +160,7 @@
                 if (lightSample)
                 {
                     seed_nee = rngThread.State;
-                    BSDF::ShadingData surfNee = surface;
+                    SD surfNee = surface;
                     nee = NEE_Emissive_Begin(sc, pos, hitInfo.normal, surfNee, sampleSetIdx, rngThread);
                 }
             }
@@ -175,7 +177,7 @@
                 float bsdfPdf = 0;
                 if (nee.facing && dot(nee.ld, nee.ld) > 0)
                 {
-                    BSDF::ShadingData surfNee = surface;
+                    SD surfNee = surface;
                     surfNee.SetWi(nee.ret.wi, hitInfo.normal);
                     bsdfPdf = BSDF::BSDFSamplerPdf(hitInfo.normal, surfNee, nee.ret.wi, rngThread);
                     bsdfPdf *= nee.dwdA;
@@ -493,17 +495,21 @@
 
     zr_status Setup()
     {
-        ZR_CUDA(cudaFuncSetAttribute(zr::k_pathtrace, cudaFuncAttributeMaxDynamicSharedMemorySize, (int)zr::PT_SMEM_BYTES));
-        int ptBlocks = 0;
-        ZR_CUDA(cudaOccupancyMaxActiveBlocksPerMultiprocessor(&ptBlocks, zr::k_pathtrace, ZR_PT_THREADS, zr::PT_SMEM_BYTES));
-        if (ptBlocks < 1)
-        {
-            zr::set_error("zr_indirect_pass: k_pathtrace (%d threads, %zu B shared) cannot be resident", ZR_PT_THREADS, zr::PT_SMEM_BYTES);
-            return ZR_ERR_UNSUPPORTED;
-        }
-        const size_t ptSmem = (size_t)ptBlocks * (zr::PT_SMEM_BYTES + 1024);
-        ZR_CUDA(cudaFuncSetAttribute(zr::k_pathtrace, cudaFuncAttributePreferredSharedMemoryCarveout,
-            (int)((ptSmem * 100 + 228 * 1024 - 1) / (228 * 1024))));
+        decltype(&zr::k_pathtrace<zr::BSDF::MF_ALL>) const kernels[2] = { zr::k_pathtrace<zr::BSDF::MF_NONE>, zr::k_pathtrace<zr::BSDF::MF_ALL> };
+        for (const auto kernel : kernels)
+        {
+            ZR_CUDA(cudaFuncSetAttribute(kernel, cudaFuncAttributeMaxDynamicSharedMemorySize, (int)zr::PT_SMEM_BYTES));
+            int ptBlocks = 0;
+            ZR_CUDA(cudaOccupancyMaxActiveBlocksPerMultiprocessor(&ptBlocks, kernel, ZR_PT_THREADS, zr::PT_SMEM_BYTES));
+            if (ptBlocks < 1)
+            {
+                zr::set_error("zr_indirect_pass: k_pathtrace (%d threads, %zu B shared) cannot be resident", ZR_PT_THREADS, zr::PT_SMEM_BYTES);
+                return ZR_ERR_UNSUPPORTED;
+            }
+            const size_t ptSmem = (size_t)ptBlocks * (zr::PT_SMEM_BYTES + 1024);
+            ZR_CUDA(cudaFuncSetAttribute(kernel, cudaFuncAttributePreferredSharedMemoryCarveout,
+                (int)((ptSmem * 100 + 228 * 1024 - 1) / (228 * 1024))));
+        }
         return shiftStreams.Init();
     }
 
@@ -573,13 +579,14 @@
 
         int cur = currTemporalIdx;
         const uint32_t dispX = (width + 15) / 16, dispY = (height + 7) / 8;
+        const bool plain = (in->scene->materialFeatures & BSDF::MF_ALL) == 0;
         ZR_PROF("k_pathtrace", stream);
-        k_pathtrace<<<strip.sched.count, ZR_PT_THREADS, PT_SMEM_BYTES, stream>>>(in->scene->dev, f, prm, sz.d_res[cur], sz.d_target, sz.d_final, dispX, dispY,
+        (plain ? k_pathtrace<BSDF::MF_NONE> : k_pathtrace<BSDF::MF_ALL>)<<<strip.sched.count, ZR_PT_THREADS, PT_SMEM_BYTES, stream>>>(in->scene->dev, f, prm, sz.d_res[cur], sz.d_target, sz.d_final, dispX, dispY,
             strip.sched.d_order);
         ZR_LAUNCH_CHECK();
         if (doTemporal)
         {
-            st = sz.queued.RunTemporal(shiftStreams, in->scene->dev, f, prm, sz.d_res[cur], sz.d_res[1 - cur], sz.d_target, sz.d_final, stream);
+            st = sz.queued.RunTemporal(shiftStreams, in->scene->dev, f, prm, sz.d_res[cur], sz.d_res[1 - cur], sz.d_target, sz.d_final, plain, stream);
             if (st != ZR_OK) return st;
         }
         strip.Exchange(sz.d_res[cur], width, height, 64u, stream);
@@ -601,7 +608,7 @@
                     k_sort<<<dim3(sx, ty1 - ty0), 256, 0, stream>>>(f, 3, 1u, rin, nullptr, sz.d_neighbor, sz.d_threadMap, sx, sy, ty0);
                     ZR_LAUNCH_CHECK();
                 }
-                st = sz.queued.Run(shiftStreams, in->scene->dev, f, prm, rin, rout, sz.d_target, sz.d_final, sz.d_neighbor, sz.d_threadMap, stream);
+                st = sz.queued.Run(shiftStreams, in->scene->dev, f, prm, rin, rout, sz.d_target, sz.d_final, sz.d_neighbor, sz.d_threadMap, plain, stream);
                 if (st != ZR_OK) return st;
                 strip.Exchange(rout, width, height, 64u, stream);
             }
diff --git a/zetaray_b200/csrc/rpt_spatial.cu b/zetaray_b200/csrc/rpt_spatial.cu
--- a/zetaray_b200/csrc/rpt_spatial.cu
+++ b/zetaray_b200/csrc/rpt_spatial.cu
@@ -346,7 +346,7 @@
 }
 
 zr_status SpatialQueued::Run(const ShiftStreams& ss, const SceneDev& sc, const FrameView& f, const RptParams& prm, const zr_rpt_reservoir* resIn,
-    zr_rpt_reservoir* resOut, const float4* target, float4* finalImg, const uint16_t* neighbor, const uint16_t* threadMap, cudaStream_t stream)
+    zr_rpt_reservoir* resOut, const float4* target, float4* finalImg, const uint16_t* neighbor, const uint16_t* threadMap, bool plain, cudaStream_t stream)
 {
     const int plane = resIn == mapBase[0] ? 0 : (resIn == mapBase[1] ? 1 : -1);
     if (plane < 0) { set_error("zr_indirect_pass: spatial input is not one of the pass's reservoir planes"); return ZR_ERR_INVALID_ARG; }
@@ -359,7 +359,7 @@
     }
     {
         ZR_PROF("k_shift", stream);
-        const zr_status ls = LaunchShifts<false>(*this, ss, sc, f, prm, resIn, nullptr, neighbor, stream);
+        const zr_status ls = LaunchShifts<false>(*this, ss, sc, f, prm, resIn, nullptr, neighbor, plain, stream);
         zr::prof_after();
         if (ls != ZR_OK) return ls;
         cudaError_t e = cudaGetLastError();
diff --git a/zetaray_b200/csrc/rpt_temporal.cu b/zetaray_b200/csrc/rpt_temporal.cu
--- a/zetaray_b200/csrc/rpt_temporal.cu
+++ b/zetaray_b200/csrc/rpt_temporal.cu
@@ -171,7 +171,7 @@
 }
 
 zr_status SpatialQueued::RunTemporal(const ShiftStreams& ss, const SceneDev& sc, const FrameView& f, const RptParams& prm, zr_rpt_reservoir* resCurr,
-    const zr_rpt_reservoir* resPrev, float4* target, float4* finalImg, cudaStream_t stream)
+    const zr_rpt_reservoir* resPrev, float4* target, float4* finalImg, bool plain, cudaStream_t stream)
 {
     const uint32_t rows = prm.rowEnd - prm.rowBegin;
     const dim3 grid((width + 31) / 32, (rows + 7) / 8);
@@ -183,7 +183,7 @@
     }
     {
         ZR_PROF("k_shift_temporal", stream);
-        const zr_status ls = LaunchShifts<true>(*this, ss, sc, f, prm, resCurr, resPrev, nullptr, stream);
+        const zr_status ls = LaunchShifts<true>(*this, ss, sc, f, prm, resCurr, resPrev, nullptr, plain, stream);
         zr::prof_after();
         if (ls != ZR_OK) return ls;
         cudaError_t e = cudaGetLastError();
diff --git a/zetaray_b200/csrc/scene.cu b/zetaray_b200/csrc/scene.cu
--- a/zetaray_b200/csrc/scene.cu
+++ b/zetaray_b200/csrc/scene.cu
@@ -115,6 +115,14 @@
     UP(emissives, desc->h_emissives, desc->num_emissives);
     sc->dev.numInstances = desc->num_instances;
     sc->dev.numEmissives = desc->num_emissives;
+    for (uint32_t i = 0; i < desc->num_materials; i++)
+    {
+        const zr_material& m = desc->h_materials[i];
+        if ((m.BaseColorTex_Subsurf_CoatWeight >> 24) & 0xff) sc->materialFeatures |= ZR_MATERIAL_COAT;
+        if (m.CoatColor_Flags & (1u << 26)) sc->materialFeatures |= ZR_MATERIAL_TRANSMISSION;
+        if ((m.CoatColor_Flags & (1u << 29)) && ((m.BaseColorTex_Subsurf_CoatWeight >> 16) & 0xff))
+            sc->materialFeatures |= ZR_MATERIAL_THIN_WALLED;
+    }
 
     std::vector<uint32_t> triMesh, meshFirst(desc->num_instances);
     uint32_t total = 0;
@@ -232,6 +240,12 @@
         out[0] = sc->info.numNodes; out[1] = sc->info.numTris; out[2] = sc->info.maxDepth; out[3] = sc->info.bytes;
         return ZR_OK;
     }
+    zr_status zr_scene_material_features(const zr_scene* sc, uint32_t* out)
+    {
+        if (!sc || !out) return ZR_ERR_INVALID_ARG;
+        *out = sc->materialFeatures;
+        return ZR_OK;
+    }
     zr_status zr_scene_trace_closest(const zr_scene* sc, const float* d_rays, uint32_t n, float* d_hits, void* stream)
     {
         if (!sc || !d_rays || !d_hits) { zr::set_error("zr_scene_trace_closest: null argument"); return ZR_ERR_INVALID_ARG; }
diff --git a/zetaray_b200/csrc/zr_bsdf.cuh b/zetaray_b200/csrc/zr_bsdf.cuh
--- a/zetaray_b200/csrc/zr_bsdf.cuh
+++ b/zetaray_b200/csrc/zr_bsdf.cuh
@@ -205,14 +205,27 @@
         return (NDF * G1) / ndotwo;
     }
 
-    struct ShadingData
-    {
+    constexpr uint32_t MF_NONE = 0;
+    constexpr uint32_t MF_ALL = ZR_MATERIAL_COAT | ZR_MATERIAL_TRANSMISSION | ZR_MATERIAL_THIN_WALLED;
+
+    template<bool Stored> struct SpecTrField { bool specTr; };
+    template<> struct SpecTrField<false> { static constexpr bool specTr = false; };
+
+    template<uint32_t MF>
+    struct ShadingDataT : SpecTrField<(MF & ZR_MATERIAL_TRANSMISSION) != 0>
+    {
+        static constexpr bool HasCoat = (MF & ZR_MATERIAL_COAT) != 0;
+        static constexpr bool HasTransmission = (MF & ZR_MATERIAL_TRANSMISSION) != 0;
+        static constexpr bool HasThinWalled = (MF & ZR_MATERIAL_THIN_WALLED) != 0;
+        using ShadingData = ShadingDataT;
+        using SpecTrField<HasTransmission>::specTr;
+
         float alpha;
         float3 wo;
         float ndotwi, ndotwo, ndotwh, whdotwi, whdotwo, wodotwi, g_wo;
         float3 baseColor_Fr0_TrCol;
         float eta;
-        bool specTr, metallic, backfacing_wo, invalid, reflection;
+        bool metallic, backfacing_wo, invalid, reflection;
         float trDepth;
         float subsurface;
         float coat_weight;
@@ -235,7 +248,7 @@
             float coat_roughness = 0, float eta_coat = DEFAULT_ETA_COAT, const uint16_t* rhoTable = nullptr)
         {
             float2 roughness4 = f2(roughness, coat_roughness);
-            if (coat_weight > 0 && coat_roughness > 0)
+            if (HasCoat && coat_weight > 0 && coat_roughness > 0)
             {
                 roughness4 = roughness4 * roughness4;
                 roughness4 = roughness4 * roughness4;
@@ -252,7 +265,8 @@
             si.metallic = metallic;
             si.alpha = roughness * roughness;
             si.baseColor_Fr0_TrCol = baseColor;
-            si.specTr = specTr;
+            if constexpr (HasTransmission)
+                si.specTr = specTr;
             si.trDepth = to_half(transmissionDepth);
             si.subsurface = to_half(subsurface);
             float eta_base = eta_curr == ETA_AIR ? eta_next : eta_curr;
@@ -268,9 +282,10 @@
             return si;
         }
 
-        ZR_D bool ThinWalled() const { return subsurface > 0; }
+        ZR_D bool ThinWalled() const { return HasThinWalled && subsurface > 0; }
         ZR_D bool Transmissive() const { return specTr || ThinWalled(); }
-        ZR_D bool Coated() const { return coat_weight != 0; }
+        ZR_D bool Coated() const { return HasCoat && coat_weight != 0; }
+        ZR_D bool TrDepthGt0() const { return HasTransmission && trDepth > 0; }
         ZR_D bool GlossSpecular() const { return alpha <= MAX_ALPHA_SPECULAR; }
         ZR_D bool CoatSpecular() const { return coat_alpha <= MAX_ALPHA_SPECULAR; }
         ZR_D float3 TransmissionTint() const { return trDepth > 0 ? f3(1) : baseColor_Fr0_TrCol; }
@@ -364,8 +379,10 @@
             return FresnelSchlick_Dielectric(Fr0, cosTheta);
         }
     };
-
-    ZR_D bool IsLobeValid(const ShadingData& surface, LOBE lt)
+    using ShadingData = ShadingDataT<MF_ALL>;
+
+    template<class SD>
+    ZR_D bool IsLobeValid(const SD& surface, LOBE lt)
     {
         if (lt == ALL) return true;
         if (surface.metallic && (lt != GLOSSY_R) && (lt != COAT)) return false;
@@ -375,14 +392,16 @@
         if (!surface.Coated() && (lt == COAT)) return false;
         return true;
     }
-    ZR_D float LobeAlpha(const ShadingData& surface, LOBE lt)
+    template<class SD>
+    ZR_D float LobeAlpha(const SD& surface, LOBE lt)
     {
         if (lt == GLOSSY_R || lt == GLOSSY_T) return surface.alpha;
         if (lt == COAT) return surface.coat_alpha;
         return 1.0f;
     }
 
-    ZR_D float3 EvalDiffuse(bool EON, const ShadingData& surface)
+    template<class SD>
+    ZR_D float3 EvalDiffuse(bool EON, const SD& surface)
     {
         float s = surface.subsurface == 0 ? 1 : surface.subsurface * 0.5f;
         float diffuseRoughness = sqrtf(surface.alpha);
@@ -396,49 +415,58 @@
         Math::CoordinateSystem onb = Math::CoordinateSystem::Build(normal);
         return mad(wiLocal.x, onb.b1, mad(wiLocal.y, onb.b2, wiLocal.z * normal));
     }
-    ZR_D float DiffusePdf(const ShadingData& surface) { return surface.ndotwi * ONE_OVER_PI; }
-    ZR_D float3 EvalGloss(const ShadingData& surface, float3 fr)
+    template<class SD>
+    ZR_D float DiffusePdf(const SD& surface) { return surface.ndotwi * ONE_OVER_PI; }
+    template<class SD>
+    ZR_D float3 EvalGloss(const SD& surface, float3 fr)
     {
         return GGXMicrofacetBRDF(surface.alpha, surface.ndotwh, surface.ndotwo, surface.ndotwi, fr, surface.GlossSpecular());
     }
-    ZR_D float3 SampleGloss(const ShadingData& surface, float3 shadingNormal, float2 u)
+    template<class SD>
+    ZR_D float3 SampleGloss(const SD& surface, float3 shadingNormal, float2 u)
     {
         if (surface.GlossSpecular())
             return reflect(-surface.wo, shadingNormal);
         float3 wh = SampleGGXMicrofacet(surface.wo, surface.alpha, shadingNormal, u);
         return reflect(-surface.wo, wh);
     }
-    ZR_D float GlossPdf(const ShadingData& surface)
+    template<class SD>
+    ZR_D float GlossPdf(const SD& surface)
     {
         if (surface.GlossSpecular())
             return surface.ndotwh >= MIN_N_DOT_H_SPECULAR ? 1.0f : 0.0f;
         float pdf = GGXMicrofacetPdf(surface.alpha, surface.ndotwh, surface.ndotwo);
         return pdf / 4.0f;
     }
-    ZR_D float EvalTranslucentTr(const ShadingData& surface, float fr)
+    template<class SD>
+    ZR_D float EvalTranslucentTr(const SD& surface, float fr)
     {
         return GGXMicrofacetBTDF(surface.alpha, surface.ndotwh, surface.ndotwo, surface.ndotwi, surface.whdotwo,
             surface.whdotwi, surface.eta, fr, surface.GlossSpecular());
     }
-    ZR_D float EvalCoat(const ShadingData& surface, float Fr)
+    template<class SD>
+    ZR_D float EvalCoat(const SD& surface, float Fr)
     {
         return surface.coat_weight * GGXMicrofacetBRDF(surface.coat_alpha, surface.ndotwh, surface.ndotwo, surface.ndotwi,
             f3(Fr), surface.CoatSpecular()).x;
     }
-    ZR_D float3 SampleCoat(const ShadingData& surface, float3 shadingNormal, float2 u)
+    template<class SD>
+    ZR_D float3 SampleCoat(const SD& surface, float3 shadingNormal, float2 u)
     {
         float3 wh = surface.CoatSpecular() ? shadingNormal :
             SampleGGXMicrofacet(surface.wo, surface.coat_alpha, shadingNormal, u);
         return reflect(-surface.wo, wh);
     }
-    ZR_D float CoatPdf(const ShadingData& surface)
+    template<class SD>
+    ZR_D float CoatPdf(const SD& surface)
     {
         if (surface.CoatSpecular())
             return surface.ndotwh >= MIN_N_DOT_H_SPECULAR ? 1.0f : 0.0f;
         float pdf = GGXMicrofacetPdf(surface.coat_alpha, surface.ndotwh, surface.ndotwo);
         return pdf / 4.0f;
     }
-    ZR_D float3 TranslucentTrOverPdf(const ShadingData& surface, float fr)
+    template<class SD>
+    ZR_D float3 TranslucentTrOverPdf(const SD& surface, float fr)
     {
         if (surface.GlossSpecular())
             return (1 - fr) * surface.TransmissionTint();
@@ -449,7 +477,8 @@
     {
         return f3(zr_expf(c * zr_logf(coat_color.x)), zr_expf(c * zr_logf(coat_color.y)), zr_expf(c * zr_logf(coat_color.z)));
     }
-    ZR_D float3 BaseWeight(const ShadingData& surface)
+    template<class SD>
+    ZR_D float3 BaseWeight(const SD& surface)
     {
         float3 base_weight = f3(1);
         if (surface.Coated())
@@ -467,14 +496,16 @@
         }
         return base_weight;
     }
-    ZR_D float3 TransmittanceToDielectricBaseTr(const ShadingData& surface)
+    template<class SD>
+    ZR_D float3 TransmittanceToDielectricBaseTr(const SD& surface)
     {
         float3 base_weight = BaseWeight(surface);
         float reflectance_g = surface.GlossSpecular() ? 0 :
             GGXReflectance_Dielectric(surface.rho, surface.alpha, surface.ndotwo, surface.eta);
         return (1 - reflectance_g) * base_weight;
     }
-    ZR_D float3 DielectricBaseSpecularTr(const ShadingData& surface, float Fr_g)
+    template<class SD>
+    ZR_D float3 DielectricBaseSpecularTr(const SD& surface, float Fr_g)
     {
         if (surface.invalid || !surface.specTr)
             return f3(0);
@@ -482,7 +513,8 @@
         float glossyTr = EvalTranslucentTr(surface, Fr_g);
         return glossyTr * surface.TransmissionTint() * transmittance;
     }
-    ZR_D float3 DielectricBaseDiffuseTr(const ShadingData& surface, float Fr_g)
+    template<class SD>
+    ZR_D float3 DielectricBaseDiffuseTr(const SD& surface, float Fr_g)
     {
         if (surface.invalid)
             return f3(0);
@@ -494,7 +526,8 @@
 
     struct BSDFEval { float3 f; float3 Fr_g; bool tir; };
 
-    ZR_D BSDFEval Unified(const ShadingData& surface)
+    template<class SD>
+    ZR_D BSDFEval Unified(const SD& surface)
     {
         BSDFEval ret;
         ret.f = f3(0); ret.Fr_g = f3(0); ret.tir = false;
@@ -554,7 +587,8 @@
     };
     struct BSDFSamplerEval { float pdf; float3 bsdfOverPdf; float3 f; };
 
-    ZR_D BSDFSample SampleBSDF_NoDiffuse(float3 normal, ShadingData surface, float2 u_c, float2 u_g,
+    template<class SD>
+    ZR_D BSDFSample SampleBSDF_NoDiffuse(float3 normal, SD surface, float2 u_c, float2 u_g,
         float u_wrs_0, float u_wrs_1)
     {
         BSDFSample ret = BSDFSample::Init();
@@ -616,7 +650,8 @@
         return ret;
     }
 
-    ZR_D BSDFSample SampleBSDF_NoDiffuse(float3 normal, const ShadingData& surface, RNG& rng)
+    template<class SD>
+    ZR_D BSDFSample SampleBSDF_NoDiffuse(float3 normal, const SD& surface, RNG& rng)
     {
         float2 u_c = rng.Uniform2D();
         float2 u_g = rng.Uniform2D();
@@ -625,7 +660,8 @@
         return SampleBSDF_NoDiffuse(normal, surface, u_c, u_g, u_wrs_0, u_wrs_1);
     }
 
-    ZR_D BSDFSample SampleBSDF_NoSpecTr(float3 normal, ShadingData surface, float2 u_coat, float2 u_g, float2 u_d,
+    template<class SD>
+    ZR_D BSDFSample SampleBSDF_NoSpecTr(float3 normal, SD surface, float2 u_coat, float2 u_g, float2 u_d,
         float u_wrs_g, float u_wrs_dr, float u_wrs_dt)
     {
         BSDFSample ret = BSDFSample::Init();
@@ -707,7 +743,8 @@
         return ret;
     }
 
-    ZR_D BSDFSample SampleBSDF(float3 normal, const ShadingData& surface, RNG& rng)
+    template<class SD>
+    ZR_D BSDFSample SampleBSDF(float3 normal, const SD& surface, RNG& rng)
     {
         float2 u_c = rng.Uniform2D();
         float2 u_g = rng.Uniform2D();
@@ -720,7 +757,8 @@
         return SampleBSDF_NoDiffuse(normal, surface, u_c, u_g, u_wrs_0, u_wrs_1);
     }
 
-    ZR_D BSDFSamplerEval EvalBSDFSampler_NoSpecTr(float3 normal, ShadingData surface, float3 wi, LOBE lobe,
+    template<class SD>
+    ZR_D BSDFSamplerEval EvalBSDFSampler_NoSpecTr(float3 normal, SD surface, float3 wi, LOBE lobe,
         float2 u_c, float2 u_g, float2 u_d)
     {
         BSDFSamplerEval ret;
@@ -786,7 +824,8 @@
         return ret;
     }
 
-    ZR_D BSDFSamplerEval EvalBSDFSampler_NoDiffuse(float3 normal, ShadingData surface, float3 wi, LOBE lobe)
+    template<class SD>
+    ZR_D BSDFSamplerEval EvalBSDFSampler_NoDiffuse(float3 normal, SD surface, float3 wi, LOBE lobe)
     {
         float3 wh = surface.SetWi(wi, normal);
         BSDFEval eval = Unified(surface);
@@ -838,7 +877,8 @@
         return ret;
     }
 
-    ZR_D BSDFSamplerEval EvalBSDFSampler(float3 normal, const ShadingData& surface, float3 wi, LOBE lobe, RNG& rng)
+    template<class SD>
+    ZR_D BSDFSamplerEval EvalBSDFSampler(float3 normal, const SD& surface, float3 wi, LOBE lobe, RNG& rng)
     {
         float2 u_c = rng.Uniform2D();
         float2 u_g = rng.Uniform2D();
@@ -849,7 +889,8 @@
         return EvalBSDFSampler_NoDiffuse(normal, surface, wi, lobe);
     }
 
-    ZR_D float BSDFSamplerPdf_NoDiffuse(float3 normal, ShadingData surface, float3 wi)
+    template<class SD>
+    ZR_D float BSDFSamplerPdf_NoDiffuse(float3 normal, SD surface, float3 wi)
     {
         float3 wh = surface.SetWi(wi, normal);
         float pdf_base = 1;
@@ -892,7 +933,8 @@
         return pdf_g;
     }
 
-    ZR_D float BSDFSamplerPdf(float3 normal, ShadingData surface, float3 wi_z, RNG& rng)
+    template<class SD>
+    ZR_D float BSDFSamplerPdf(float3 normal, SD surface, float3 wi_z, RNG& rng)
     {
         if (surface.specTr)
             return BSDFSamplerPdf_NoDiffuse(normal, surface, wi_z);
diff --git a/zetaray_b200/csrc/zr_pixel.cuh b/zetaray_b200/csrc/zr_pixel.cuh
--- a/zetaray_b200/csrc/zr_pixel.cuh
+++ b/zetaray_b200/csrc/zr_pixel.cuh
@@ -61,12 +61,14 @@
         atomicAdd(&costMap[(size_t)(y >> 5) * ((W + 31) >> 5) + (x >> 5)], (unsigned long long)(clock64() - t0));
 }
 
-struct Pixel
+template<class SD>
+struct PixelT
 {
     GFlags flags; float roughness; float z; float3 pos, normal, origin; float2 lensSample;
-    BSDF::ShadingData surface; float eta_next;
+    SD surface; float eta_next;
     float coatRoughness, coatIor;
 };
+using Pixel = PixelT<BSDF::ShadingData>;
 
 ZR_D float3 row3(const float m[3][4], int r) { return f3(m[r][0], m[r][1], m[r][2]); }
 
@@ -77,11 +79,12 @@
     return DecodeFlags(w & 0xff);
 }
 
-ZR_D Pixel LoadPixel(const FrameView& f, const SceneDev& sc, const uint4* __restrict__ core, const uint2* __restrict__ coat,
+template<class SD = BSDF::ShadingData>
+ZR_D PixelT<SD> LoadPixel(const FrameView& f, const SceneDev& sc, const uint4* __restrict__ core, const uint2* __restrict__ coat,
     int px, int py, bool prev, int coatX, int coatY)
 {
     const zr_frame_constants& fc = f.fc;
-    Pixel p;
+    PixelT<SD> p;
     const uint4 c = ld128(&core[(size_t)py * f.W + px]);
     p.flags = DecodeFlags(c.w & 0xff);
     p.roughness = (float)((c.w >> 8) & 0xff) / 255.0f;
@@ -120,7 +123,7 @@
     }
     p.coatRoughness = coat_roughness; p.coatIor = coat_ior;
     const float3 wo = normalize(p.origin - p.pos);
-    p.surface = BSDF::ShadingData::Init(p.normal, wo, p.flags.metallic, p.roughness, baseColor, BSDF::ETA_AIR, p.eta_next,
+    p.surface = SD::Init(p.normal, wo, p.flags.metallic, p.roughness, baseColor, BSDF::ETA_AIR, p.eta_next,
         p.flags.transmissive, p.flags.trDepthGt0 ? 1.0f : 0.0f, to_half(baseW), coat_weight, coat_color, coat_roughness,
         coat_ior, sc.rho);
     return p;
diff --git a/zetaray_b200/csrc/zr_rdi.cuh b/zetaray_b200/csrc/zr_rdi.cuh
--- a/zetaray_b200/csrc/zr_rdi.cuh
+++ b/zetaray_b200/csrc/zr_rdi.cuh
@@ -136,7 +136,8 @@
 };
 
 #define ZR_PHASE() __syncthreads()
-ZR_D Reservoir RIS_InitialCandidates_Sync(bool act, const SceneDev& sc, float3 pos, float3 normal, float roughness, BSDF::ShadingData surface,
+template<class SD>
+ZR_D Reservoir RIS_InitialCandidates_Sync(bool act, const SceneDev& sc, float3 pos, float3 normal, float roughness, SD surface,
     uint32_t sampleSetIdx, int numBsdfSamples, RNG& rng)
 {
     Reservoir r = Reservoir::Init();
@@ -249,11 +250,14 @@
     return fabsf(planeDist) <= tolerance * linearDepth;
 }
 
-struct TemporalCandidate { BSDF::ShadingData surface; float3 pos, normal; int px, py; bool valid; };
-
-ZR_D TemporalCandidate FindTemporalCandidate(const FrameView& f, const SceneDev& sc, float3 pos, float3 normal, float roughness, const BSDF::ShadingData& surface, float2 prevUV)
-{
-    TemporalCandidate c; c.valid = false; c.px = c.py = 0; c.pos = c.normal = f3(0);
+template<class SD>
+struct TemporalCandidateT { SD surface; float3 pos, normal; int px, py; bool valid; };
+using TemporalCandidate = TemporalCandidateT<BSDF::ShadingData>;
+
+template<class SD>
+ZR_D TemporalCandidateT<SD> FindTemporalCandidate(const FrameView& f, const SceneDev& sc, float3 pos, float3 normal, float roughness, const SD& surface, float2 prevUV)
+{
+    TemporalCandidateT<SD> c; c.valid = false; c.px = c.py = 0; c.pos = c.normal = f3(0);
     if (prevUV.x < 0.0f || prevUV.y < 0.0f || prevUV.x > 1.0f || prevUV.y > 1.0f) return c;
     const float2 renderDim = f2((float)f.W, (float)f.H);
     float2 pp = prevUV * renderDim;
@@ -263,14 +267,15 @@
     if (prevFlags.invalid || prevFlags.emissive || (fabsf(prevRoughness - roughness) > 0.15f) ||
         (prevFlags.metallic != surface.metallic) || (prevFlags.transmissive != surface.specTr))
         return c;
-    Pixel p = LoadPixel(f, sc, f.pcore, f.pcoat, ppx, ppy, true, ppx, ppy);
+    const PixelT<SD> p = LoadPixel<SD>(f, sc, f.pcore, f.pcoat, ppx, ppy, true, ppx, ppy);
     if (!PlaneHeuristicDI(p.pos, normal, pos, p.z))
         return c;
     c.surface = p.surface; c.px = ppx; c.py = ppy; c.pos = p.pos; c.normal = p.normal; c.valid = true;
     return c;
 }
 
-ZR_D void TemporalResample1_Sync(bool act, const SceneDev& sc, float3 pos, float3 normal, const BSDF::ShadingData& surface, TemporalCandidate candidate,
+template<class SD>
+ZR_D void TemporalResample1_Sync(bool act, const SceneDev& sc, float3 pos, float3 normal, const SD& surface, TemporalCandidateT<SD> candidate,
     const zr_rdi_reservoir* prevRes, uint32_t W, Reservoir& r_curr, RNG& rng)
 {
     Reservoir r_prev = Reservoir::Init();
@@ -314,7 +319,7 @@
     }
     const bool doTtC = act && (r_prev.lightIdx != UINT32_MAX_);
     EmissiveData prevEmissive;
-    BSDF::ShadingData surfaceWi = surface;
+    SD surfaceWi = surface;
     float3 target_curr = f3(0);
     if (doTtC)
     {
@@ -377,8 +382,9 @@
         const float denom = numerator + ((float)r_c.M / (float)k) * p_c_y_c;
         m_c += 1 - (numerator / denom);
     }
-    ZR_D void Stream_Sync(bool act, const SceneDev& sc, const Reservoir& r_c, float3 pos_c, float3 normal_c, BSDF::ShadingData surface_c, const Reservoir& r_i,
-        float3 pos_i, float3 normal_i, BSDF::ShadingData surface_i, RNG& rng)
+    template<class SD>
+    ZR_D void Stream_Sync(bool act, const SceneDev& sc, const Reservoir& r_c, float3 pos_c, float3 normal_c, SD surface_c, const Reservoir& r_i,
+        float3 pos_i, float3 normal_i, SD surface_i, RNG& rng)
     {
         float3 target_c_y_i = f3(0), target_i_y_c = f3(0.0f);
         float m_i = 0;
diff --git a/zetaray_b200/csrc/zr_rpt.cuh b/zetaray_b200/csrc/zr_rpt.cuh
--- a/zetaray_b200/csrc/zr_rpt.cuh
+++ b/zetaray_b200/csrc/zr_rpt.cuh
@@ -255,7 +255,8 @@
         }
     };
 
-    ZR_D bool IsSpecularSurface(const ShadingData& surface)
+    template<class SD>
+    ZR_D bool IsSpecularSurface(const SD& surface)
     {
         return surface.GlossSpecular() && (surface.metallic || surface.specTr) && (!surface.Coated() || surface.CoatSpecular());
     }
@@ -348,7 +349,8 @@
         return rs;
     }
 
-    ZR_D DirectLightingEstimate NEE_Bsdf_Finish(const SceneDev& sc, float3 pos, const ShadingData& surface, int nextBounce,
+    template<class SD>
+    ZR_D DirectLightingEstimate NEE_Bsdf_Finish(const SceneDev& sc, float3 pos, const SD& surface, int nextBounce,
         int maxNumBounces, BSDF::BSDFSample& bsdfSample, const HitEmissive& hitInfo)
     {
         DirectLightingEstimate ret = DirectLightingEstimate::Init();
@@ -390,7 +392,8 @@
 
     struct NeeLightState { DirectLightingEstimate ret; float3 ld; float t, lightPdf, dwdA; bool facing; };
 
-    ZR_D NeeLightState NEE_Emissive_Begin(const SceneDev& sc, float3 pos, float3 normal, ShadingData& surface, uint32_t sampleSetIdx, RNG& rng)
+    template<class SD>
+    ZR_D NeeLightState NEE_Emissive_Begin(const SceneDev& sc, float3 pos, float3 normal, SD& surface, uint32_t sampleSetIdx, RNG& rng)
     {
         NeeLightState st;
         st.ret = DirectLightingEstimate::Init();
@@ -426,24 +429,25 @@
 
     struct OffsetPath { float3 target; float partialJacobian; bool surfKMin1Tramsmissive; };
 
-    struct OffsetPathContext
+    template<class SD>
+    struct OffsetPathContextT
     {
         float3 throughput, pos, normal;
-        ShadingData surface;
+        SD surface;
         float eta_curr, eta_next;
         RNG rngReplay;
 
-        static ZR_D OffsetPathContext Init()
-        {
-            OffsetPathContext c;
+        static ZR_D OffsetPathContextT Init()
+        {
+            OffsetPathContextT c;
             c.throughput = f3(0); c.pos = f3(0); c.normal = f3(0);
-            c.surface = ShadingData::InitEmpty();
+            c.surface = SD::InitEmpty();
             c.eta_curr = BSDF::ETA_AIR; c.eta_next = BSDF::DEFAULT_ETA_MAT; c.rngReplay.State = 0;
             return c;
         }
-        ZR_D OffsetPathContext Quantize() const
-        {
-            OffsetPathContext ctx = Init();
+        ZR_D OffsetPathContextT Quantize() const
+        {
+            OffsetPathContextT ctx = Init();
             ctx.throughput = f3(to_half(throughput.x), to_half(throughput.y), to_half(throughput.z));
             if (dot(ctx.throughput, ctx.throughput) == 0)
                 return ctx;
@@ -469,16 +473,18 @@
                 float coat_eta = surface.coat_eta >= 1.0f ? surface.coat_eta : 1.0f / surface.coat_eta;
                 coat_ior = mad(Math::UNorm8ToFloat(Math::FloatToUNorm8((coat_eta - 1.0f) / 1.5f)), 1.5f, 1.0f);
             }
-            ctx.surface = ShadingData::Init(ctx.normal, wo, metallic, roughness, baseColor, ctx.eta_curr, eta_next_, specTr,
+            ctx.surface = SD::Init(ctx.normal, wo, metallic, roughness, baseColor, ctx.eta_curr, eta_next_, specTr,
                 trDepth, to_half(subsurface), coat_weight, coat_color, coat_roughness, coat_ior, surface.rho);
             return ctx;
         }
     };
-
-    ZR_D OffsetPathContext Replay_kGt2_Sync(bool act, const SceneDev& sc, float3 pos, float3 normal, float ior, const ShadingData& surface,
+    using OffsetPathContext = OffsetPathContextT<ShadingData>;
+
+    template<class SD>
+    ZR_D OffsetPathContextT<SD> Replay_kGt2_Sync(bool act, const SceneDev& sc, float3 pos, float3 normal, float ior, const SD& surface,
         const Reconnection& rc, float alpha_min)
     {
-        OffsetPathContext ctx = OffsetPathContext::Init();
+        OffsetPathContextT<SD> ctx = OffsetPathContextT<SD>::Init();
         BSDF::BSDFSample bsdfSample = BSDF::BSDFSample::Init();
         const int numBounces = (int)rc.k - 2;
         int bounce = 0;
@@ -523,7 +529,7 @@
                     ctx.pos = mad(hitInfo.t, bsdfSample.wi, ctx.pos);
                     ctx.normal = hitInfo.normal;
                     bounce++;
-                    if (inTranslucentMedium && (ctx.surface.trDepth > 0))
+                    if (inTranslucentMedium && ctx.surface.TrDepthGt0())
                     {
                         float3 c = ctx.surface.baseColor_Fr0_TrCol;
                         float3 extCoeff = f3(-zr_logf(c.x), -zr_logf(c.y), -zr_logf(c.z)) / ctx.surface.trDepth;
@@ -557,12 +563,12 @@
         return ctx;
     }
 
-    template<int CASE = 0>
-    ZR_D OffsetPath Shift2_Sync(bool act, const SceneDev& sc, float3 pos, float3 normal, float ior, const ShadingData& surface,
-        const Reconnection& rc, const OffsetPathContext* replayed, float alpha_min)
+    template<int CASE = 0, class SD>
+    ZR_D OffsetPath Shift2_Sync(bool act, const SceneDev& sc, float3 pos, float3 normal, float ior, const SD& surface,
+        const Reconnection& rc, const OffsetPathContextT<SD>* replayed, float alpha_min)
     {
         OffsetPath ret; ret.target = f3(0); ret.partialJacobian = 0; ret.surfKMin1Tramsmissive = false;
-        OffsetPathContext ctx = OffsetPathContext::Init();
+        OffsetPathContextT<SD> ctx = OffsetPathContextT<SD>::Init();
         const bool case1 = CASE == 0 ? rc.IsCase1() : CASE == 1, case2 = CASE == 0 ? rc.IsCase2() : CASE == 2,
             case3 = CASE == 0 ? rc.IsCase3() : CASE == 3;
         bool go = act;
@@ -644,7 +650,7 @@
                 if (!GetMaterialData(sc, -w_k_min_1, ctx.eta_curr, hitInfo, ctx.surface, ctx.eta_next)) { step = false; go = false; }
                 else
                 {
-                    if (inTranslucentMedium && (ctx.surface.trDepth > 0))
+                    if (inTranslucentMedium && ctx.surface.TrDepthGt0())
                     {
                         float3 c = ctx.surface.baseColor_Fr0_TrCol;
                         float3 extCoeff = f3(-zr_logf(c.x), -zr_logf(c.y), -zr_logf(c.z)) / ctx.surface.trDepth;
@@ -662,7 +668,7 @@
             }
         }
         const bool nee = go && !case1;
-        ShadingData surfWi = ctx.surface;
+        SD surfWi = ctx.surface;
         float3 wiE = rc.w_k_lightNormal_w_sky;
         float3 nrmE = ctx.normal;
         LOBE lobeE = rc.lobe_k;
diff --git a/zetaray_b200/csrc/zr_rpt_io.cuh b/zetaray_b200/csrc/zr_rpt_io.cuh
--- a/zetaray_b200/csrc/zr_rpt_io.cuh
+++ b/zetaray_b200/csrc/zr_rpt_io.cuh
@@ -133,8 +133,9 @@
 
     struct PrevHit { float alpha_lobe; float3 wi; float pdf; BSDF::LOBE lobe; };
 
+    template<class SD>
     ZR_D void MaybeSetCase2OrCase3(int pathVertex, float3 pos, float3 normal, float t, uint32_t ID, uint32_t meshIdx,
-        const BSDF::ShadingData& surface, const PrevHit& prevHit, const DirectLightingEstimate& ls, uint32_t seed_nee,
+        const SD& surface, const PrevHit& prevHit, const DirectLightingEstimate& ls, uint32_t seed_nee,
         Reconnection& rc, float alpha_min)
     {
         const float alpha_lobe_direct = BSDF::LobeAlpha(surface, ls.lobe);
diff --git a/zetaray_b200/csrc/zr_rpt_shift.cuh b/zetaray_b200/csrc/zr_rpt_shift.cuh
--- a/zetaray_b200/csrc/zr_rpt_shift.cuh
+++ b/zetaray_b200/csrc/zr_rpt_shift.cuh
@@ -24,11 +24,12 @@
     }
 
 
-    template<int CASE, bool REPLAY, bool TEMPORAL>
+    template<int CASE, bool REPLAY, bool TEMPORAL, uint32_t MF>
     __global__ void __launch_bounds__(SHIFT_THREADS, SHIFT_MINBLOCKS) k_shift(SceneDev sc, FrameView f, RptParams prm,
         const zr_rpt_reservoir* __restrict__ resIn, const zr_rpt_reservoir* __restrict__ resPrev, const uint16_t* __restrict__ neighbor,
         const uint32_t* __restrict__ queue, uint32_t* __restrict__ counters, uint32_t cls, ShiftResult* __restrict__ out)
     {
+        using SD = BSDF::ShadingDataT<MF>;
         __shared__ uint32_t s_base;
         const uint32_t total = counters[cls];
         for (;;)
@@ -43,7 +44,7 @@
             uint32_t dir = 0;
             bool replayOk = act;
             Reservoir r = Reservoir::Init();
-            Pixel p, pr;
+            PixelT<SD> p, pr;
             if (act)
             {
                 const uint32_t item = __ldg(&queue[base + threadIdx.x]);
@@ -57,11 +58,11 @@
                     r = Reservoir::Load_NonReconnection(rec);
                     r.rc.x_k_in_motion = false;
                     r.Load_Reconnection(rec);
-                    if (dir == 0) p = LoadPixel(f, sc, f.core, f.coat, nx, ny, false, x, y);
-                    else p = LoadPixel(f, sc, f.core, f.coat, x, y, false, x, y);
+                    if (dir == 0) p = LoadPixel<SD>(f, sc, f.core, f.coat, nx, ny, false, x, y);
+                    else p = LoadPixel<SD>(f, sc, f.core, f.coat, x, y, false, x, y);
                     if (REPLAY)
                     {
-                        if (dir == 0) pr = LoadPixel(f, sc, f.core, f.coat, nx, ny, false, nx, ny);
+                        if (dir == 0) pr = LoadPixel<SD>(f, sc, f.core, f.coat, nx, ny, false, nx, ny);
                         else pr = p;
                     }
                 }
@@ -78,12 +79,12 @@
                         if (dir == 0) XkToPrev(sc, r.rc);
                         else XkToCurr(sc, r.rc);
                     }
-                    if (dir == 0) p = LoadPixel(f, sc, f.pcore, f.pcoat, ppx, ppy, true, x, y);
-                    else p = LoadPixel(f, sc, f.core, f.coat, x, y, false, x, y);
+                    if (dir == 0) p = LoadPixel<SD>(f, sc, f.pcore, f.pcoat, ppx, ppy, true, x, y);
+                    else p = LoadPixel<SD>(f, sc, f.core, f.coat, x, y, false, x, y);
                     if (REPLAY) pr = p;
                 }
             }
-            OffsetPathContext ctx = OffsetPathContext::Init();
+            OffsetPathContextT<SD> ctx = OffsetPathContextT<SD>::Init();
             if (REPLAY)
             {
                 ZR_PHASE();
@@ -111,7 +112,7 @@
 
     template<bool TEMPORAL>
     zr_status LaunchShifts(const SpatialQueued& q, const ShiftStreams& ss, const SceneDev& sc, const FrameView& f, const RptParams& prm,
-        const zr_rpt_reservoir* resIn, const zr_rpt_reservoir* resPrev, const uint16_t* neighbor, cudaStream_t stream)
+        const zr_rpt_reservoir* resIn, const zr_rpt_reservoir* resPrev, const uint16_t* neighbor, bool plain, cudaStream_t stream)
     {
         const uint32_t grid = (uint32_t)ss.numSMs * SHIFT_MINBLOCKS;
         cudaStream_t s1 = ss.aux[0], s2 = ss.aux[1];
@@ -119,7 +120,7 @@
         ZR_CUDA(cudaStreamWaitEvent(s1, ss.evFork, 0));
         ZR_CUDA(cudaStreamWaitEvent(s2, ss.evFork, 0));
 #define ZR_LAUNCH_SHIFT(CASE, REPLAY, CLS, STREAM) \
-        k_shift<CASE, REPLAY, TEMPORAL><<<grid, SHIFT_THREADS, 0, STREAM>>>(sc, f, prm, resIn, resPrev, neighbor, q.d_queue + (size_t)(CLS) * q.capacity, \
+        (plain ? k_shift<CASE, REPLAY, TEMPORAL, BSDF::MF_NONE> : k_shift<CASE, REPLAY, TEMPORAL, BSDF::MF_ALL>)<<<grid, SHIFT_THREADS, 0, STREAM>>>(sc, f, prm, resIn, resPrev, neighbor, q.d_queue + (size_t)(CLS) * q.capacity, \
             q.d_counters, CLS, q.d_shift); \
         zr::count_launch()
         ZR_LAUNCH_SHIFT(1, false, 0, stream);
diff --git a/zetaray_b200/csrc/zr_rpt_spatial.h b/zetaray_b200/csrc/zr_rpt_spatial.h
--- a/zetaray_b200/csrc/zr_rpt_spatial.h
+++ b/zetaray_b200/csrc/zr_rpt_spatial.h
@@ -43,8 +43,9 @@
 
     zr_status Build(uint32_t w, uint32_t h, const zr_rpt_reservoir* res0, const zr_rpt_reservoir* res1);
     zr_status Run(const ShiftStreams& ss, const SceneDev& sc, const FrameView& f, const RptParams& prm, const zr_rpt_reservoir* resIn,
-        zr_rpt_reservoir* resOut, const float4* target, float4* finalImg, const uint16_t* neighbor, const uint16_t* threadMap, cudaStream_t stream);
+        zr_rpt_reservoir* resOut, const float4* target, float4* finalImg, const uint16_t* neighbor, const uint16_t* threadMap, bool plain,
+        cudaStream_t stream);
     zr_status RunTemporal(const ShiftStreams& ss, const SceneDev& sc, const FrameView& f, const RptParams& prm, zr_rpt_reservoir* resCurr,
-        const zr_rpt_reservoir* resPrev, float4* target, float4* finalImg, cudaStream_t stream);
+        const zr_rpt_reservoir* resPrev, float4* target, float4* finalImg, bool plain, cudaStream_t stream);
 };
 }
diff --git a/zetaray_b200/csrc/zr_rt.cuh b/zetaray_b200/csrc/zr_rt.cuh
--- a/zetaray_b200/csrc/zr_rt.cuh
+++ b/zetaray_b200/csrc/zr_rt.cuh
@@ -162,7 +162,8 @@
     return true;
 }
 
-ZR_D bool GetMaterialData(const SceneDev& sc, float3 wo, float eta_curr, Hit& hitInfo, BSDF::ShadingData& surface, float& eta)
+template<class SD>
+ZR_D bool GetMaterialData(const SceneDev& sc, float3 wo, float eta_curr, Hit& hitInfo, SD& surface, float& eta)
 {
     const zr_material mat = LoadMaterial(sc, hitInfo.matIdx);
     const bool hitBackface = dot(wo, hitInfo.normal) < 0;
@@ -183,7 +184,7 @@
     float3 coat_color = Mat::GetCoatColor(mat);
     float coat_roughness = Mat::GetCoatRoughness(mat);
     float coat_ior = Mat::GetCoatIOR(mat);
-    surface = BSDF::ShadingData::Init(hitInfo.normal, wo, metallic >= 0.9f, roughness, baseColor, eta_curr, eta_next, tr,
+    surface = SD::Init(hitInfo.normal, wo, metallic >= 0.9f, roughness, baseColor, eta_curr, eta_next, tr,
         trDepth, subsurface, coat_weight, coat_color, coat_roughness, coat_ior, sc.rho);
     return true;
 }
diff --git a/zetaray_b200/csrc/zr_scene.cuh b/zetaray_b200/csrc/zr_scene.cuh
--- a/zetaray_b200/csrc/zr_scene.cuh
+++ b/zetaray_b200/csrc/zr_scene.cuh
@@ -280,4 +280,5 @@
     bool samplesValid = false;
     zr_voxel_sample* d_lvg = nullptr;
     bool lvgValid = false;
+    uint32_t materialFeatures = 0;
 };
```

Measured after the change: 313.8, median of 6. 9.4% higher.
